# uncbiag/OAI_analysis_2

Measured on AMD Instinct MI355X. Metric: knee MRI volumes/sec (segment+register), 384x384x160 fp32, higher is better.
Workload: dtype fp16x3 (every fp32 value held as 2 fp16 terms = 22 mantissa bits, 3 MFMA passes per product, fp32 accumulate; fp32 in and out of every entry point; full-size parity vs the reference in `parity`)

## Files before the change

### include/oai_hip.h

```cpp
#ifndef OAI_HIP_H
#define OAI_HIP_H

#include <stddef.h>
#include <stdint.h>

#ifdef __cplusplus
extern "C" {
#endif

#define OAI_OK 0
#define OAI_ERR_ARG 1
#define OAI_ERR_HIP 2
#define OAI_ERR_WORKSPACE 3

int oai_version(void);
const char* oai_last_error(void);
int oai_device_info(char* name, int cap);


int oai_grid_sample3d(const float* src_dev, int C, int d, int h, int w,
                      const float* coords_dev, int D, int H, int W, float* out_dev, void* stream);

int oai_warp_set_option(const char* name, int value);

int oai_compose(const float* disp_dev, int d, int h, int w, const float* coords_dev,
                int D, int H, int W, int shortcut, float* out_dev, void* stream);

int oai_avgpool2_3d(const float* in_dev, int C, int D, int H, int W, float* out_dev, void* stream);

int oai_resize_trilinear(const float* in_dev, int C, int d, int h, int w,
                         float* out_dev, int D, int H, int W, void* stream);

int oai_phi_to_itk_displacement(const float* phi_dev, int D, int H, int W, double* disp_dev, void* stream);

#define OAI_WARP_CHAIN_MAX_FIELDS 8
int oai_warp_chain(const float* start_dev, int D, int H, int W, int n_fields, const float* const* fields,
                   const int* field_dims_zyx, const float* image_dev, int id, int ih, int iw, float* out_dev, void* stream);

typedef struct oai_affine { double A[9]; double b[3]; } oai_affine;

int oai_resample_through_disp(const float* prob_dev, int nzA, int nyA, int nxA,
                              const double* disp_dev, int Dn, int Hn, int Wn,
                              const oai_affine* b_index_to_net, const oai_affine* net_to_a_index,
                              float* out_dev, int nzB, int nyB, int nxB, void* stream);

int oai_resample_maps_through_phi(const float* probs_dev, int n_maps, int nzA, int nyA, int nxA,
                                  const float* phi_dev, int Dn, int Hn, int Wn,
                                  const oai_affine* b_index_to_net, const oai_affine* net_to_a_index,
                                  float* out_dev, int nzB, int nyB, int nxB, void* stream);

size_t oai_image_normalize_workspace_bytes(void);
int oai_image_normalize(const float* in_dev, size_t n, float pct_lo, float pct_hi, float out_min, float out_max,
                        float* out_dev, float* window_out_dev, void* workspace_dev, size_t workspace_bytes, void* stream);


typedef struct oai_unet oai_unet;

typedef struct oai_layer_params {
    int kind, cin, cout;
    const float* weight_host;
    const float* bias_host;
    const float* bn_gamma_host;
    const float* bn_beta_host;
    const float* bn_mean_host;
    const float* bn_var_host;
} oai_layer_params;

#define OAI_UNET_NUM_LAYERS 18

int oai_unet_create(const oai_layer_params layers_host[OAI_UNET_NUM_LAYERS], float bn_eps, oai_unet** out);
void oai_unet_destroy(oai_unet* h);

#define OAI_PREC_F32 0
#define OAI_PREC_BF16X3 1
#define OAI_PREC_BF16X6 2
#define OAI_PREC_FP16X3 3
int oai_unet_set_precision(oai_unet* h, int mode);
int oai_unet_range_flag(oai_unet* h, int reset, int* out, void* stream);
int oai_unet_range_flag_snapshot(oai_unet* h, int* dst_dev, void* stream);
#define OAI_UNET_RANGE_STATE_WORDS (1 + OAI_UNET_NUM_LAYERS)
int oai_unet_range_state_snapshot(oai_unet* h, int* state_dev, void* stream);
int oai_unet_range_flag_from_state(const int* state_dev, int* flag_dev, void* stream);
int oai_unet_census(oai_unet* h, float max_out[OAI_UNET_NUM_LAYERS], int reset, void* stream);
int oai_unet_calibrate_step(oai_unet* h, void* stream, int* more);
int oai_unet_get_act_exponents(const oai_unet* h, int e_out[OAI_UNET_NUM_LAYERS], int* calibrated);
int oai_unet_set_act_exponents(oai_unet* h, const int e[OAI_UNET_NUM_LAYERS]);
int oai_unet_set_option(oai_unet* h, const char* name, int value);

size_t oai_unet_workspace_bytes(const oai_unet* h, int td, int th, int tw, int batch);
size_t oai_segment_workspace_bytes(const oai_unet* h, int D, int H, int W, const int tile_zyx[3], const int overlap_zyx[3], int batch);

int oai_unet_forward_tiles(oai_unet* h, const float* tiles_dev, float* logits_dev, int B,
                           int td, int th, int tw, void* workspace_dev, size_t workspace_bytes,
                           void* stream);

int oai_segment_tiles(oai_unet* h, const float* vol_dev, int D, int H, int W,
                      const int tile_zyx[3], const int overlap_zyx[3], const int crop_zyx[3],
                      int tile_begin, int tile_end,
                      int out_mode, float* blocks_dev, int batch,
                      void* workspace_dev, size_t workspace_bytes, void* stream);

int oai_stitch_blocks(const float* blocks_dev, int n_classes, int D, int H, int W,
                      const int tile_zyx[3], const int overlap_zyx[3], const int crop_zyx[3],
                      float* maps_dev, void* stream);

int oai_stitch_blocks_ranged(const float* blocks_dev, int n_classes, int D, int H, int W,
                             const int tile_zyx[3], const int overlap_zyx[3], const int crop_zyx[3],
                             const int* bounds_host, int n_ranges, int slot_stride,
                             float* maps_dev, void* stream);

int oai_partition_tiles(const float* vol_dev, int D, int H, int W, const int tile_zyx[3], const int overlap_zyx[3],
                        int tile_begin, int tile_end, float* tiles_dev, void* stream);

int oai_assemble_vote(const int* tile_labels_dev, int n_labels, int D, int H, int W, const int tile_zyx[3], const int overlap_zyx[3],
                      unsigned char* out_dev, void* stream);

int oai_unet_profile(oai_unet* h, int enable);
int oai_unet_profile_read(oai_unet* h, double* conv3_ms, long long* conv3_launches);

double oai_unet_tile_flops(const oai_unet* h, int td, int th, int tw, const int overlap_zyx[3], int trimmed);
double oai_unet_volume_flops(const oai_unet* h, int D, int H, int W, const int tile_zyx[3], const int overlap_zyx[3],
                             const int crop_zyx[3], int trimmed, int conv3_only);
int oai_unet_tile_costs(const oai_unet* h, int D, int H, int W, const int tile_zyx[3], const int overlap_zyx[3],
                        const int crop_zyx[3], double* costs_host, int n_tiles);
double oai_unet_tile_flops_conv3(const oai_unet* h, int td, int th, int tw, const int overlap_zyx[3], int trimmed);


typedef struct oai_icon oai_icon;

typedef struct oai_icon_unet_params {
    const float* down_w[5]; const float* down_b[5];
    const float* up_w[5];   const float* up_b[5];
    const float* bn_gamma[5]; const float* bn_beta[5]; const float* bn_mean[5]; const float* bn_var[5];
    const float* last_w; const float* last_b;
} oai_icon_unet_params;

enum { OAI_ICON_FFVF = 0, OAI_ICON_DOWN = 1, OAI_ICON_TWO = 2 };
typedef struct oai_icon_node { int kind; int a; int b; } oai_icon_node;

int oai_icon_create(const oai_icon_unet_params* nets_host, int n_nets, const oai_icon_node* nodes_host, int n_nodes, int root,
                    int D, int H, int W, oai_icon** out);
int oai_icon_describe(const oai_icon* h, int* n_nets, int* levels_host, int* chain_len);
void oai_icon_destroy(oai_icon* h);
size_t oai_icon_workspace_bytes(const oai_icon* h);

int oai_icon_forward(oai_icon* h, const float* A_dev, const float* B_dev, float* phi_dev,
                     void* workspace_dev, size_t workspace_bytes, void* stream);

int oai_icon_set_graph(oai_icon* h, int enable);
int oai_icon_set_option(oai_icon* h, const char* name, int value);
int oai_icon_graph_info(const oai_icon* h, int* captured, long long* replays, long long* direct_runs);

int oai_icon_unet_forward(oai_icon* h, int which, const float* a_dev, const float* b_dev, int D, int H, int W,
                          float* out_dev, void* workspace_dev, size_t workspace_bytes, void* stream);

int oai_mc_table(signed char* out_256x16_host);
size_t oai_mc_workspace_bytes(int D, int H, int W);
int oai_mc_count(const float* vol_dev, int D, int H, int W, float iso, void* workspace_dev, size_t workspace_bytes,
                 long long* n_verts_host, long long* n_tris_host, void* stream);
int oai_mc_emit(const float* vol_dev, int D, int H, int W, float iso, const float spacing_xyz_host[3], const void* workspace_dev,
                float* verts_dev, int* faces_dev, void* stream);
int oai_mesh_smooth(const float* verts_in_dev, long long n_verts, const int* offsets_dev, const int* neighbours_dev,
                    int iterations, float relaxation, float* tmp_dev, float* verts_out_dev, void* stream);
int oai_mesh_point_distance(const float* points_dev, long long n_points, const float* verts_dev, const int* faces_dev,
                            long long n_tris, float* dist_dev, void* stream);
size_t oai_mesh_grid_workspace_bytes(const int grid_dims_xyz[3], long long n_tris);
int oai_mesh_point_distance_grid(const float* points_dev, long long n_points, const float* verts_dev, const int* faces_dev,
                                 long long n_tris, const float grid_lo_xyz_host[3], float cell_size, const int grid_dims_xyz_host[3],
                                 void* workspace_dev, size_t workspace_bytes, float* dist_dev, void* stream);

int oai_map_attributes(const float* src_pts_dev, long long n_src, const float* src_vals_dev, int n_comp, const float* tgt_pts_dev,
                       long long n_tgt, double radius, float* out_vals_dev, void* stream);
size_t oai_point_grid_workspace_bytes(const int grid_dims_xyz[3], long long n_src);
int oai_map_attributes_grid(const float* src_pts_dev, long long n_src, const float* src_vals_dev, int n_comp, const float* tgt_pts_dev,
                            long long n_tgt, double radius, const double grid_lo_xyz_host[3], double cell_size, const int grid_dims_xyz_host[3],
                            void* workspace_dev, size_t workspace_bytes, float* out_vals_dev, void* stream);
int oai_point_footprint(const float* src_pts_dev, long long n_src, const float* tgt_pts_dev, long long n_tgt, double radius, int* count_dev,
                        double* nearest_d2_dev, int* nearest_j_dev, void* stream);
int oai_point_footprint_grid(const float* src_pts_dev, long long n_src, const float* tgt_pts_dev, long long n_tgt, double radius,
                             const double grid_lo_xyz_host[3], double cell_size, const int grid_dims_xyz_host[3], void* workspace_dev,
                             size_t workspace_bytes, int* count_dev, double* nearest_d2_dev, int* nearest_j_dev, void* stream);
size_t oai_thickness_map_workspace_bytes(long long n_points);
int oai_fit_circle(const float* pts_dev, long long n, int col_x, int col_y, void* workspace_dev, size_t workspace_bytes, double centre_host[2],
                   double* radius_host, int* iterations_host, void* stream);
int oai_project_circle(const float* pts_dev, long long n, int col_x, int col_y, const double centre_host[2], double* angle_dev, double* z_dev,
                       void* stream);
int oai_project_plateaus(const float* pts_dev, const float* thickness_dev, long long n, void* workspace_dev, size_t workspace_bytes,
                         double* x_dev, double* y_dev, double* thickness_out_dev, long long* n_right_host, long long* n_left_host, void* stream);

size_t oai_thickness_image_workspace_bytes(long long n_faces, int height, int width);
int oai_thickness_image_build(const double* uv_dev, long long n_pts, const int* faces_dev, long long n_faces, const unsigned char* face_skip_dev,
                              const double lo_host[2], const double step_host[2], int height, int width, void* workspace_dev,
                              size_t workspace_bytes, int* owner_dev, int* corners_dev, double* weights_dev, long long* n_covered_host,
                              void* stream);
int oai_thickness_image_apply(const int* owner_dev, const int* corners_dev, const double* weights_dev, int height, int width,
                              const float* values_dev, long long n_pts, int n_knees, float* image_dev, void* stream);

#define OAI_MESH_FC 0
#define OAI_MESH_TC 1
size_t oai_mesh_split_workspace_bytes(long long n_verts, long long n_faces, int mesh_type, int n_init);
int oai_mesh_split_features(const float* verts_dev, long long n_verts, const int* faces_dev, long long n_faces, int mesh_type,
                            void* workspace_dev, size_t workspace_bytes, double* centroids_dev, double* normals_dev,
                            long long slab_counts_host[3], void* stream);
int oai_mesh_split_kmeans(long long n_faces, int mesh_type, void* workspace_dev, size_t workspace_bytes, const double* normals_dev, int n_init,
                          int max_iter, const long long slab_counts_host[3], const long long* first_centre_host, const double* uniforms_host,
                          signed char* side_dev, int* n_iter_host, void* stream);
size_t oai_mesh_submesh_workspace_bytes(long long n_verts, long long n_faces);
int oai_mesh_submesh(const float* verts_dev, long long n_verts, const int* faces_dev, long long n_faces, const signed char* side_dev, int which,
                     void* workspace_dev, size_t workspace_bytes, float* verts_out_dev, int* faces_out_dev, int* face_idx_out_dev,
                     long long* n_verts_out_host, long long* n_faces_out_host, void* stream);

size_t oai_mesh_components_workspace_bytes(long long n_verts, long long n_faces);
int oai_mesh_components(const int* faces_dev, long long n_faces, long long n_verts, void* workspace_dev, size_t workspace_bytes, int* label_dev,
                        int* rounds_host, void* stream);
size_t oai_mesh_keep_large_regions_workspace_bytes(long long n_verts, long long n_faces);
int oai_mesh_keep_large_regions(const float* verts_dev, long long n_verts, const int* faces_dev, long long n_faces, long long min_cells,
                                void* workspace_dev, size_t workspace_bytes, float* verts_out_dev, int* faces_out_dev, long long* n_verts_out_host,
                                long long* n_faces_out_host, void* stream);
size_t oai_mesh_adjacency_workspace_bytes(long long n_verts, long long n_faces);
int oai_mesh_adjacency(const int* faces_dev, long long n_faces, long long n_verts, void* workspace_dev, size_t workspace_bytes, int* offsets_dev,
                       int* nbrs_dev, long long* n_nbrs_host, void* stream);
size_t oai_mesh_grid_params_workspace_bytes(void);
int oai_mesh_grid_params(const float* verts_dev, long long n_verts, const int* faces_dev, long long n_faces, void* workspace_dev,
                         size_t workspace_bytes, double* out7_dev, void* stream);

size_t oai_cuberille_workspace_bytes(int D, int H, int W);
int oai_cuberille_count(const float* vol_dev, int D, int H, int W, float iso, void* workspace_dev, size_t workspace_bytes,
                        long long* n_verts_host, long long* n_faces_host, void* stream);
int oai_cuberille_emit(const float* vol_dev, int D, int H, int W, float iso, const double geometry_host[24], int flip_winding, int triangles,
                       int project, double threshold, double step_length, double relaxation, int max_steps, int move_after_converged,
                       void* workspace_dev, size_t workspace_bytes, long long n_verts, long long n_faces, float* verts_dev, int* faces_dev,
                       int* steps_dev, void* stream);

int oai_transform_points_through_phi(const float* pts_dev, long long n, const float* phi_dev, int Dn, int Hn, int Wn,
                                     const oai_affine* point_to_net, const oai_affine* net_to_out, float* out_dev, unsigned char* inside_dev,
                                     void* stream);

size_t oai_phi_jacobian_workspace_bytes(int D, int H, int W);
int oai_phi_jacobian(const float* phi_dev, int D, int H, int W, float* det_out_dev, void* workspace_dev, size_t workspace_bytes,
                     double* stats_dev, void* stream);
size_t oai_mask_overlap_workspace_bytes(long long n);
int oai_mask_overlap(const float* a_dev, const float* b_dev, long long n, float threshold, void* workspace_dev, size_t workspace_bytes,
                     long long* counts_dev, void* stream);

int oai_inverse_points_through_phi(const float* pts_dev, long long n, const float* phi_dev, int Dn, int Hn, int Wn,
                                   const oai_affine* point_to_net, const oai_affine* net_to_out, int max_iter, double tol, float* out_dev,
                                   unsigned char* status_dev, void* stream);
size_t oai_invert_phi_workspace_bytes(int D, int H, int W);
int oai_invert_phi(const float* phi_dev, int D, int H, int W, int max_iter, double tol, float* psi_out_dev, unsigned char* status_out_dev,
                   void* workspace_dev, size_t workspace_bytes, double* stats_dev, void* stream);

int oai_mask_surface(const float* map_dev, int D, int H, int W, float threshold, int mode, unsigned char* out_dev, void* stream);
size_t oai_edt_workspace_bytes(int D, int H, int W);
int oai_edt(const unsigned char* feature_dev, int D, int H, int W, const double spacing_xyz[3], float scale, int accumulate, float* dist_dev,
            double* sq_out_dev, void* workspace_dev, size_t workspace_bytes, long long* n_features_dev, void* stream);
size_t oai_surface_distance_workspace_bytes(long long n);
int oai_surface_distance(const unsigned char* surf_a_dev, const float* dist_to_b_dev, const unsigned char* surf_b_dev, const float* dist_to_a_dev,
                         long long n, const float* percentiles, int n_percentiles, void* workspace_dev, size_t workspace_bytes, double* out_dev,
                         void* stream);

size_t oai_image_moments_workspace_bytes(long long n);
int oai_image_moments(const float* a_dev, const float* b_dev, long long n, const unsigned char* mask_dev, void* workspace_dev,
                      size_t workspace_bytes, double* stats_dev, void* stream);
int oai_joint_histogram(const float* a_dev, const float* b_dev, long long n, const float range_a[2], const float range_b[2], int bins,
                        const unsigned char* mask_dev, long long* hist_dev, void* stream);
int oai_histogram_entropies(const long long* hist_dev, int bins, double* out_dev, void* stream);
size_t oai_lncc_workspace_bytes(int D, int H, int W);
int oai_lncc(const float* a_dev, const float* b_dev, int D, int H, int W, const double* taps_host, int radius, double eps,
             const unsigned char* mask_dev, double* cc_out_dev, void* workspace_dev, size_t workspace_bytes, double* stats_dev, void* stream);

size_t oai_label_components_workspace_bytes(int D, int H, int W);
int oai_label_components(const float* map_dev, const unsigned char* mask_dev, int D, int H, int W, float threshold, int complement,
                         int connectivity, long long min_voxels, int* labels_dev, int* size_dev, void* workspace_dev, size_t workspace_bytes,
                         long long* summary_dev, void* stream);
int oai_component_sizes(const int* labels_dev, long long n, long long n_components, long long* sizes_dev, void* stream);

size_t oai_local_thickness_workspace_bytes(int D, int H, int W);
// ... 19 lines not shown
```

### oai_analysis_2_amd/_lib.py

```python
from __future__ import annotations

import ctypes as C
import os
from typing import Optional

HERE = os.path.dirname(os.path.abspath(__file__))
LIB_PATH = os.environ.get("OAI_LIB_PATH") or os.path.join(HERE, "liboai_hip.so")


class OaiError(RuntimeError):
    pass


class Affine(C.Structure):
    _fields_ = [("A", C.c_double * 9), ("b", C.c_double * 3)]


class LayerParams(C.Structure):
    _fields_ = [("kind", C.c_int), ("cin", C.c_int), ("cout", C.c_int),
                ("weight", C.c_void_p), ("bias", C.c_void_p),
                ("bn_gamma", C.c_void_p), ("bn_beta", C.c_void_p), ("bn_mean", C.c_void_p), ("bn_var", C.c_void_p)]


class IconUnetParams(C.Structure):
    _fields_ = [("down_w", C.c_void_p * 5), ("down_b", C.c_void_p * 5),
                ("up_w", C.c_void_p * 5), ("up_b", C.c_void_p * 5),
                ("bn_gamma", C.c_void_p * 5), ("bn_beta", C.c_void_p * 5),
                ("bn_mean", C.c_void_p * 5), ("bn_var", C.c_void_p * 5),
                ("last_w", C.c_void_p), ("last_b", C.c_void_p)]


class IconNode(C.Structure):
    _fields_ = [("kind", C.c_int), ("a", C.c_int), ("b", C.c_int)]


_I, _P, _F, _Z, _D = C.c_int, C.c_void_p, C.c_float, C.c_size_t, C.c_double
_I3 = C.POINTER(C.c_int)
SIGNATURES = {
    "oai_version": (_I, []),
    "oai_last_error": (C.c_char_p, []),
    "oai_device_info": (_I, [C.c_char_p, _I]),
    "oai_grid_sample3d": (_I, [_P, _I, _I, _I, _I, _P, _I, _I, _I, _P, _P]),
    "oai_compose": (_I, [_P, _I, _I, _I, _P, _I, _I, _I, _I, _P, _P]),
    "oai_avgpool2_3d": (_I, [_P, _I, _I, _I, _I, _P, _P]),
    "oai_resize_trilinear": (_I, [_P, _I, _I, _I, _I, _P, _I, _I, _I, _P]),
    "oai_phi_to_itk_displacement": (_I, [_P, _I, _I, _I, _P, _P]),
    "oai_resample_through_disp": (_I, [_P, _I, _I, _I, _P, _I, _I, _I, C.POINTER(Affine), C.POINTER(Affine),
                                       _P, _I, _I, _I, _P]),
    "oai_warp_chain": (_I, [_P, _I, _I, _I, _I, C.POINTER(_P), C.POINTER(_I), _P, _I, _I, _I, _P, _P]),
    "oai_resample_maps_through_phi": (_I, [_P, _I, _I, _I, _I, _P, _I, _I, _I, C.POINTER(Affine), C.POINTER(Affine),
                                           _P, _I, _I, _I, _P]),
    "oai_unet_tile_costs": (_I, [_P, _I, _I, _I, C.POINTER(C.c_int), C.POINTER(C.c_int), C.POINTER(C.c_int), C.POINTER(C.c_double), _I]),
    "oai_mc_table": (_I, [_P]),
    "oai_mc_workspace_bytes": (_Z, [_I, _I, _I]),
    "oai_mc_count": (_I, [_P, _I, _I, _I, _F, _P, _Z, C.POINTER(C.c_longlong), C.POINTER(C.c_longlong), _P]),
    "oai_mc_emit": (_I, [_P, _I, _I, _I, _F, C.POINTER(C.c_float), _P, _P, _P, _P]),
    "oai_mesh_smooth": (_I, [_P, C.c_longlong, _P, _P, _I, _F, _P, _P, _P]),
    "oai_mesh_point_distance": (_I, [_P, C.c_longlong, _P, _P, C.c_longlong, _P, _P]),
    "oai_mesh_grid_workspace_bytes": (_Z, [C.POINTER(C.c_int), C.c_longlong]),
    "oai_mesh_point_distance_grid": (_I, [_P, C.c_longlong, _P, _P, C.c_longlong, C.POINTER(C.c_float), _F, C.POINTER(C.c_int), _P, _Z, _P, _P]),
    "oai_map_attributes": (_I, [_P, C.c_longlong, _P, _I, _P, C.c_longlong, _D, _P, _P]),
    "oai_point_grid_workspace_bytes": (_Z, [C.POINTER(C.c_int), C.c_longlong]),
    "oai_map_attributes_grid": (_I, [_P, C.c_longlong, _P, _I, _P, C.c_longlong, _D, C.POINTER(_D), _D, C.POINTER(C.c_int), _P, _Z, _P, _P]),
    "oai_point_footprint": (_I, [_P, C.c_longlong, _P, C.c_longlong, _D, _P, _P, _P, _P]),
    "oai_point_footprint_grid": (_I, [_P, C.c_longlong, _P, C.c_longlong, _D, C.POINTER(_D), _D, C.POINTER(C.c_int), _P, _Z, _P, _P, _P, _P]),
    "oai_thickness_map_workspace_bytes": (_Z, [C.c_longlong]),
    "oai_fit_circle": (_I, [_P, C.c_longlong, _I, _I, _P, _Z, C.POINTER(_D), C.POINTER(_D), C.POINTER(_I), _P]),
    "oai_project_circle": (_I, [_P, C.c_longlong, _I, _I, C.POINTER(_D), _P, _P, _P]),
    "oai_project_plateaus": (_I, [_P, _P, C.c_longlong, _P, _Z, _P, _P, _P, C.POINTER(C.c_longlong), C.POINTER(C.c_longlong), _P]),
    "oai_thickness_image_workspace_bytes": (_Z, [C.c_longlong, _I, _I]),
    "oai_thickness_image_build": (_I, [_P, C.c_longlong, _P, C.c_longlong, _P, C.POINTER(_D), C.POINTER(_D), _I, _I, _P, _Z, _P, _P, _P,
                                       C.POINTER(C.c_longlong), _P]),
    "oai_thickness_image_apply": (_I, [_P, _P, _P, _I, _I, _P, C.c_longlong, _I, _P, _P]),
    "oai_mesh_split_workspace_bytes": (_Z, [C.c_longlong, C.c_longlong, _I, _I]),
    "oai_mesh_split_features": (_I, [_P, C.c_longlong, _P, C.c_longlong, _I, _P, _Z, _P, _P, C.POINTER(C.c_longlong), _P]),
    "oai_mesh_split_kmeans": (_I, [C.c_longlong, _I, _P, _Z, _P, _I, _I, C.POINTER(C.c_longlong), C.POINTER(C.c_longlong), C.POINTER(_D), _P,
                                   C.POINTER(_I), _P]),
    "oai_mesh_submesh_workspace_bytes": (_Z, [C.c_longlong, C.c_longlong]),
    "oai_mesh_submesh": (_I, [_P, C.c_longlong, _P, C.c_longlong, _P, _I, _P, _Z, _P, _P, _P, C.POINTER(C.c_longlong), C.POINTER(C.c_longlong), _P]),
    "oai_mesh_components_workspace_bytes": (_Z, [C.c_longlong, C.c_longlong]),
    "oai_mesh_components": (_I, [_P, C.c_longlong, C.c_longlong, _P, _Z, _P, C.POINTER(_I), _P]),
    "oai_mesh_keep_large_regions_workspace_bytes": (_Z, [C.c_longlong, C.c_longlong]),
    "oai_mesh_keep_large_regions": (_I, [_P, C.c_longlong, _P, C.c_longlong, C.c_longlong, _P, _Z, _P, _P, C.POINTER(C.c_longlong),
                                         C.POINTER(C.c_longlong), _P]),
    "oai_mesh_adjacency_workspace_bytes": (_Z, [C.c_longlong, C.c_longlong]),
    "oai_mesh_adjacency": (_I, [_P, C.c_longlong, C.c_longlong, _P, _Z, _P, _P, C.POINTER(C.c_longlong), _P]),
    "oai_mesh_grid_params_workspace_bytes": (_Z, []),
    "oai_mesh_grid_params": (_I, [_P, C.c_longlong, _P, C.c_longlong, _P, _Z, _P, _P]),
    "oai_cuberille_workspace_bytes": (_Z, [_I, _I, _I]),
    "oai_cuberille_count": (_I, [_P, _I, _I, _I, _F, _P, _Z, C.POINTER(C.c_longlong), C.POINTER(C.c_longlong), _P]),
    "oai_cuberille_emit": (_I, [_P, _I, _I, _I, _F, C.POINTER(_D), _I, _I, _I, _D, _D, _D, _I, _I, _P, _Z, C.c_longlong, C.c_longlong,
                                _P, _P, _P, _P]),
    "oai_transform_points_through_phi": (_I, [_P, C.c_longlong, _P, _I, _I, _I, C.POINTER(Affine), C.POINTER(Affine), _P, _P, _P]),
    "oai_phi_jacobian_workspace_bytes": (_Z, [_I, _I, _I]),
    "oai_phi_jacobian": (_I, [_P, _I, _I, _I, _P, _P, _Z, _P, _P]),
    "oai_inverse_points_through_phi": (_I, [_P, C.c_longlong, _P, _I, _I, _I, C.POINTER(Affine), C.POINTER(Affine), _I, _D, _P, _P, _P]),
    "oai_invert_phi_workspace_bytes": (_Z, [_I, _I, _I]),
    "oai_invert_phi": (_I, [_P, _I, _I, _I, _I, _D, _P, _P, _P, _Z, _P, _P]),
    "oai_mask_overlap_workspace_bytes": (_Z, [C.c_longlong]),
    "oai_mask_overlap": (_I, [_P, _P, C.c_longlong, _F, _P, _Z, _P, _P]),
    "oai_mask_surface": (_I, [_P, _I, _I, _I, _F, _I, _P, _P]),
    "oai_edt_workspace_bytes": (_Z, [_I, _I, _I]),
    "oai_edt": (_I, [_P, _I, _I, _I, C.POINTER(_D), _F, _I, _P, _P, _P, _Z, _P, _P]),
    "oai_surface_distance_workspace_bytes": (_Z, [C.c_longlong]),
    "oai_surface_distance": (_I, [_P, _P, _P, _P, C.c_longlong, C.POINTER(_F), _I, _P, _Z, _P, _P]),
    "oai_image_moments_workspace_bytes": (_Z, [C.c_longlong]),
    "oai_image_moments": (_I, [_P, _P, C.c_longlong, _P, _P, _Z, _P, _P]),
    "oai_joint_histogram": (_I, [_P, _P, C.c_longlong, C.POINTER(_F), C.POINTER(_F), _I, _P, _P, _P]),
    "oai_histogram_entropies": (_I, [_P, _I, _P, _P]),
    "oai_lncc_workspace_bytes": (_Z, [_I, _I, _I]),
    "oai_lncc": (_I, [_P, _P, _I, _I, _I, C.POINTER(_D), _I, _D, _P, _P, _P, _Z, _P, _P]),
    "oai_label_components_workspace_bytes": (_Z, [_I, _I, _I]),
    "oai_label_components": (_I, [_P, _P, _I, _I, _I, _F, _I, _I, C.c_longlong, _P, _P, _P, _Z, _P, _P]),
    "oai_component_sizes": (_I, [_P, C.c_longlong, C.c_longlong, _P, _P]),
    "oai_local_thickness_workspace_bytes": (_Z, [_I, _I, _I]),
    "oai_local_thickness": (_I, [_P, _I, _I, _I, C.POINTER(_D), C.c_longlong, _P, _P, _P, _Z, _P, _P]),
    "oai_masked_stats_workspace_bytes": (_Z, [C.c_longlong]),
    "oai_masked_stats": (_I, [_P, _P, C.c_longlong, C.POINTER(_F), _I, _P, _Z, _P, _P]),
    "oai_mesh_areas_workspace_bytes": (_Z, [C.c_longlong, C.c_longlong]),
    "oai_mesh_areas": (_I, [_P, C.c_longlong, _P, C.c_longlong, _P, _Z, _P, _P, _P]),
    "oai_region_stats_workspace_bytes": (_Z, [C.c_longlong, _I]),
    "oai_region_stats": (_I, [_P, _P, _P, _P, C.c_longlong, _I, _P, _Z, _P, _P]),
    "oai_image_normalize_workspace_bytes": (_Z, []),
    "oai_image_normalize": (_I, [_P, _Z, _F, _F, _F, _F, _P, _P, _P, _Z, _P]),
    "oai_partition_tiles": (_I, [_P, _I, _I, _I, _I3, _I3, _I, _I, _P, _P]),
    "oai_assemble_vote": (_I, [_P, _I, _I, _I, _I, _I3, _I3, _P, _P]),
    "oai_unet_create": (_I, [C.POINTER(LayerParams), _F, C.POINTER(_P)]),
    "oai_unet_destroy": (None, [_P]),
    "oai_unet_set_precision": (_I, [_P, _I]),
    "oai_unet_range_flag": (_I, [_P, _I, C.POINTER(_I), _P]),
    "oai_unet_range_flag_snapshot": (_I, [_P, _P, _P]),
    "oai_unet_range_state_snapshot": (_I, [_P, _P, _P]),
    "oai_unet_range_flag_from_state": (_I, [_P, _P, _P]),
    "oai_unet_census": (_I, [_P, C.POINTER(_F), _I, _P]),
    "oai_unet_calibrate_step": (_I, [_P, _P, C.POINTER(_I)]),
    "oai_unet_get_act_exponents": (_I, [_P, C.POINTER(_I), C.POINTER(_I)]),
    "oai_unet_set_act_exponents": (_I, [_P, C.POINTER(_I)]),
    "oai_unet_set_option": (_I, [_P, C.c_char_p, _I]),
    "oai_unet_workspace_bytes": (_Z, [_P, _I, _I, _I, _I]),
    "oai_segment_workspace_bytes": (_Z, [_P, _I, _I, _I, _I3, _I3, _I]),
    "oai_unet_forward_tiles": (_I, [_P, _P, _P, _I, _I, _I, _I, _P, _Z, _P]),
    "oai_segment_tiles": (_I, [_P, _P, _I, _I, _I, _I3, _I3, _I3, _I, _I, _I, _P, _I, _P, _Z, _P]),
    "oai_unet_volume_flops": (_D, [_P, _I, _I, _I, _I3, _I3, _I3, _I, _I]),
    "oai_warp_set_option": (_I, [C.c_char_p, _I]),
    "oai_stitch_blocks": (_I, [_P, _I, _I, _I, _I, _I3, _I3, _I3, _P, _P]),
    "oai_stitch_blocks_ranged": (_I, [_P, _I, _I, _I, _I, _I3, _I3, _I3, _P, _I, _I, _P, _P]),
    "oai_unet_tile_flops": (_D, [_P, _I, _I, _I, _I3, _I]),
    "oai_unet_tile_flops_conv3": (_D, [_P, _I, _I, _I, _I3, _I]),
    "oai_unet_profile": (_I, [_P, _I]),
    "oai_unet_profile_read": (_I, [_P, C.POINTER(_D), C.POINTER(C.c_longlong)]),
    "oai_icon_create": (_I, [C.POINTER(IconUnetParams), _I, C.POINTER(IconNode), _I, _I, _I, _I, _I, C.POINTER(_P)]),
    "oai_icon_describe": (_I, [_P, C.POINTER(_I), C.POINTER(_I), C.POINTER(_I)]),
    "oai_icon_destroy": (None, [_P]),
    "oai_icon_workspace_bytes": (_Z, [_P]),
    "oai_icon_forward": (_I, [_P, _P, _P, _P, _P, _Z, _P]),
    "oai_icon_set_graph": (_I, [_P, _I]),
    "oai_icon_set_option": (_I, [_P, C.c_char_p, _I]),
    "oai_icon_graph_info": (_I, [_P, C.POINTER(_I), C.POINTER(C.c_longlong), C.POINTER(C.c_longlong)]),
    "oai_icon_unet_forward": (_I, [_P, _I, _P, _P, _I, _I, _I, _P, _P, _Z, _P]),
}

_lib: Optional[C.CDLL] = None


def load() -> C.CDLL:
    global _lib
    if _lib is not None:
        return _lib
    import torch
    if not os.path.exists(LIB_PATH):
        raise OaiError(f"{LIB_PATH} is missing: build it with `python -m oai_analysis_2_amd.build` "
                       "(there is no CPU fallback in this package)")
    lib = C.CDLL(LIB_PATH)
    for name, (res, args) in SIGNATURES.items():
        fn = getattr(lib, name, None)
        if fn is None:
            raise OaiError(f"liboai_hip.so does not export {name}")
        fn.restype = res
        fn.argtypes = args
    _lib = lib
    return lib


def check(status: int, what: str = "") -> None:
    if status != 0:
        msg = load().oai_last_error()
        raise OaiError(f"{what or 'liboai_hip'} failed ({status}): {msg.decode() if msg else '?'}")


STREAM = object()


def call(name: str, *args, device=None) -> None:
    if name not in SIGNATURES:
        raise OaiError(f"{name} is not an entry point of liboai_hip.so (include/oai_hip.h declares none of that name)")
    if device is None:
        if any(a is STREAM for a in args):
            raise ValueError(f"{name}: STREAM stands for the current stream of a device, and no device was given")
        check(getattr(load(), name)(*args), name)
        return
    import torch
    with torch.cuda.device(device):
        stream = torch.cuda.current_stream().cuda_stream
        check(getattr(load(), name)(*[stream if a is STREAM else a for a in args]), name)

# ... 10 lines not shown
```

### oai_analysis_2_amd/csrc/unet.hip

```cpp
#include <cmath>
#include <cstdint>
#include <cstdlib>
#include <cstring>
#include <vector>

#include "common.h"
#include "unet_kernels.h"
#include "unet_sres.h"
#include "unet_sres2.h"
#include "unet_wino.h"
#include "unet_wino_f32.h"

namespace oai {

enum LayerId { EC0, EC1, EC2, EC3, EC4, EC5, EC6, EC7, DC9, DC8, DC7, DC6, DC5, DC4, DC3, DC2, DC1, DC0 };
__host__ __device__ static inline int layer_level(int k) { const int v[18] = {0, 0, 1, 1, 2, 2, 3, 3, 2, 2, 2, 1, 1, 1, 0, 0, 0, 0}; return v[k]; }
__host__ __device__ static inline int layer_kind(int k) { const int v[18] = {0, 0, 0, 0, 0, 0, 0, 0, 2, 1, 1, 2, 1, 1, 2, 1, 1, 3}; return v[k]; }
static const int kKind[18] = {0, 0, 0, 0, 0, 0, 0, 0, 2, 1, 1, 2, 1, 1, 2, 1, 1, 3};

struct Layer {
    int kind = 0, cin = 0, cout = 0;
    int c0 = 0, c1 = 0;
    float4* panel = nullptr;
    float4* panel_bf[3] = {nullptr, nullptr, nullptr};
    float* scale_f16 = nullptr;
    float* shift_f16 = nullptr;
    float* plain_f16 = nullptr;
    std::vector<float> ws;
    int rel1 = 0;
    size_t panel_f16_floats = 0;
    float4* panel_wino_f32 = nullptr;
    float4* panel_wino = nullptr;
    size_t panel_wino_floats = 0;
    float4* panel_wino16 = nullptr;
    size_t panel_wino16_floats = 0;
    float4* panel_m16 = nullptr;
    size_t panel_m16_floats = 0;
    std::vector<float> wk_host;
    std::vector<float> scale_host, shift_host, plain_host;
    float* plain = nullptr;
    float* scale = nullptr;
    float* shift = nullptr;
};

}

struct oai_unet {
    oai::Layer L[18];
    int variant = 0;
    int precision = OAI_PREC_F32;
    int* range_flag = nullptr;
    unsigned* census = nullptr;
    int* eval_out = nullptr;
    int act_exp[18] = {0};
    bool calibrated = false;
    int opt_wino_f32 = 1;
    int opt_first_blocks = 24;
    int opt_up_nbw = 0;
    int opt_shared = 1;
    int opt_wide = 1;
    int opt_wino = 19;
    int opt_wino_layers = 0x3FFFF;
    int opt_m16 = 1;
    int opt_m16_layers = 0x3FFFF;
    int opt_dead_stores = 1;
    int opt_census = 1;
    int xcd_group = 32;
    int fuse_first = 1;
    int sres_mrep = 4;
    bool opt_sres = true;
    bool sres = false;
    unsigned char* zero_rec = nullptr;
    int n_classes = 0;
    std::vector<void*> allocs;
    bool profile = false;
    std::vector<hipEvent_t> ev_pool;
    size_t ev_used = 0;
};

#ifdef OAI_DIAG
static unsigned long long* g_diag_stamps = nullptr;
static unsigned long long* diag_stamps() {
    if (!g_diag_stamps && oai::diag_env("OAI_STAMPS", 0)) {
        if (hipMalloc((void**)&g_diag_stamps, 32 * sizeof(unsigned long long)) != hipSuccess) return nullptr;
        (void)hipMemset(g_diag_stamps, 0, 32 * sizeof(unsigned long long));
    }
    return g_diag_stamps;
}
extern "C" int oai_diag_stamps(unsigned long long out[32], int reset) {
    if (!g_diag_stamps) return 1;
    if (hipMemcpy(out, g_diag_stamps, 32 * sizeof(unsigned long long), hipMemcpyDeviceToHost) != hipSuccess) return 2;
    if (reset) (void)hipMemset(g_diag_stamps, 0, 32 * sizeof(unsigned long long));
    return 0;
}
#endif

namespace oai {

static int conv_kc(int variant) { return variant == 1 ? 16 : 8; }

static std::vector<float> canonical_k3(const oai_layer_params& p) {
    std::vector<float> w((size_t)27 * p.cin * p.cout);
    for (int t = 0; t < 27; ++t)
        for (int ci = 0; ci < p.cin; ++ci)
            for (int co = 0; co < p.cout; ++co) {
                float v;
                if (p.kind == 0) v = p.weight_host[((size_t)co * p.cin + ci) * 27 + t];
                else v = p.weight_host[((size_t)ci * p.cout + co) * 27 + (26 - t)];
                w[((size_t)t * p.cin + ci) * p.cout + co] = v;
            }
    return w;
}

struct ChunkSrc {
    bool first;
    int Csrc, cofs, cl0;
    ChunkSrc(int ch, int C0, int C1, int KC) {
        const int nch0 = (C0 + KC - 1) / KC;
        first = ch < nch0; Csrc = first ? C0 : C1; cofs = first ? 0 : C0; cl0 = (first ? ch : ch - nch0) * KC;
    }
};

static std::vector<float> pack_conv3_panel(const std::vector<float>& wk, int C0, int C1, int Cout, int KC) {
    const int Cin = C0 + C1, KG = KC / 8;
    const int ncb = (Cout + 63) / 64, nch0 = (C0 + KC - 1) / KC, nch1 = (C1 + KC - 1) / KC;
    std::vector<float> out(((size_t)ncb * (nch0 + nch1) * 27 * KG * 2 + 2) * 64 * 4, 0.0f);
    size_t o = 0;
    for (int cb = 0; cb < ncb; ++cb)
        for (int ch = 0; ch < nch0 + nch1; ++ch) {
            const ChunkSrc cs(ch, C0, C1, KC);
            for (int t = 0; t < 27; ++t)
                for (int kg = 0; kg < KG; ++kg)
                    for (int nr = 0; nr < 2; ++nr)
                        for (int lane = 0; lane < 64; ++lane)
                            for (int s = 0; s < 4; ++s, ++o) {
                                const int cl = cs.cl0 + kg * 8 + 4 * (lane >> 5) + s;
                                const int co = cb * 64 + nr * 32 + (lane & 31);
                                if (cl < cs.Csrc && co < Cout) out[o] = wk[((size_t)t * Cin + cs.cofs + cl) * Cout + co];
                            }
        }
    return out;
}

static inline double wino_u(int f, double g0, double g1, double g2) { return f == 0 ? g0 : f == 1 ? 0.5 * (g0 + g1 + g2) : f == 2 ? 0.5 * (g0 - g1 + g2) : g2; }

static inline float wino_weight(const std::vector<float>& wk, int f, int t, int Cin, int ci, int Cout, int co, double scale = 1.0) {
    const size_t i = ((size_t)(t * 3) * Cin + ci) * Cout + co, dx = (size_t)Cin * Cout;
    return (float)wino_u(f, wk[i] * scale, wk[i + dx] * scale, wk[i + 2 * dx] * scale);
}

static std::vector<float> pack_wino_f32_panel(const std::vector<float>& wk, int C0, int C1, int Cout) {
    constexpr int KC = 8;
    const int Cin = C0 + C1;
    const int ncb = (Cout + 63) / 64, nch0 = (C0 + KC - 1) / KC, nch1 = (C1 + KC - 1) / KC;
    std::vector<float> out(((size_t)ncb * 4 * (nch0 + nch1) * 9 * 2 + 6) * 64 * 4, 0.0f);
    size_t o = 0;
    for (int cb = 0; cb < ncb; ++cb)
        for (int f = 0; f < 4; ++f)
            for (int ch = 0; ch < nch0 + nch1; ++ch) {
                const ChunkSrc cs(ch, C0, C1, KC);
                for (int q = 0; q < 9; ++q)
                    for (int nr = 0; nr < 2; ++nr)
                        for (int lane = 0; lane < 64; ++lane)
                            for (int s = 0; s < 4; ++s, ++o) {
                                const int cl = cs.cl0 + 4 * (lane >> 5) + s;
                                const int co = cb * 64 + nr * 32 + (lane & 31);
                                if (cl < cs.Csrc && co < Cout) out[o] = wino_weight(wk, f, q, Cin, cs.cofs + cl, Cout, co);
                            }
            }
    return out;
}

static inline uint16_t f32_to_bf16_rne(float f) {
    uint32_t u;
    memcpy(&u, &f, 4);
    if ((u & 0x7fffffffu) > 0x7f800000u) return (uint16_t)((u >> 16) | 0x40);
    u += 0x7fffu + ((u >> 16) & 1u);
    return (uint16_t)(u >> 16);
}
static inline float bf16_to_f32(uint16_t b) {
    uint32_t u = (uint32_t)b << 16;
    float f;
    memcpy(&f, &u, 4);
    return f;
}

static inline uint16_t f32_to_f16_rne(float f) {
    uint32_t u;
    memcpy(&u, &f, 4);
    const uint32_t sign = (u >> 16) & 0x8000u;
    u &= 0x7fffffffu;
    if (u >= 0x7f800000u) return (uint16_t)(sign | (u > 0x7f800000u ? 0x7e00u : 0x7c00u));
    if (u >= 0x477ff000u) return (uint16_t)(sign | 0x7c00u);
    if (u < 0x33000001u) return (uint16_t)sign;
    int e = (int)(u >> 23) - 127;
    uint32_t m = (u & 0x7fffffu) | 0x800000u;
    int shift = e < -14 ? (-14 - e) + 13 : 13;
    uint32_t half = m >> shift, rem = m & ((1u << shift) - 1), mid = 1u << (shift - 1);
    if (rem > mid || (rem == mid && (half & 1))) ++half;
    uint32_t out = e < -14 ? half : (((uint32_t)(e + 15) << 10) + (half - 0x400u));
    return (uint16_t)(sign | out);
}
static inline float f16_to_f32(uint16_t h) {
    const uint32_t sign = (uint32_t)(h & 0x8000u) << 16;
    uint32_t e = (h >> 10) & 31u, m = h & 0x3ffu, u;
    if (e == 0) {
        if (m == 0) u = sign;
        else { int s = 0; while (!(m & 0x400u)) { m <<= 1; ++s; } u = sign | ((uint32_t)(113 - s) << 23) | ((m & 0x3ffu) << 13); }
    } else if (e == 31) u = sign | 0x7f800000u | (m << 13);
    else u = sign | ((e + 112) << 23) | (m << 13);
    float f;
// ... 129 lines not shown
    std::vector<float> out((size_t)nnb * nkg * 2 * 64 * 4, 0.0f);
    size_t o = 0;
    for (int nb = 0; nb < nnb; ++nb)
        for (int kg = 0; kg < nkg; ++kg)
            for (int nr = 0; nr < 2; ++nr)
                for (int lane = 0; lane < 64; ++lane)
                    for (int s = 0; s < 4; ++s, ++o) {
                        const int ci = kg * 8 + 4 * (lane >> 5) + s;
                        const int col = nb * 64 + nr * 32 + (lane & 31);
                        if (ci < p.cin && col < N) {
                            const int par = col / p.cout, co = col % p.cout;
                            out[o] = p.weight_host[((size_t)ci * p.cout + co) * 8 + par];
                        }
                    }
    return out;
}

static std::vector<float> pack_up_panel_f16(const float* w , int cin, int cout, const std::vector<float>& wscale) {
    const int N = 8 * cout, nnb = (N + 63) / 64, nks = (cin + 15) / 16;
    std::vector<float> out((size_t)nnb * nks * 4 * 64 * 4, 0.0f);
    uint16_t* o16 = reinterpret_cast<uint16_t*>(out.data());
    size_t u = 0;
    for (int nb = 0; nb < nnb; ++nb)
        for (int ks = 0; ks < nks; ++ks)
            for (int k = 0; k < 2; ++k)
                for (int nr = 0; nr < 2; ++nr)
                    for (int lane = 0; lane < 64; ++lane, ++u)
                        for (int j = 0; j < 8; ++j) {
                            const int ci = ks * 16 + 8 * (lane >> 5) + j;
                            const int col = nb * 64 + nr * 32 + (lane & 31);
                            if (ci < cin && col < N) {
                                const int par = col / cout, co = col % cout;
                                o16[u * 8 + j] = f16_term(w[((size_t)ci * cout + co) * 8 + par] * wscale[co], k);
                            }
                        }
    return out;
}

template <typename T>
static int upload(oai_unet* h, const std::vector<float>& v, T** dst) {
    void* d = nullptr;
    OAI_CHECK_HIP(hipMalloc(&d, v.size() * sizeof(float)));
    h->allocs.push_back(d);
    OAI_CHECK_HIP(hipMemcpy(d, v.data(), v.size() * sizeof(float), hipMemcpyHostToDevice));
    *dst = reinterpret_cast<T*>(d);
    return OAI_OK;
}

template <typename T>
static int upload_into(oai_unet* h, const std::vector<float>& v, T** dst) {
    if (!*dst) return upload(h, v, dst);
    OAI_CHECK_HIP(hipMemcpy(*dst, v.data(), v.size() * sizeof(float), hipMemcpyHostToDevice));
    return OAI_OK;
}

static inline int layer_src0(int k) { return k - 1; }
static inline int layer_src1(int k) { return k == DC8 ? EC5 : k == DC5 ? EC3 : k == DC2 ? EC1 : -1; }

static int pack_wino_layer(oai_unet* h, int k) {
    Layer& L = h->L[k];
    if (L.kind == 2 || L.wk_host.empty() || L.cout % 64 != 0 || L.ws.empty()) return OAI_OK;
    const std::vector<float> panel = pack_wino_panel(L.wk_host, L.c0, L.c1, L.cout, L.ws, ldexpf(1.0f, L.rel1));
    if (L.panel_wino && panel.size() != L.panel_wino_floats) return set_error(OAI_ERR_ARG, "Winograd panel of layer %d changed size", k);
    L.panel_wino_floats = panel.size();
    if (int rc = upload_into(h, panel, &L.panel_wino)) return rc;
    const std::vector<float> p16 = pack_wino16_panel(L.wk_host, L.c0, L.c1, L.cout, L.ws, ldexpf(1.0f, L.rel1));
    if (L.panel_wino16 && p16.size() != L.panel_wino16_floats) return set_error(OAI_ERR_ARG, "16x16x32 Winograd panel of layer %d changed size", k);
    L.panel_wino16_floats = p16.size();
    return upload_into(h, p16, &L.panel_wino16);
}

static int pack_fp16_layer(oai_unet* h, int k) {
    Layer& L = h->L[k];
    const int s1 = layer_src1(k);
    const int rel1 = s1 >= 0 ? h->act_exp[layer_src0(k)] - h->act_exp[s1] : 0;
    const float f1 = ldexpf(1.0f, rel1);
    L.ws.assign(L.cout, 1.0f);
    std::vector<float> panel;
    if (L.kind == 2) {
        for (int co = 0; co < L.cout; ++co) {
            float amax = 0.0f;
            for (int ci = 0; ci < L.cin; ++ci)
                for (int q = 0; q < 8; ++q) amax = fmaxf(amax, fabsf(L.wk_host[((size_t)ci * L.cout + co) * 8 + q]));
            if (amax > 0.0f && std::isfinite(amax)) { int e; frexpf(amax, &e); L.ws[co] = ldexpf(1.0f, 8 - e); }
        }
        panel = pack_up_panel_f16(L.wk_host.data(), L.cin, L.cout, L.ws);
    } else {
        const int Cin = L.c0 + L.c1;
        const size_t per = L.wk_host.size() / L.cout;
        for (int co = 0; co < L.cout; ++co) {
            float amax = 0.0f;
            for (size_t i = 0; i < per; ++i)
                amax = fmaxf(amax, fabsf(L.wk_host[i * L.cout + co]) * ((int)(i % Cin) >= L.c0 ? f1 : 1.0f));
            if (amax > 0.0f && std::isfinite(amax)) { int e; frexpf(amax, &e); L.ws[co] = ldexpf(1.0f, 8 - e); }
        }
        panel = pack_conv3_panel_bf(L.wk_host, L.c0, L.c1, L.cout, 2, true, &L.ws, f1);
    }
    if (L.panel_bf[2] && panel.size() != L.panel_f16_floats) return set_error(OAI_ERR_ARG, "fp16 panel of layer %d changed size", k);
    L.panel_f16_floats = panel.size();
    L.rel1 = rel1;
    if (int rc = upload_into(h, panel, &L.panel_bf[2])) return rc;
    if (L.kind != 2) {
        const std::vector<float> p16 = pack_conv3_m16_panel(L.wk_host, L.c0, L.c1, L.cout, L.ws, f1);
        if (L.panel_m16 && p16.size() != L.panel_m16_floats) return set_error(OAI_ERR_ARG, "16x16x32 panel of layer %d changed size", k);
        L.panel_m16_floats = p16.size();
        if (int rc = upload_into(h, p16, &L.panel_m16)) return rc;
    }
    return (h->opt_wino || L.panel_wino) ? pack_wino_layer(h, k) : OAI_OK;
}

static int refresh_fp16_affine(oai_unet* h) {
    for (int k = 0; k < 17; ++k) {
        Layer& L = h->L[k];
        const int e_out = h->act_exp[k], e_in = k == EC0 ? 0 : h->act_exp[layer_src0(k)];
        std::vector<float> sc(L.cout), sh(L.cout);
        for (int co = 0; co < L.cout; ++co) {
            const float ws = L.ws.empty() ? 1.0f : L.ws[co];
            sc[co] = ldexpf(L.scale_host[co] / ws, e_out - e_in);
            sh[co] = ldexpf(L.shift_host[co], e_out);
        }
        if (int rc = upload_into(h, sc, &L.scale_f16)) return rc;
        if (int rc = upload_into(h, sh, &L.shift_f16)) return rc;
    }
    Layer& H = h->L[DC0];
    std::vector<float> w(H.plain_host.size());
    for (size_t i = 0; i < w.size(); ++i) w[i] = ldexpf(H.plain_host[i], -h->act_exp[DC1]);
    return upload_into(h, w, &H.plain_f16);
}

struct Box { int lo[3], hi[3]; };

__host__ __device__ static void full_box(Box& b, const int dims[3]) { for (int i = 0; i < 3; ++i) { b.lo[i] = 0; b.hi[i] = dims[i]; } }

__host__ __device__ static void plan_regions(const int tile[3], const int keep_lo[3], const int keep_hi[3], bool trimmed, Box need[18]) {
    int dims[4][3];
    for (int l = 0; l < 4; ++l) for (int i = 0; i < 3; ++i) dims[l][i] = tile[i] >> l;
    for (int k = 0; k < 18; ++k) full_box(need[k], dims[layer_level(k)]);
    for (int i = 0; i < 3; ++i) { need[DC0].lo[i] = keep_lo[i]; need[DC0].hi[i] = keep_hi[i]; }
    if (!trimmed) return;
    auto grow = [&](const Box& b, int lvl) { Box r; for (int i = 0; i < 3; ++i) { r.lo[i] = b.lo[i] > 0 ? b.lo[i] - 1 : 0; r.hi[i] = b.hi[i] + 1 < dims[lvl][i] ? b.hi[i] + 1 : dims[lvl][i]; } return r; };
    auto halve = [&](const Box& b) { Box r; for (int i = 0; i < 3; ++i) { r.lo[i] = b.lo[i] / 2; r.hi[i] = (b.hi[i] + 1) / 2; } return r; };
    Box keep; for (int i = 0; i < 3; ++i) { keep.lo[i] = keep_lo[i]; keep.hi[i] = keep_hi[i]; }
    need[DC0] = keep; need[DC1] = keep;
    need[DC2] = grow(need[DC1], 0);
    need[DC3] = grow(need[DC2], 0);
    need[DC4] = halve(need[DC3]);
    need[DC5] = grow(need[DC4], 1);
    need[DC6] = grow(need[DC5], 1);
    need[DC7] = halve(need[DC6]);
    need[DC8] = grow(need[DC7], 2);
}

constexpr int kMaxTilesPerTable = 4096;
enum Buf { B_E0, B_SYN0, B_P0, B_E2, B_SYN1, B_P1, B_E4, B_SYN2, B_P2, B_E6, B_E7, B_U9, B_D8, B_D7, B_U6, B_D5, B_D4, B_U3, B_D2, B_D1, B_COUNT };

static size_t carve_workspace(const oai_unet* h, int td, int th, int tw, int batch, const void* base, float* buf[B_COUNT], int*& table) {
    const size_t v0 = (size_t)td * th * tw, v1 = v0 / 8, v2 = v1 / 8, v3 = v2 / 8;
    const oai::Layer* L = h->L;
    auto pc = [&](int k) { return (size_t)((L[k].cout + 15) / 16 * 16); };
    const size_t sizes[B_COUNT] = {
        v0 * pc(EC0), v0 * pc(EC1), v1 * pc(EC1), v1 * pc(EC2), v1 * pc(EC3), v2 * pc(EC3),
        v2 * pc(EC4), v2 * pc(EC5), v3 * pc(EC5), v3 * pc(EC6), v3 * pc(EC7), v2 * pc(DC9),
        v2 * pc(DC8), v2 * pc(DC7), v1 * pc(DC6), v1 * pc(DC5), v1 * pc(DC4), v0 * pc(DC3),
        v0 * pc(DC2), v0 * pc(DC1)};
    Ws ws(base);
    table = ws.take<int>((size_t)18 * kMaxTilesPerTable * 6);
    for (int i = 0; i < B_COUNT; ++i) buf[i] = ws.take<float>(sizes[i] * batch);
    return ws.off;
}
static size_t workspace_bytes(const oai_unet* h, int td, int th, int tw, int batch) {
    float* buf[B_COUNT];
    int* table;
    return carve_workspace(h, td, th, tw, batch, nullptr, buf, table);
}

static int launch_begin(const oai_unet* h, hipStream_t st) {
    if (!h->profile) return OAI_OK;
    oai_unet* hm = const_cast<oai_unet*>(h);
    while (hm->ev_used + 2 > hm->ev_pool.size()) {
        hipEvent_t e;
        OAI_CHECK_HIP(hipEventCreate(&e));
        hm->ev_pool.push_back(e);
    }
    OAI_CHECK_HIP(hipEventRecord(hm->ev_pool[hm->ev_used], st));
    return OAI_OK;
}
static int launch_end(const oai_unet* h, hipStream_t st) {
    OAI_CHECK_LAUNCH();
    if (!h->profile) return OAI_OK;
    oai_unet* hm = const_cast<oai_unet*>(h);
    OAI_CHECK_HIP(hipEventRecord(hm->ev_pool[hm->ev_used + 1], st));
    hm->ev_used += 2;
    return OAI_OK;
}

static unsigned xcd_deal(const oai_unet* h, unsigned grid, int& nblocks, int& xcd_group) {
    if (h->xcd_group <= 0) return grid;
    nblocks = (int)grid; xcd_group = h->xcd_group;
    const unsigned q = 8u * (unsigned)h->xcd_group;
    return (grid + q - 1) / q * q;
}

static inline int layer_id(const oai_unet* h, const Layer& L) { return (int)(&L - h->L); }
static inline bool layer_bit(const oai_unet* h, int mask, const Layer& L) { return (mask >> layer_id(h, L)) & 1; }
static inline unsigned* census_of(const oai_unet* h, int k) { return h->opt_census ? h->census + 16 * k : nullptr; }
#ifdef OAI_DIAG
static unsigned long long* layer_stamps(const oai_unet* h, const Layer& L) {
    static const int only = diag_env("OAI_STAMP_LAYER", -1);
    return only >= 0 && layer_id(h, L) != only ? nullptr : diag_stamps();
}
#endif

static inline unsigned capped_blocks(size_t total, size_t cap) { return (unsigned)std::min<size_t>((total + 255) / 256, cap); }

template <int RX, int RY, int WY, int WX, int V = 0>
static void launch_sres2(int var, unsigned grid, hipStream_t st, const ConvArgs& a, const unsigned char* zero_rec) {
#ifdef OAI_DIAG
    if constexpr (V < 10)
        if (var != V) return launch_sres2<RX, RY, WY, WX, V + 1>(var, grid, st, a, zero_rec);
#endif
    conv3_igemm_sres2<RX, RY, WY, WX, V><<<grid, 512, 0, st>>>(a, zero_rec);
}

template <int MREP, int KC, int RX, int RY, int WY, int WX>
static int launch_conv3_shape(const oai_unet* h, ConvArgs a, const Box& box, int ntiles, hipStream_t st, int mrep_override = 0) {
    for (int i = 0; i < 3; ++i) { a.lo[i] = box.lo[i]; a.hi[i] = box.hi[i]; }
    if (box.hi[0] <= box.lo[0] || box.hi[1] <= box.lo[1] || box.hi[2] <= box.lo[2]) return OAI_OK;
    const int sres_mrep = mrep_override ? mrep_override : h->sres_mrep;
    constexpr bool kMainShape = RX == 16 && RY == 2 && WY == 4 && WX == 1;
    constexpr bool kWideShape = kMainShape || (RX == 16 && RY == 2 && WY == 2 && WX == 2);
    bool wide = KC == 8 && kWideShape && h->sres && h->opt_wide && sres_mrep == 4 && !a.first_w && !a.head_w && a.Cout % 128 == 0;
    if (wide && h->opt_wide == 1) {
        const size_t nwg = (size_t)ntiles * cdiv(box.hi[0] - box.lo[0], 4) * cdiv(box.hi[1] - box.lo[1], WY * RY) * cdiv(box.hi[2] - box.lo[2], WX * RX) * (a.Cout / 128);
        wide = nwg >= (kMainShape ? 1024 : 512);
    }
    if (wide) a.ncb = a.Cout / 128;
    const bool bf = KC == 8 && h->precision != OAI_PREC_F32;
    constexpr int kF32Mrep = MREP > 2 ? 2 : MREP;
    a.nbz = cdiv(box.hi[0] - box.lo[0], bf ? (h->sres ? sres_mrep : 2) : kF32Mrep);
    a.nby = cdiv(box.hi[1] - box.lo[1], WY * RY);
    a.nbx = cdiv(box.hi[2] - box.lo[2], WX * RX);
    unsigned grid = (unsigned)((size_t)ntiles * a.nbz * a.nby * a.nbx * a.ncb);
    if (KC == 8 && h->sres) grid = xcd_deal(h, grid, a.nblocks, a.xcd_group);
    if (int rc = launch_begin(h, st)) return rc;
    if (KC == 8 && h->sres) {
        static const int one_wg = diag_env("OAI_ONE_WG", 0);
        bool done = false;
        const bool m16 = h->opt_m16 && a.wpanel16 && a.Cout % 128 != 0 && !one_wg;
        if (m16) a.wpanel = a.wpanel16;
        if constexpr (RX == 16 && RY == 2 && WY == 4 && WX == 1) {
            if (a.first_w) {
                if (m16) conv3_igemm_sres<4, RX, RY, WY, WX, true, true><<<grid, 256, 0, st>>>(a, h->zero_rec);
                else conv3_igemm_sres<4, RX, RY, WY, WX, true><<<grid, 256, 0, st>>>(a, h->zero_rec);
                done = true;
            }
        }
        if constexpr (kWideShape) {
            if (wide) {
                static const int var = diag_env("OAI_WIDE_VAR", 0);
                launch_sres2<RX, RY, WY, WX>(var >= 1 && var <= 10 ? var : 0, grid, st, a, h->zero_rec);
                done = true;
            }
        }
        if (done) { }
        else if (a.first_w) return set_error(OAI_ERR_ARG, "fused ec0 asked of a tile shape that has no such kernel");
        else if (m16 && sres_mrep == 4) conv3_igemm_sres<4, RX, RY, WY, WX, false, true><<<grid, 256, 0, st>>>(a, h->zero_rec);
        else if (m16) conv3_igemm_sres<2, RX, RY, WY, WX, false, true><<<grid, 256, 0, st>>>(a, h->zero_rec);
        else if (sres_mrep == 4) conv3_igemm_sres<4, RX, RY, WY, WX><<<grid, 256, one_wg ? 24 * 1024 : 0, st>>>(a, h->zero_rec);
        else conv3_igemm_sres<2, RX, RY, WY, WX><<<grid, 256, 0, st>>>(a, h->zero_rec);
    }
    else if (KC == 8 && h->precision == OAI_PREC_BF16X3) conv3_igemm_bf16s<2, false, 2, RX, RY, WY, WX><<<grid, 256, 0, st>>>(a);
    else if (KC == 8 && h->precision == OAI_PREC_BF16X6) conv3_igemm_bf16s<3, false, 2, RX, RY, WY, WX><<<grid, 256, 0, st>>>(a);
    else if (KC == 8 && h->precision == OAI_PREC_FP16X3) conv3_igemm_bf16s<2, true, 2, RX, RY, WY, WX><<<grid, 256, 0, st>>>(a);
    else conv3_igemm_f32<kF32Mrep, KC, RX, RY, WY, WX><<<grid, 256, 0, st>>>(a);
    return launch_end(h, st);
}

struct Cover { Box main, xs, ys; int hr, wr; };
static Cover cover_box(const Box& box, int xunit, int tall_y, int tall_x, bool no_strips) {
    const int ry = box.hi[1] - box.lo[1], rx = box.hi[2] - box.lo[2], ny = ry / 8, nx = rx / xunit;
    Cover c{box, box, box, ry - 8 * ny, rx - xunit * nx};
    if (no_strips || ny == 0 || nx == 0) c.hr = c.wr = 0;
    if (c.hr > tall_y) c.hr = 0;
    if (c.wr > tall_x) c.wr = 0;
    if (c.hr) c.main.hi[1] = box.lo[1] + 8 * ny;
    if (c.wr) c.main.hi[2] = box.lo[2] + xunit * nx;
    c.xs.lo[2] = c.main.hi[2];
    c.ys.lo[1] = c.main.hi[1]; c.ys.hi[2] = c.main.hi[2];
    return c;
}
static Cover direct_cover(const oai_unet* h, const Box& box) { return cover_box(box, 16, 4, 8, h->variant == 2); }

static bool first_fusion_ok(const oai_unet* h) {
    return h->sres && h->fuse_first && h->variant == 0 && h->sres_mrep == 4 && h->L[EC0].cout == 32 && h->L[EC1].c0 == 32;
}
static bool first_fusable(const oai_unet* h, const Box& ec1_box) {
    if (!first_fusion_ok(h)) return false;
    const Cover c = direct_cover(h, ec1_box);
    return c.hr == 0 && c.wr == 0;
}

struct Scatter { const int* boxes; int ntiles, tile0; int g[3], e[3], t[3]; };

static int fill_conv_args(const oai_unet* h, const Layer& L, const float* s0, const float* s1, float* out, const int dims[3],
                          const int* boxes, float* pool_out, const ConvArgs* head, const TileSource* first, const int* store_boxes,
                          const Scatter* sc, ConvArgs& a) {
    if (head) a = *head;
    if (store_boxes && h->sres && h->opt_dead_stores) { a.store_boxes = store_boxes; a.store_grow = 1; }
    if (first) {
        a.first_w = h->L[EC0].plain; a.first_scale = h->L[EC0].scale_f16; a.first_shift = h->L[EC0].shift_f16; a.first_src = *first;
        a.first_census = census_of(h, EC0);
    }
    if (sc) {
        a.sc_boxes = sc->boxes; a.sc_ntiles = sc->ntiles; a.sc_tile0 = sc->tile0;
        for (int i = 0; i < 3; ++i) { a.sc_g[i] = sc->g[i]; a.sc_e[i] = sc->e[i]; a.sc_t[i] = sc->t[i]; }
    }
    a.boxes = boxes;
    a.pool_out = pool_out;
    a.range_flag = h->range_flag;
#ifdef OAI_DIAG
    a.stamps = layer_stamps(h, L);
#endif
    a.src0 = s0; a.src1 = s1; a.C0 = L.c0; a.C1 = s1 ? L.c1 : 0;
    const bool f16 = h->precision == OAI_PREC_FP16X3;
    a.out = out; a.Cout = L.cout; a.scale = f16 ? L.scale_f16 : L.scale; a.shift = f16 ? L.shift_f16 : L.shift;
    a.census = h->sres ? census_of(h, layer_id(h, L)) : nullptr;
    a.wpanel = h->precision == OAI_PREC_F32 ? L.panel : L.panel_bf[h->precision == OAI_PREC_BF16X3 ? 0 : h->precision == OAI_PREC_BF16X6 ? 1 : 2];
    a.wpanel16 = h->precision == OAI_PREC_FP16X3 && layer_bit(h, h->opt_m16_layers, L) ? L.panel_m16 : nullptr;
    a.D = dims[0]; a.H = dims[1]; a.W = dims[2];
    a.ncb = (L.cout + 63) / 64;
    a.relu = 1;
    if (h->sres && (size_t)dims[0] * dims[1] * dims[2] * 128 >= (1ull << 32))
        return set_error(OAI_ERR_ARG, "tile level %dx%dx%d too large for the split-resident kernel (>= 2^25 voxels)", dims[0], dims[1], dims[2]);
    return OAI_OK;
}

template <int RX, int RY, int WY, int WX>
static int launch_conv3_one(const oai_unet* h, const Layer& L, const float* s0, float* out, const int dims[3], const Box& box, int ntiles,
                            hipStream_t st, const int* boxes, float* pool_only = nullptr) {
    ConvArgs a;
    if (int rc = fill_conv_args(h, L, s0, nullptr, out, dims, boxes, pool_only, nullptr, nullptr, nullptr, nullptr, a)) return rc;
    if (pool_only) { a.store_boxes = boxes; a.store_grow = -(1 << 20); }
    return launch_conv3_shape<4, 8, RX, RY, WY, WX>(h, a, box, ntiles, st, pool_only ? 2 : 0);
}

static bool wino_ws_fits() {
    static const bool fits = [] {
        auto one = [](auto kern) { int n = 0; return hipOccupancyMaxActiveBlocksPerMultiprocessor(&n, kern, 512, 0) == hipSuccess && n >= 1; };
        return one(conv3_wino_sres<1, 8, 4, 1, true>) && one(conv3_wino_sres<1, 16, 2, 1, true>) &&
               one(conv3_wino_sres<1, 8, 4, 1, true, true>) && one(conv3_wino_sres<1, 16, 2, 1, true, true>);
    }();
    return fits;
}
static bool wino_m16_64(const oai_unet* h, const Layer& L, int cout) {
    return cout % 128 != 0 && (h->opt_wino & 32) && !(h->opt_wino & (4 | 8)) && L.panel_wino16 && wino_ws_fits();
}

template <int TY, int NP>
static int launch_wino_shape(const oai_unet* h, const Layer& L, ConvArgs a, const Box& box, int ntiles, hipStream_t st) {
    for (int i = 0; i < 3; ++i) { a.lo[i] = box.lo[i]; a.hi[i] = box.hi[i]; }
    if (box.hi[0] <= box.lo[0] || box.hi[1] <= box.lo[1] || box.hi[2] <= box.lo[2]) return OAI_OK;
    const int ng = (a.Cout % 128 == 0 && !((h->opt_wino & 8) && TY != 4)) ? 2 : 1;
    a.wpanel = L.panel_wino;
    a.ncb = a.Cout / (64 * ng);
    a.nbz = cdiv(box.hi[0] - box.lo[0], 4); a.nby = cdiv(box.hi[1] - box.lo[1], TY); a.nbx = cdiv(box.hi[2] - box.lo[2], 2 * NP);
    unsigned grid = (unsigned)((size_t)ntiles * a.nbz * a.nby * a.nbx * a.ncb);
    grid = xcd_deal(h, grid, a.nblocks, a.xcd_group);
    if (int rc = launch_begin(h, st)) return rc;
    if (ng == 2 && (h->opt_wino & 16) && L.panel_wino16) {
        a.wpanel = L.panel_wino16;
        conv3_wino_sres<2, TY, NP, 1, false, true><<<grid, 512, 0, st>>>(a, h->zero_rec);
    } else if (ng == 2) conv3_wino_sres<2, TY, NP><<<grid, 512, 0, st>>>(a, h->zero_rec);
    else if constexpr (TY != 4) {
        if ((h->opt_wino & 4) || !wino_ws_fits()) conv3_wino_sres<1, TY, NP, 2><<<grid, 512, 0, st>>>(a, h->zero_rec);
        else if (wino_m16_64(h, L, a.Cout)) {
            a.wpanel = L.panel_wino16;
            conv3_wino_sres<1, TY, NP, 1, true, true><<<grid, 512, 0, st>>>(a, h->zero_rec);
        } else conv3_wino_sres<1, TY, NP, 1, true><<<grid, 512, 0, st>>>(a, h->zero_rec);
    } else if (wino_m16_64(h, L, a.Cout)) {
        a.wpanel = L.panel_wino16;
        conv3_wino_sres<1, TY, NP, 2, false, true><<<grid, 512, 0, st>>>(a, h->zero_rec);
    } else conv3_wino_sres<1, TY, NP, 2><<<grid, 512, 0, st>>>(a, h->zero_rec);
    return launch_end(h, st);
}

static int launch_conv3_wino(const oai_unet* h, const Layer& L, const ConvArgs& a, Box box, int ntiles, hipStream_t st) {
    box.lo[2] &= ~1;
    const Cover c = cover_box(box, 8, 4, 4, false);
    if (int rc = launch_wino_shape<8, 4>(h, L, a, c.main, ntiles, st)) return rc;
    if (c.wr)
        if (int rc = launch_wino_shape<16, 2>(h, L, a, c.xs, ntiles, st)) return rc;
    if (c.hr)
        if (int rc = launch_wino_shape<4, 8>(h, L, a, c.ys, ntiles, st)) return rc;
    return OAI_OK;
}

static bool wino_pool_box(const Box& box, const int dims[3]) {
    for (int i = 0; i < 3; ++i)
        if (box.lo[i] != 0 || box.hi[i] != dims[i] || (dims[i] & 1)) return false;
    return dims[0] % 4 == 0 && dims[1] % 8 == 0 && dims[2] % 8 == 0;
}

template <int TY, int NP>
static int launch_wino_f32_shape(const oai_unet* h, const Layer& L, ConvArgs a, const Box& box, int ntiles, hipStream_t st) {
    for (int i = 0; i < 3; ++i) { a.lo[i] = box.lo[i]; a.hi[i] = box.hi[i]; }
    if (box.hi[0] <= box.lo[0] || box.hi[1] <= box.lo[1] || box.hi[2] <= box.lo[2]) return OAI_OK;
    a.wpanel = L.panel_wino_f32;
    a.ncb = (a.Cout + 63) / 64;
    a.nbz = cdiv(box.hi[0] - box.lo[0], 2); a.nby = cdiv(box.hi[1] - box.lo[1], TY); a.nbx = cdiv(box.hi[2] - box.lo[2], 2 * NP);
    unsigned grid = (unsigned)((size_t)ntiles * a.nbz * a.nby * a.nbx * a.ncb);
    grid = xcd_deal(h, grid, a.nblocks, a.xcd_group);
    if (int rc = launch_begin(h, st)) return rc;
    conv3_wino_f32<TY, NP><<<grid, 256, 0, st>>>(a, reinterpret_cast<const float*>(h->zero_rec));
    return launch_end(h, st);
}

static int launch_conv3_wino_f32(const oai_unet* h, const Layer& L, const ConvArgs& a, Box box, int ntiles, hipStream_t st) {
    box.lo[2] &= ~1;
    const Cover c = cover_box(box, 8, 4, 4, a.pool_out != nullptr);
    if (int rc = launch_wino_f32_shape<8, 4>(h, L, a, c.main, ntiles, st)) return rc;
    if (c.wr)
        if (int rc = launch_wino_f32_shape<16, 2>(h, L, a, c.xs, ntiles, st)) return rc;
    if (c.hr)
        if (int rc = launch_wino_f32_shape<4, 8>(h, L, a, c.ys, ntiles, st)) return rc;
    return OAI_OK;
}

static int launch_conv3(const oai_unet* h, const Layer& L, const float* s0, const float* s1, float* out,
                        const int dims[3], const Box& box, int ntiles, hipStream_t st, const int* boxes = nullptr,
                        float* pool_out = nullptr, const ConvArgs* head = nullptr, const TileSource* first = nullptr,
                        const int* store_boxes = nullptr, const Scatter* sc = nullptr) {
    ConvArgs a;
    if (int rc = fill_conv_args(h, L, s0, s1, out, dims, boxes, pool_out, head, first, store_boxes, sc, a)) return rc;
    if (h->variant == 1) return launch_conv3_shape<2, 16, 16, 2, 4, 1>(h, a, box, ntiles, st);
    if (h->precision == OAI_PREC_F32 && h->variant == 0 && h->opt_wino_f32 && L.panel_wino_f32 && a.Cout % 4 == 0 && !a.head_w && !a.first_w && !a.sc_boxes &&
        (!a.pool_out || (wino_pool_box(box, dims) && dims[0] % 2 == 0)) && layer_bit(h, h->opt_wino_layers, L))
        return launch_conv3_wino_f32(h, L, a, box, ntiles, st);
    if (h->sres && h->opt_wino && L.panel_wino && h->sres_mrep == 4 && !a.first_w && !a.head_w && !a.sc_boxes &&
        (!a.pool_out || (a.Cout % 128 == 0 && a.relu && wino_pool_box(box, dims))) && a.Cout % 64 == 0 && (h->opt_wino & (a.Cout % 128 == 0 ? 1 : 2)) && (a.Cout % 128 == 0 || (a.C0 + 15) / 16 + (a.C1 + 15) / 16 >= 8) && layer_bit(h, h->opt_wino_layers, L) && (size_t)dims[0] * dims[1] * dims[2] < (1u << 24))
        return launch_conv3_wino(h, L, a, box, ntiles, st);
    const Cover c = direct_cover(h, box);
    if (int rc = launch_conv3_shape<4, 8, 16, 2, 4, 1>(h, a, c.main, ntiles, st)) return rc;
    if (c.wr) {
        const int rc = c.wr <= 2 ? launch_conv3_shape<4, 8, 2, 16, 4, 1>(h, a, c.xs, ntiles, st)
                     : c.wr <= 4 ? launch_conv3_shape<4, 8, 4, 8, 4, 1>(h, a, c.xs, ntiles, st)
                                 : launch_conv3_shape<4, 8, 8, 4, 4, 1>(h, a, c.xs, ntiles, st);
        if (rc) return rc;
    }
    if (!c.hr) return OAI_OK;
    return c.hr <= 2 ? launch_conv3_shape<4, 8, 16, 2, 1, 4>(h, a, c.ys, ntiles, st) : launch_conv3_shape<4, 8, 16, 2, 2, 2>(h, a, c.ys, ntiles, st);
}

static int launch_up(const oai_unet* h, const Layer& L, const float* src, float* out, const int in_dims[3], const Box& out_need,
                     int ntiles, hipStream_t st, const int* in_boxes = nullptr) {
    UpArgs a;
    a.boxes = in_boxes;
    a.range_flag = h->range_flag;
    a.zero = h->zero_rec;
#ifdef OAI_DIAG
    a.stamps = layer_stamps(h, L);
#endif
    const bool split = h->precision == OAI_PREC_FP16X3 && L.panel_bf[2];
    a.src = src; a.Cin = L.cin; a.out = out; a.Cout = L.cout;
    a.wpanel = split ? L.panel_bf[2] : L.panel;
    a.scale = split ? L.scale_f16 : L.scale;
    a.shift = split ? L.shift_f16 : L.shift;
    a.census = h->sres ? census_of(h, layer_id(h, L)) : nullptr;
    a.D = in_dims[0]; a.H = in_dims[1]; a.W = in_dims[2];
    for (int i = 0; i < 3; ++i) { a.lo[i] = out_need.lo[i] / 2; a.hi[i] = (out_need.hi[i] + 1) / 2; }
    const int nvox = (a.hi[0] - a.lo[0]) * (a.hi[1] - a.lo[1]) * (a.hi[2] - a.lo[2]);
    a.nmb = cdiv(nvox, split && h->sres ? 128 : 64);
    a.nnb = cdiv(8 * L.cout, 256);
    a.relu = 1;
    if (split && h->sres) {
        a.nbw = 1;
        if (L.cout % 16 == 0 && h->opt_up_nbw > 1) a.nbw = std::min(h->opt_up_nbw, a.nnb);
        else if (L.cout % 16 == 0 && h->opt_up_nbw == 0) {
            a.nbw = a.nnb;
            while (a.nbw > 1 && (size_t)ntiles * a.nmb * cdiv(a.nnb, a.nbw) < 8192) a.nbw = (a.nbw + 1) / 2;
        }
        const unsigned grid = xcd_deal(h, (unsigned)((size_t)ntiles * a.nmb * cdiv(a.nnb, a.nbw)), a.nblocks, a.xcd_group);
        upconv2_igemm_sres<<<grid, 256, 0, st>>>(a);
    }
    else if (split) upconv2_igemm<true><<<(unsigned)((size_t)ntiles * a.nmb * a.nnb), 256, 0, st>>>(a);
    else upconv2_igemm<false><<<(unsigned)((size_t)ntiles * a.nmb * a.nnb), 256, 0, st>>>(a);
    OAI_CHECK_LAUNCH();
    return OAI_OK;
}

static bool pool_fusable(const oai_unet* h, const int dims[3], const Box& box) {
    if (h->variant != 0) return false;
    for (int i = 0; i < 3; ++i) if (box.lo[i] != 0 || box.hi[i] != dims[i]) return false;
    return dims[0] % 4 == 0 && dims[1] % 8 == 0 && dims[2] % 16 == 0;
}

static int launch_pool(const oai_unet* h, const float* in, float* out, const int dims[3], int C, int ntiles, hipStream_t st, int shell_only = 0) {
    if (h->sres) {
        const int nch = (C + 15) / 16;
        const size_t Do = dims[0] / 2, Ho = dims[1] / 2, Wo = dims[2] / 2;
        const size_t faces = Do * Ho * Wo - (Do - 2) * (Ho - 2) * (Wo - 2) - (shell_only == 2 ? 2 * Ho * Wo : 0);
        const size_t total = (size_t)ntiles * (shell_only ? faces : Do * Ho * Wo) * nch * 4;
        maxpool2_sres_kernel<<<capped_blocks(total, 256 * 32), 256, 0, st>>>(reinterpret_cast<const unsigned char*>(in), reinterpret_cast<unsigned char*>(out),
                                                                dims[0], dims[1], dims[2], nch, total, shell_only);
        OAI_CHECK_LAUNCH();
        return OAI_OK;
    }
    const size_t total4 = (size_t)ntiles * (dims[0] / 2) * (dims[1] / 2) * (dims[2] / 2) * (C / 4);
    maxpool2_kernel<<<capped_blocks(total4, 256 * 32), 256, 0, st>>>(in, out, dims[0], dims[1], dims[2], C, total4);
    OAI_CHECK_LAUNCH();
    return OAI_OK;
}

struct SharedEnc {
    float* SP0;
    int PD, PH, PW;
    const float* vol; int D, H, W;
    int grid[3], eff[3], overlap[3];
};

static int run_batch(oai_unet* h, const TileSource& src, int n, const Box need[18], int out_mode,
                     float* blocks_out, float* const buf[B_COUNT], hipStream_t st,
                     const int* table = nullptr, int table_tiles = 0, int t0 = 0, const SharedEnc* se = nullptr) {
    auto tb = [&](int layer) -> const int* { return table ? table + ((size_t)layer * table_tiles + t0) * 6 : nullptr; };
    const Layer* L = h->L;
    int d[4][3];
    for (int l = 0; l < 4; ++l) { d[l][0] = src.td >> l; d[l][1] = src.th >> l; d[l][2] = src.tw >> l; }
    const size_t v0 = (size_t)src.td * src.th * src.tw;

    int rc;
#define RUN(x) do { rc = (x); if (rc) return rc; } while (0)
    if (se) {
        {
            TileSource vs{};
            vs.vol = se->vol; vs.D = se->D; vs.H = se->H; vs.W = se->W; vs.td = se->PD; vs.th = se->PH; vs.tw = se->PW;
            vs.ez = se->PD; vs.ey = se->PH; vs.ex = se->PW; vs.oz = se->overlap[0]; vs.oy = se->overlap[1]; vs.ox = se->overlap[2]; vs.gy = 1; vs.gx = 1;
            const int per_row = se->grid[1] * se->grid[2], P[3] = {se->PD, se->PH, se->PW};
            Scatter sc;
            sc.boxes = tb(DC2); sc.ntiles = n; sc.tile0 = src.tile_begin;
            for (int i = 0; i < 3; ++i) { sc.g[i] = se->grid[i]; sc.e[i] = se->eff[i]; }
            sc.t[0] = src.td; sc.t[1] = src.th; sc.t[2] = src.tw;
            const int t_first = src.tile_begin, t_last = src.tile_begin + n - 1;
            const int zspan = (src.td + se->eff[0] - 1) / se->eff[0];
            const int s_first = t_first / per_row, s_last = t_last / per_row + zspan - 1;
            Box prev{}; bool have_prev = false;
            for (int s = s_first; s <= s_last; ++s) {
                int jlo = 1 << 30, jhi = -1, klo = 1 << 30, khi = -1;
                for (int i = s - zspan + 1; i <= s; ++i) {
                    if (i < 0 || i >= se->grid[0]) continue;
                    const int a0 = std::max(t_first, i * per_row), a1 = std::min(t_last, (i + 1) * per_row - 1);
                    if (a0 > a1) continue;
                    const int j0 = (a0 - i * per_row) / se->grid[2], j1 = (a1 - i * per_row) / se->grid[2];
                    jlo = std::min(jlo, j0); jhi = std::max(jhi, j1);
                    if (j0 == j1) { klo = std::min(klo, (a0 - i * per_row) % se->grid[2]); khi = std::max(khi, (a1 - i * per_row) % se->grid[2]); }
                    else { klo = 0; khi = se->grid[2] - 1; }
                }
                if (jhi < 0) continue;
                Box bx;
                bx.lo[0] = se->eff[0] * s; bx.hi[0] = std::min(P[0], se->eff[0] * (s + 1));
                if (s == s_last) bx.hi[0] = std::min(P[0], se->eff[0] * (t_last / per_row) + src.td);
                bx.lo[1] = se->eff[1] * jlo; bx.hi[1] = std::min(P[1], se->eff[1] * jhi + src.th);
                bx.lo[2] = se->eff[2] * klo; bx.hi[2] = std::min(P[2], se->eff[2] * khi + src.tw);
                if (have_prev && prev.lo[1] == bx.lo[1] && prev.hi[1] == bx.hi[1] && prev.lo[2] == bx.lo[2] && prev.hi[2] == bx.hi[2] && prev.hi[0] == bx.lo[0]) {
                    prev.hi[0] = bx.hi[0];
                    continue;
                }
                if (have_prev) RUN(launch_conv3(h, L[EC1], nullptr, nullptr, buf[B_SYN0], P, prev, 1, st, nullptr, se->SP0, nullptr, &vs, nullptr, &sc));
                prev = bx; have_prev = true;
            }
            if (have_prev) RUN(launch_conv3(h, L[EC1], nullptr, nullptr, buf[B_SYN0], P, prev, 1, st, nullptr, se->SP0, nullptr, &vs, nullptr, &sc));
        }
        const int nch1 = (L[EC1].cout + 15) / 16;
        {
            const size_t total = (size_t)n * (d[1][0] * d[1][1] * d[1][2]) * nch1 * 4;
            pooled_gather_kernel<<<capped_blocks(total, 256 * 64), 256, 0, st>>>(reinterpret_cast<const unsigned char*>(se->SP0), reinterpret_cast<unsigned char*>(buf[B_P0]), src,
                                                                   d[1][0], d[1][1], d[1][2], se->PD / 2, se->PH / 2, se->PW / 2, nch1, total);
            OAI_CHECK_LAUNCH();
        }
        {
            const size_t pairs = (size_t)6 * d[0][1] * (d[0][2] / 2) + (size_t)(d[0][0] - 6) * 6 * (d[0][2] / 2) + (size_t)(d[0][0] - 6) * (d[0][1] - 6) * 4;
            dim3 grid(std::min<unsigned>(cdiv(pairs, 256), (unsigned)h->opt_first_blocks), n);
            conv3_first_sres_kernel<32><<<grid, 256, 0, st>>>(src, L[EC0].plain, L[EC0].scale_f16, L[EC0].shift_f16, reinterpret_cast<unsigned char*>(buf[B_E0]), 1,
                                                              h->range_flag, census_of(h, EC0), 3);
            OAI_CHECK_LAUNCH();
        }
        const int td = d[0][0], th = d[0][1], tw = d[0][2];
        const Box zlo = {{0, 0, 0}, {2, th, tw}}, zhi = {{td - 2, 0, 0}, {td, th, tw}};
        const Box ylo = {{2, 0, 0}, {td - 2, 2, tw}}, yhi = {{2, th - 2, 0}, {td - 2, th, tw}};
        const Box xlo = {{2, 2, 0}, {td - 2, th - 2, 2}}, xhi = {{2, 2, tw - 2}, {td - 2, th - 2, tw}};
        const bool zpool = tb(EC1) != nullptr && h->opt_dead_stores;
        RUN((launch_conv3_one<16, 2, 4, 1>(h, L[EC1], buf[B_E0], buf[B_SYN0], d[0], zlo, n, st, tb(EC1), zpool ? buf[B_P0] : nullptr)));
        RUN((launch_conv3_one<16, 2, 4, 1>(h, L[EC1], buf[B_E0], buf[B_SYN0], d[0], zhi, n, st, tb(EC1), zpool ? buf[B_P0] : nullptr)));
        RUN((launch_conv3_one<16, 2, 1, 4>(h, L[EC1], buf[B_E0], buf[B_SYN0], d[0], ylo, n, st, tb(EC1))));
        RUN((launch_conv3_one<16, 2, 1, 4>(h, L[EC1], buf[B_E0], buf[B_SYN0], d[0], yhi, n, st, tb(EC1))));
        RUN((launch_conv3_one<2, 16, 4, 1>(h, L[EC1], buf[B_E0], buf[B_SYN0], d[0], xlo, n, st, tb(EC1))));
        RUN((launch_conv3_one<2, 16, 4, 1>(h, L[EC1], buf[B_E0], buf[B_SYN0], d[0], xhi, n, st, tb(EC1))));
        RUN(launch_pool(h, buf[B_SYN0], buf[B_P0], d[0], L[EC1].cout, n, st, zpool ? 2 : 1));
    } else {
    const bool fuse_first = first_fusable(h, need[EC1]);
    const TileSource* fsrc = fuse_first ? &src : nullptr;
    if (!fuse_first) {
        const dim3 grid_all(cdiv(v0 / 2, 256), n);
        const dim3 grid(std::min<unsigned>(cdiv(v0 / 2, 256), (unsigned)h->opt_first_blocks), n);
        const int c = L[EC0].cout;
        unsigned char* e0s = reinterpret_cast<unsigned char*>(buf[B_E0]);
        const bool f16 = h->precision == OAI_PREC_FP16X3;
        const float* sc0 = f16 ? L[EC0].scale_f16 : L[EC0].scale;
        const float* sh0 = f16 ? L[EC0].shift_f16 : L[EC0].shift;
        unsigned* cen0 = census_of(h, EC0);
        if (h->sres && c == 32) conv3_first_sres_kernel<32><<<grid, 256, 0, st>>>(src, L[EC0].plain, sc0, sh0, e0s, 1, h->range_flag, cen0, 0);
        else if (h->sres && c == 16) conv3_first_sres_kernel<16><<<grid, 256, 0, st>>>(src, L[EC0].plain, sc0, sh0, e0s, 1, h->range_flag, cen0, 0);
        else if (h->sres && c == 8) conv3_first_sres_kernel<8><<<grid, 256, 0, st>>>(src, L[EC0].plain, sc0, sh0, e0s, 1, h->range_flag, cen0, 0);
        else if (c == 32) conv3_first_kernel<32><<<grid_all, 256, 0, st>>>(src, L[EC0].plain, sc0, sh0, buf[B_E0], 1);
        else if (c == 16) conv3_first_kernel<16><<<grid_all, 256, 0, st>>>(src, L[EC0].plain, sc0, sh0, buf[B_E0], 1);
        else if (c == 8) conv3_first_kernel<8><<<grid_all, 256, 0, st>>>(src, L[EC0].plain, sc0, sh0, buf[B_E0], 1);
        else return set_error(OAI_ERR_ARG, "ec0 cout %d unsupported (8, 16 or 32)", c);
        OAI_CHECK_LAUNCH();
    }
    if (pool_fusable(h, d[0], need[EC1])) {
        RUN(launch_conv3(h, L[EC1], buf[B_E0], nullptr, buf[B_SYN0], d[0], need[EC1], n, st, tb(EC1), buf[B_P0], nullptr, fsrc, tb(DC2)));
    } else {
        RUN(launch_conv3(h, L[EC1], buf[B_E0], nullptr, buf[B_SYN0], d[0], need[EC1], n, st, tb(EC1), nullptr, nullptr, fsrc));
        RUN(launch_pool(h, buf[B_SYN0], buf[B_P0], d[0], L[EC1].cout, n, st));
    }
    }
    RUN(launch_conv3(h, L[EC2], buf[B_P0], nullptr, buf[B_E2], d[1], need[EC2], n, st, tb(EC2)));
    if (pool_fusable(h, d[1], need[EC3])) {
        RUN(launch_conv3(h, L[EC3], buf[B_E2], nullptr, buf[B_SYN1], d[1], need[EC3], n, st, tb(EC3), buf[B_P1], nullptr, nullptr, tb(DC5)));
    } else {
        RUN(launch_conv3(h, L[EC3], buf[B_E2], nullptr, buf[B_SYN1], d[1], need[EC3], n, st, tb(EC3)));
        RUN(launch_pool(h, buf[B_SYN1], buf[B_P1], d[1], L[EC3].cout, n, st));
    }
    RUN(launch_conv3(h, L[EC4], buf[B_P1], nullptr, buf[B_E4], d[2], need[EC4], n, st, tb(EC4)));
    if (pool_fusable(h, d[2], need[EC5])) {
        RUN(launch_conv3(h, L[EC5], buf[B_E4], nullptr, buf[B_SYN2], d[2], need[EC5], n, st, tb(EC5), buf[B_P2], nullptr, nullptr, tb(DC8)));
    } else {
        RUN(launch_conv3(h, L[EC5], buf[B_E4], nullptr, buf[B_SYN2], d[2], need[EC5], n, st, tb(EC5)));
        RUN(launch_pool(h, buf[B_SYN2], buf[B_P2], d[2], L[EC5].cout, n, st));
    }
    RUN(launch_conv3(h, L[EC6], buf[B_P2], nullptr, buf[B_E6], d[3], need[EC6], n, st, tb(EC6)));
    RUN(launch_conv3(h, L[EC7], buf[B_E6], nullptr, buf[B_E7], d[3], need[EC7], n, st, tb(EC7)));
    RUN(launch_up(h, L[DC9], buf[B_E7], buf[B_U9], d[3], need[DC9], n, st, tb(DC9)));
    RUN(launch_conv3(h, L[DC8], buf[B_U9], buf[B_SYN2], buf[B_D8], d[2], need[DC8], n, st, tb(DC8)));
    RUN(launch_conv3(h, L[DC7], buf[B_D8], nullptr, buf[B_D7], d[2], need[DC7], n, st, tb(DC7)));
    RUN(launch_up(h, L[DC6], buf[B_D7], buf[B_U6], d[2], need[DC6], n, st, tb(DC6)));
    RUN(launch_conv3(h, L[DC5], buf[B_U6], buf[B_SYN1], buf[B_D5], d[1], need[DC5], n, st, tb(DC5)));
    RUN(launch_conv3(h, L[DC4], buf[B_D5], nullptr, buf[B_D4], d[1], need[DC4], n, st, tb(DC4)));
    RUN(launch_up(h, L[DC3], buf[B_D4], buf[B_U3], d[1], need[DC3], n, st, tb(DC3)));
    RUN(launch_conv3(h, L[DC2], buf[B_U3], buf[B_SYN0], buf[B_D2], d[0], need[DC2], n, st, tb(DC2)));
    const int kz = src.vol ? src.oz : 0, ky = src.vol ? src.oy : 0, kx = src.vol ? src.ox : 0;
    const int ez = src.vol ? src.ez : src.td, ey = src.vol ? src.ey : src.th, ex = src.vol ? src.ex : src.tw;
    static const bool no_fuse = diag_env("OAI_NO_HEAD_FUSE", 0) != 0;
    const bool fuse_head = h->sres && !no_fuse && L[DC1].cout <= 64 && L[DC0].cin == L[DC1].cout && h->n_classes <= 4 &&
                           need[DC1].lo[0] <= need[DC0].lo[0] && need[DC1].hi[0] >= need[DC0].hi[0];
    if (fuse_head) {
        ConvArgs ha;
        ha.head_w = L[DC0].plain_f16; ha.head_b = L[DC0].shift;
        ha.head_boxes = tb(DC0); ha.head_out = blocks_out;
        ha.head_ncls = h->n_classes; ha.head_mode = out_mode;
        ha.head_k[0] = kz; ha.head_k[1] = ky; ha.head_k[2] = kx; ha.head_e[0] = ez; ha.head_e[1] = ey; ha.head_e[2] = ex;
        RUN(launch_conv3(h, L[DC1], buf[B_D2], nullptr, buf[B_D1], d[0], need[DC0], n, st, tb(DC0), nullptr, &ha));
        return OAI_OK;
    }
    RUN(launch_conv3(h, L[DC1], buf[B_D2], nullptr, buf[B_D1], d[0], need[DC1], n, st, tb(DC1)));
#undef RUN
    {
        const Box& k = need[DC0];
        const float* hw = h->precision == OAI_PREC_FP16X3 ? L[DC0].plain_f16 : L[DC0].plain;
        const int bz = k.hi[0] - k.lo[0], by = k.hi[1] - k.lo[1], bx = k.hi[2] - k.lo[2];
        dim3 grid(cdiv((size_t)bz * by * bx, 256), n);
        if (h->sres)
            head_sres_kernel<<<grid, 256, 0, st>>>(reinterpret_cast<const unsigned char*>(buf[B_D1]), L[DC0].cin, d[0][0], d[0][1], d[0][2],
                                                   k.lo[0], k.lo[1], k.lo[2], bz, by, bx, kz, ky, kx, ez, ey, ex, hw,
                                                   L[DC0].shift, h->n_classes, out_mode, blocks_out, tb(DC0));
        else
        head_kernel<<<grid, 256, 0, st>>>(buf[B_D1], L[DC0].cin, d[0][0], d[0][1], d[0][2], k.lo[0], k.lo[1], k.lo[2],
                                          bz, by, bx, kz, ky, kx, ez, ey, ex, hw, L[DC0].shift, h->n_classes,
                                          out_mode, blocks_out, tb(DC0));
        OAI_CHECK_LAUNCH();
    }
    return OAI_OK;
}

static double layer_flops(const oai_unet* h, int k, const Box& b) {
    const double vox = (double)(b.hi[0] - b.lo[0]) * (b.hi[1] - b.lo[1]) * (b.hi[2] - b.lo[2]);
    const int taps = (kKind[k] == 0 || kKind[k] == 1) ? 27 : 1;
    return 2.0 * vox * taps * h->L[k].cin * h->L[k].cout;
}

constexpr float kLowRange = 8.0f;
constexpr int kTargetExp = 10;

__global__ void range_eval_kernel(int* __restrict__ flag, unsigned* __restrict__ census, int* __restrict__ dst, int reset, float low) {
    const int t = threadIdx.x;
    unsigned m = 0;
    if (t < 18)
        for (int i = 0; i < 16; ++i) m = max(m, census[t * 16 + i]);
    const bool lowhit = t < 17 && m != 0 && __uint_as_float(m) < low;
    const unsigned long long any = __ballot(lowhit);
    if (t == 0) {
        dst[0] = flag[0] | (any ? 2 : 0);
        if (reset) flag[0] = 0;
    }
    if (reset && t < 18)
        for (int i = 0; i < 16; ++i) census[t * 16 + i] = 0;
}

__global__ void range_state_kernel(int* __restrict__ flag, unsigned* __restrict__ census, int* __restrict__ dst) {
    const int t = threadIdx.x;
    if (t < 18) {
        unsigned m = 0;
        for (int i = 0; i < 16; ++i) { m = max(m, census[t * 16 + i]); census[t * 16 + i] = 0; }
        dst[1 + t] = (int)m;
    }
    if (t == 0) { dst[0] = flag[0] & 1; flag[0] = 0; }
}

__global__ void range_flag_from_state_kernel(const int* __restrict__ state, int* __restrict__ dst, float low) {
    const int t = threadIdx.x;
    const unsigned m = t < 17 ? (unsigned)state[1 + t] : 0u;
    const bool lowhit = t < 17 && m != 0 && __uint_as_float(m) < low;
    const unsigned long long any = __ballot(lowhit);
    if (t == 0) dst[0] = (state[0] & 1) | (any ? 2 : 0);
}

}

using namespace oai;

static int stitch_impl(const float* blocks, int ncls, int D, int H, int W, const int tile[3], const int overlap[3],
                       const int crop[3], float* maps, void* stream, const StitchRanges& rg);

template <typename T>
static int alloc_zeroed(oai_unet* h, size_t bytes, T** ptr) {
    void* d = nullptr;
    if (hipMalloc(&d, bytes) != hipSuccess) return set_error(OAI_ERR_HIP, "oai_unet_create: hipMalloc failed");
    h->allocs.push_back(d);
    (void)hipMemset(d, 0, bytes);
    *ptr = reinterpret_cast<T*>(d);
    return OAI_OK;
}

static inline bool is_conv3_igemm(int k) { return k >= 1 && k < 17 && (kKind[k] == 0 || kKind[k] == 1); }

static double tile_flops(const oai_unet* h, int td, int th, int tw, const int overlap[3], int trimmed, bool conv3_only) {
    if (!h) return 0.0;
    const int tile[3] = {td, th, tw};
    int lo[3], hi[3];
    for (int i = 0; i < 3; ++i) { lo[i] = overlap ? overlap[i] : 0; hi[i] = tile[i] - lo[i]; }
    Box need[18];
    plan_regions(tile, lo, hi, trimmed != 0, need);
    double f = 0;
    for (int k = 0; k < 18; ++k)
        if (!conv3_only || is_conv3_igemm(k)) f += layer_flops(h, k, need[k]);
    return f;
}

extern "C" {

int oai_unet_create(const oai_layer_params layers[OAI_UNET_NUM_LAYERS], float bn_eps, oai_unet** out) {
    OAI_CHECK_ARG(layers && out, "oai_unet_create: null pointer");
    for (int k = 0; k < 18; ++k) {
        OAI_CHECK_ARG(layers[k].weight_host, "oai_unet_create: layer %d has no weight (strict load)", k);
        OAI_CHECK_ARG(layers[k].kind == kKind[k], "oai_unet_create: layer %d kind %d, expected %d", k, layers[k].kind, kKind[k]);
        OAI_CHECK_ARG(layers[k].cin > 0 && layers[k].cout > 0, "oai_unet_create: layer %d bad channels", k);
    }
    const int chain[][2] = {{EC0, EC1}, {EC1, EC2}, {EC2, EC3}, {EC3, EC4}, {EC4, EC5}, {EC5, EC6}, {EC6, EC7}, {EC7, DC9},
                            {DC8, DC7}, {DC7, DC6}, {DC5, DC4}, {DC4, DC3}, {DC2, DC1}, {DC1, DC0}};
    for (auto& c : chain)
        OAI_CHECK_ARG(layers[c[0]].cout == layers[c[1]].cin, "oai_unet_create: layer %d cout != layer %d cin", c[0], c[1]);
    OAI_CHECK_ARG(layers[DC8].cin == layers[DC9].cout + layers[EC5].cout, "oai_unet_create: dc8 cin != dc9 + ec5");
    OAI_CHECK_ARG(layers[DC5].cin == layers[DC6].cout + layers[EC3].cout, "oai_unet_create: dc5 cin != dc6 + ec3");
    OAI_CHECK_ARG(layers[DC2].cin == layers[DC3].cout + layers[EC1].cout, "oai_unet_create: dc2 cin != dc3 + ec1");
    OAI_CHECK_ARG(layers[EC0].cin == 1, "oai_unet_create: only in_channels == 1 is supported (the reference's config)");
    OAI_CHECK_ARG(layers[DC0].cout <= 4, "oai_unet_create: n_classes must be <= 4");
    for (int k = 0; k < 18; ++k) {
        OAI_CHECK_ARG(k == EC0 || layers[k].cin % 8 == 0, "oai_unet_create: layer %d cin must be a multiple of 8", k);
        OAI_CHECK_ARG(k == DC0 || layers[k].cout % 8 == 0, "oai_unet_create: layer %d cout must be a multiple of 8", k);
    }

    oai_unet* h = new oai_unet();
    int rc = alloc_zeroed(h, 256, &h->range_flag);
    if (!rc) rc = alloc_zeroed(h, 256, &h->zero_rec);
    if (!rc) rc = alloc_zeroed(h, 18 * 16 * sizeof(unsigned) + 256, &h->census);
    if (rc) { oai_unet_destroy(h); return rc; }
    h->eval_out = reinterpret_cast<int*>(h->census + 18 * 16);
    h->variant = diag_env("OAI_CONV_VARIANT", 0);
    if (h->variant < 0 || h->variant > 2) h->variant = 0;
    h->n_classes = layers[DC0].cout;
    const int KC = conv_kc(h->variant);
    for (int k = 0; k < 18 && rc == OAI_OK; ++k) {
        const oai_layer_params& p = layers[k];
        Layer& L = h->L[k];
        L.kind = p.kind; L.cin = p.cin; L.cout = p.cout; L.c0 = p.cin; L.c1 = 0;
        if (k == DC8) { L.c0 = layers[DC9].cout; L.c1 = layers[EC5].cout; }
        if (k == DC5) { L.c0 = layers[DC6].cout; L.c1 = layers[EC3].cout; }
        if (k == DC2) { L.c0 = layers[DC3].cout; L.c1 = layers[EC1].cout; }
        std::vector<float> sc(p.cout, 1.0f), sh(p.cout, 0.0f);
        for (int c = 0; c < p.cout; ++c) {
            const float b = p.bias_host ? p.bias_host[c] : 0.0f;
            if (p.bn_gamma_host) {
                const float s = p.bn_gamma_host[c] / sqrtf(p.bn_var_host[c] + bn_eps);
                sc[c] = s;
                sh[c] = (b - p.bn_mean_host[c]) * s + p.bn_beta_host[c];
            } else sh[c] = b;
        }
        L.scale_host = sc; L.shift_host = sh;
        if ((rc = upload(h, sc, &L.scale))) break;
        if ((rc = upload(h, sh, &L.shift))) break;
        if (k == EC0) {
            std::vector<float> wk = canonical_k3(p);
            rc = upload(h, wk, &L.plain);
        } else if (p.kind == 0 || p.kind == 1) {
            L.wk_host = canonical_k3(p);
            rc = upload(h, pack_conv3_panel(L.wk_host, L.c0, L.c1, p.cout, KC), &L.panel);
            if (!rc && KC == 8) rc = upload(h, pack_wino_f32_panel(L.wk_host, L.c0, L.c1, p.cout), &L.panel_wino_f32);
        } else if (p.kind == 2) {
            L.wk_host.assign(p.weight_host, p.weight_host + (size_t)p.cin * p.cout * 8);
            rc = upload(h, pack_up_panel(p), &L.panel);
        } else {
            std::vector<float> w(p.weight_host, p.weight_host + (size_t)p.cout * p.cin);
            L.plain_host = w;
            rc = upload(h, w, &L.plain);
        }
    }
    if (rc != OAI_OK) { oai_unet_destroy(h); return rc; }
    *out = h;
    return OAI_OK;
}

int oai_unet_set_precision(oai_unet* h, int mode) {
    OAI_CHECK_ARG(h, "oai_unet_set_precision: null handle");
    OAI_CHECK_ARG(mode >= OAI_PREC_F32 && mode <= OAI_PREC_FP16X3, "oai_unet_set_precision: unknown mode %d", mode);
    OAI_CHECK_ARG(mode == OAI_PREC_F32 || h->variant == 0, "oai_unet_set_precision: split modes need OAI_CONV_VARIANT=0");
    if (mode != OAI_PREC_F32) {
        const int slot = mode == OAI_PREC_BF16X3 ? 0 : mode == OAI_PREC_BF16X6 ? 1 : 2, NS = slot == 1 ? 3 : 2;
        for (int k = 1; k < 17; ++k) {
            Layer& L = h->L[k];
            if (slot == 2) {
                if (!L.panel_bf[2])
                    if (int rc = pack_fp16_layer(h, k)) return rc;
                continue;
            }
            if ((L.kind != 0 && L.kind != 1) || L.panel_bf[slot]) continue;
            if (int rc = upload(h, pack_conv3_panel_bf(L.wk_host, L.c0, L.c1, L.cout, NS), &L.panel_bf[slot])) return rc;
        }
        if (slot == 2 && !h->L[EC0].scale_f16)
            if (int rc = refresh_fp16_affine(h)) return rc;
    }
    h->precision = mode;
    h->sres = mode == OAI_PREC_FP16X3 && h->opt_sres;
    return OAI_OK;
}

struct IntOption { const char* name; int oai_unet::*field; int lo, hi; const char* message; };
static const IntOption kIntOptions[] = {
    {"shared_enc", &oai_unet::opt_shared, 0, 1, "oai_unet_set_option: shared_enc must be 0 or 1"},
    {"wide", &oai_unet::opt_wide, 0, 2, "oai_unet_set_option: wide must be 0, 1 or 2 (2 = also for launches of fewer than 1024 workgroups)"},
    {"winograd_layers", &oai_unet::opt_wino_layers, 0, 0x3FFFF, "oai_unet_set_option: winograd_layers is a mask over the 18 layers"},
    {"m16", &oai_unet::opt_m16, 0, 1, "oai_unet_set_option: m16 must be 0 or 1"},
    {"m16_layers", &oai_unet::opt_m16_layers, 0, 0x3FFFF, "oai_unet_set_option: m16_layers is a mask over the 18 layers"},
    {"dead_stores", &oai_unet::opt_dead_stores, 0, 1, "oai_unet_set_option: dead_stores must be 0 or 1"},
    {"winograd_f32", &oai_unet::opt_wino_f32, 0, 1, "oai_unet_set_option: winograd_f32 must be 0 or 1"},
    {"first_blocks", &oai_unet::opt_first_blocks, 1, 4096, "oai_unet_set_option: first_blocks must be in [1, 4096]"},
    {"up_nbw", &oai_unet::opt_up_nbw, 0, 64, "oai_unet_set_option: up_nbw must be in [0, 64]"},
    {"fuse_first", &oai_unet::fuse_first, 0, 1, "oai_unet_set_option: fuse_first must be 0 or 1"},
    {"xcd_group", &oai_unet::xcd_group, 0, 4096, "oai_unet_set_option: xcd_group must be in [0, 4096]"},
};

int oai_unet_set_option(oai_unet* h, const char* name, int value) {
    OAI_CHECK_ARG(h && name, "oai_unet_set_option: null pointer");
    for (const IntOption& o : kIntOptions)
        if (!strcmp(name, o.name)) {
            OAI_CHECK_ARG(value >= o.lo && value <= o.hi, "%s", o.message);
            h->*o.field = value;
            return OAI_OK;
        }
    if (!strcmp(name, "sres")) {
        OAI_CHECK_ARG(value == 0 || value == 1, "oai_unet_set_option: sres must be 0 or 1");
        h->opt_sres = value != 0;
        h->sres = h->precision == OAI_PREC_FP16X3 && h->opt_sres;
    } else if (!strcmp(name, "sres_mrep")) {
        OAI_CHECK_ARG(value == 2 || value == 4, "oai_unet_set_option: sres_mrep must be 2 or 4");
        h->sres_mrep = value;
    } else if (!strcmp(name, "winograd")) {
        OAI_CHECK_ARG(value >= 0 && value <= 63, "oai_unet_set_option: winograd must be in [0, 63]");
        if (value && !h->opt_wino && h->L[EC0].scale_f16) {
            OAI_CHECK_HIP(hipDeviceSynchronize());
            for (int k = 1; k < 17; ++k)
                if (h->L[k].panel_bf[2] && !h->L[k].panel_wino)
                    if (int rc = pack_wino_layer(h, k)) return rc;
        }
        h->opt_wino = value;
    } else if (!strcmp(name, "census")) {
        OAI_CHECK_ARG(value == 0 || value == 1, "oai_unet_set_option: census must be 0 or 1");
        OAI_CHECK_ARG(value == 1 || h->calibrated, "oai_unet_set_option: census 0 needs a calibrated handle (activation exponents set)");
        h->opt_census = value;
    } else if (!strcmp(name, "calibrated")) {
        OAI_CHECK_ARG(value == 0, "oai_unet_set_option: calibrated can only be cleared (0)");
        OAI_CHECK_ARG(h->opt_census == 1, "oai_unet_set_option: an uncalibrated handle needs the census (option census is 0)");
        h->calibrated = false;
    } else {
        return set_error(OAI_ERR_ARG, "oai_unet_set_option: unknown option '%s'", name);
    }
    return OAI_OK;
}

int oai_unet_range_flag(oai_unet* h, int reset, int* out, void* stream) {
    OAI_CHECK_ARG(h && out, "oai_unet_range_flag: null pointer");
    hipStream_t st = (hipStream_t)stream;
    range_eval_kernel<<<1, 64, 0, st>>>(h->range_flag, h->census, h->eval_out, reset, kLowRange);
    OAI_CHECK_LAUNCH();
    OAI_CHECK_HIP(hipMemcpyAsync(out, h->eval_out, sizeof(int), hipMemcpyDeviceToHost, st));
    OAI_CHECK_HIP(hipStreamSynchronize(st));
    return OAI_OK;
}

int oai_unet_range_flag_snapshot(oai_unet* h, int* dst_dev, void* stream) {
    OAI_CHECK_ARG(h && dst_dev, "oai_unet_range_flag_snapshot: null pointer");
    hipStream_t st = (hipStream_t)stream;
    range_eval_kernel<<<1, 64, 0, st>>>(h->range_flag, h->census, dst_dev, 1, kLowRange);
    OAI_CHECK_LAUNCH();
    return OAI_OK;
}

int oai_unet_range_state_snapshot(oai_unet* h, int* state_dev, void* stream) {
    OAI_CHECK_ARG(h && state_dev, "oai_unet_range_state_snapshot: null pointer");
    range_state_kernel<<<1, 64, 0, (hipStream_t)stream>>>(h->range_flag, h->census, state_dev);
    OAI_CHECK_LAUNCH();
    return OAI_OK;
}

int oai_unet_range_flag_from_state(const int* state_dev, int* flag_dev, void* stream) {
    OAI_CHECK_ARG(state_dev && flag_dev, "oai_unet_range_flag_from_state: null pointer");
    range_flag_from_state_kernel<<<1, 64, 0, (hipStream_t)stream>>>(state_dev, flag_dev, kLowRange);
    OAI_CHECK_LAUNCH();
    return OAI_OK;
}

int oai_unet_census(oai_unet* h, float max_out[OAI_UNET_NUM_LAYERS], int reset, void* stream) {
    OAI_CHECK_ARG(h && max_out, "oai_unet_census: null pointer");
    hipStream_t st = (hipStream_t)stream;
    unsigned host[18 * 16];
    OAI_CHECK_HIP(hipMemcpyAsync(host, h->census, sizeof(host), hipMemcpyDeviceToHost, st));
    OAI_CHECK_HIP(hipStreamSynchronize(st));
    for (int k = 0; k < 18; ++k) {
        unsigned m = 0;
        for (int i = 0; i < 16; ++i) m = host[k * 16 + i] > m ? host[k * 16 + i] : m;
        memcpy(&max_out[k], &m, 4);
    }
    if (reset) {
        OAI_CHECK_HIP(hipMemsetAsync(h->census, 0, sizeof(host), st));
        OAI_CHECK_HIP(hipMemsetAsync(h->range_flag, 0, sizeof(int), st));
    }
    return OAI_OK;
}

int oai_unet_get_act_exponents(const oai_unet* h, int e_out[OAI_UNET_NUM_LAYERS], int* calibrated) {
    OAI_CHECK_ARG(h && e_out, "oai_unet_get_act_exponents: null pointer");
    for (int k = 0; k < 18; ++k) e_out[k] = h->act_exp[k];
    if (calibrated) *calibrated = h->calibrated ? 1 : 0;
    return OAI_OK;
}

int oai_unet_set_act_exponents(oai_unet* h, const int e[OAI_UNET_NUM_LAYERS]) {
    OAI_CHECK_ARG(h && e, "oai_unet_set_act_exponents: null pointer");
    for (int k = 0; k < 17; ++k) OAI_CHECK_ARG(e[k] >= -100 && e[k] <= 100, "oai_unet_set_act_exponents: exponent %d of layer %d outside [-100, 100]", e[k], k);
    OAI_CHECK_ARG(e[DC0] == 0, "oai_unet_set_act_exponents: dc0 produces logits, its exponent must be 0");
    OAI_CHECK_HIP(hipDeviceSynchronize());
    for (int k = 0; k < 18; ++k) h->act_exp[k] = e[k];
    h->calibrated = true;
    if (!h->L[EC0].scale_f16) return OAI_OK;
    for (int k : {DC8, DC5, DC2}) {
        const int rel1 = h->act_exp[layer_src0(k)] - h->act_exp[layer_src1(k)];
        if (rel1 != h->L[k].rel1)
            if (int rc = pack_fp16_layer(h, k)) return rc;
    }
    return refresh_fp16_affine(h);
}

int oai_unet_calibrate_step(oai_unet* h, void* stream, int* more) {
    OAI_CHECK_ARG(h && more, "oai_unet_calibrate_step: null pointer");
    OAI_CHECK_ARG(h->precision == OAI_PREC_FP16X3, "oai_unet_calibrate_step: the activation exponents belong to OAI_PREC_FP16X3");
    float mx[18];
    if (int rc = oai_unet_census(h, mx, 1, stream)) return rc;
    int e[18], changed = 0, reported = 0;
    for (int k = 0; k < 18; ++k) e[k] = h->act_exp[k];
    for (int k = 0; k < 17; ++k) {
        if (!(mx[k] > 0.0f)) continue;
        ++reported;
        if (!std::isfinite(mx[k])) { e[k] = e[k] - 32 < -100 ? -100 : e[k] - 32; changed = 1; continue; }
        int b;
        frexpf(mx[k], &b);
        if (b - 1 >= kTargetExp - 1 && b - 1 <= kTargetExp + 1) continue;
        e[k] += kTargetExp - (b - 1);
        if (e[k] > 100) e[k] = 100;
        if (e[k] < -100) e[k] = -100;
        changed = 1;
    }
    *more = changed;
    if (!reported)
        return oai::set_error(OAI_ERR_ARG, "oai_unet_calibrate_step: the range census is empty (no fp16x3 pass since the last step, or option census / sres is 0)");
    if (!changed) { h->calibrated = true; return OAI_OK; }
    const bool was = h->calibrated;
    const int rc = oai_unet_set_act_exponents(h, e);
    h->calibrated = was;
    return rc;
}

int oai_unet_profile(oai_unet* h, int enable) {
    OAI_CHECK_ARG(h, "oai_unet_profile: null handle");
    h->profile = enable != 0;
    return OAI_OK;
}

int oai_unet_profile_read(oai_unet* h, double* conv3_ms, long long* conv3_launches) {
    OAI_CHECK_ARG(h && conv3_ms && conv3_launches, "oai_unet_profile_read: null pointer");
    double ms = 0.0;
    for (size_t i = 0; i + 1 < h->ev_used; i += 2) {
        OAI_CHECK_HIP(hipEventSynchronize(h->ev_pool[i + 1]));
        float t = 0.0f;
        OAI_CHECK_HIP(hipEventElapsedTime(&t, h->ev_pool[i], h->ev_pool[i + 1]));
        ms += t;
    }
    *conv3_ms = ms;
    *conv3_launches = (long long)(h->ev_used / 2);
    h->ev_used = 0;
    return OAI_OK;
}

double oai_unet_tile_flops_conv3(const oai_unet* h, int td, int th, int tw, const int overlap[3], int trimmed) {
    return tile_flops(h, td, th, tw, overlap, trimmed, true);
}

void oai_unet_destroy(oai_unet* h) {
    if (!h) return;
    for (hipEvent_t e : h->ev_pool) (void)hipEventDestroy(e);
    for (void* p : h->allocs) (void)hipFree(p);
    delete h;
}

size_t oai_unet_workspace_bytes(const oai_unet* h, int td, int th, int tw, int batch) {
    if (!h || td <= 0 || th <= 0 || tw <= 0 || batch <= 0) return 0;
    return workspace_bytes(h, td, th, tw, batch);
}

double oai_unet_tile_flops(const oai_unet* h, int td, int th, int tw, const int overlap[3], int trimmed) {
    return tile_flops(h, td, th, tw, overlap, trimmed, false);
}

static int check_tile(int td, int th, int tw) {
    OAI_CHECK_ARG(td >= 8 && th >= 8 && tw >= 8 && td % 8 == 0 && th % 8 == 0 && tw % 8 == 0,
                  "tile size %dx%dx%d must be a positive multiple of 8 per axis (three 2x poolings)", td, th, tw);
    return OAI_OK;
}

int oai_unet_forward_tiles(oai_unet* h, const float* tiles, float* logits, int B, int td, int th, int tw,
                           void* ws, size_t ws_bytes, void* stream) {
    OAI_CHECK_ARG(h && tiles && logits && ws, "oai_unet_forward_tiles: null pointer");
    OAI_CHECK_ARG(B > 0, "oai_unet_forward_tiles: B must be > 0");
    if (int rc = check_tile(td, th, tw)) return rc;
    int batch = B;
    while (batch > 1 && workspace_bytes(h, td, th, tw, batch) > ws_bytes) --batch;
    float* buf[B_COUNT];
    int* table;
    const size_t need_bytes = carve_workspace(h, td, th, tw, batch, ws, buf, table);
    if (need_bytes > ws_bytes)
        return set_error(OAI_ERR_WORKSPACE, "oai_unet_forward_tiles: workspace %zu B < %zu B needed for one tile", ws_bytes, need_bytes);
    const int tile[3] = {td, th, tw};
    const int lo[3] = {0, 0, 0};
    Box need[18];
    plan_regions(tile, lo, tile, false, need);
    TileSource src{};
    src.vol = nullptr; src.td = td; src.th = th; src.tw = tw;
    const size_t v0 = (size_t)td * th * tw;
    for (int s = 0; s < B; s += batch) {
        const int n = B - s < batch ? B - s : batch;
        src.tiles = tiles + (size_t)s * v0;
        src.tile_begin = 0;
        if (int rc = run_batch(h, src, n, need, 2, logits + (size_t)s * h->n_classes * v0, buf, (hipStream_t)stream)) return rc;
    }
    return OAI_OK;
}

__host__ __device__ static void keep_interval(int t, int eff, int ovl, int size, int crop, int& lo, int& hi) {
    const int v0 = t * eff;
    const int a = crop - v0 > 0 ? crop - v0 : 0;
    const int b = size - crop - v0 < eff ? size - crop - v0 : eff;
    lo = ovl + a;
    hi = ovl + b;
}

struct SegGeom {
    int eff[3], grid[3], ntiles;
};

static int seg_geometry(int D, int H, int W, const int tile[3], const int overlap[3], SegGeom& g) {
    const int size[3] = {D, H, W};
    for (int i = 0; i < 3; ++i) {
        OAI_CHECK_ARG(overlap[i] >= 0 && tile[i] - 2 * overlap[i] > 0, "overlap too large for the tile");
        g.eff[i] = tile[i] - 2 * overlap[i];
        g.grid[i] = (size[i] + g.eff[i] - 1) / g.eff[i];
    }
    g.ntiles = g.grid[0] * g.grid[1] * g.grid[2];
    return OAI_OK;
}

struct SegParams {
    int size[3], tile[3], overlap[3], crop[3], eff[3], grid[3];
    int trimmed;
};

__host__ __device__ static void tile_regions(int t, const SegParams& p, Box need[18]) {
    const int idx[3] = {t / (p.grid[1] * p.grid[2]), (t / p.grid[2]) % p.grid[1], t % p.grid[2]};
    int lo[3], hi[3];
    bool dead = false;
    for (int i = 0; i < 3; ++i) {
        keep_interval(idx[i], p.eff[i], p.overlap[i], p.size[i], p.crop[i], lo[i], hi[i]);
        if (hi[i] <= lo[i]) dead = true;
        if (!p.trimmed) { lo[i] = p.overlap[i]; hi[i] = p.tile[i] - p.overlap[i]; }
    }
    plan_regions(p.tile, lo, hi, p.trimmed != 0, need);
    if (dead && p.trimmed)
        for (int k = 0; k < 18; ++k) for (int i = 0; i < 3; ++i) need[k].lo[i] = need[k].hi[i] = 0;
}

__global__ void box_table_kernel(SegParams p, int t0, int n, int* __restrict__ table) {
    const int t = blockIdx.x * blockDim.x + threadIdx.x;
    if (t >= n) return;
    Box need[18];
    tile_regions(t0 + t, p, need);
    for (int k = 0; k < 18; ++k) {
        int* row = table + ((size_t)k * n + t) * 6;
        const bool up = layer_kind(k) == 2;
        for (int i = 0; i < 3; ++i) {
            row[i] = up ? need[k].lo[i] / 2 : need[k].lo[i];
            row[3 + i] = up ? (need[k].hi[i] + 1) / 2 : need[k].hi[i];
        }
    }
}

static SegParams seg_params(int D, int H, int W, const int tile[3], const int overlap[3], const int* crop, const SegGeom& g, bool trimmed) {
    SegParams p;
    const int size[3] = {D, H, W};
    for (int i = 0; i < 3; ++i) {
        p.size[i] = size[i]; p.tile[i] = tile[i]; p.overlap[i] = overlap[i]; p.crop[i] = crop ? crop[i] : 0;
        p.eff[i] = g.eff[i]; p.grid[i] = g.grid[i];
    }
    p.trimmed = trimmed ? 1 : 0;
    return p;
}

static size_t shared_enc_bytes(const oai_unet* h, const int tile[3], const int overlap[3], const SegGeom& g, int P[3]) {
    if (!first_fusion_ok(h) || !h->opt_shared || h->L[EC1].cout % 16 != 0) return 0;
    const int blk[3] = {4, 8, 16};
    for (int i = 0; i < 3; ++i) {
        P[i] = g.eff[i] * g.grid[i] + 2 * overlap[i];
        if (tile[i] % blk[i] || P[i] % blk[i] || g.eff[i] % blk[i] || overlap[i] < 4 || tile[i] < 8) return 0;
    }
    const size_t pv = (size_t)P[0] * P[1] * P[2];
    if (pv * 128 >= (1ull << 32)) return 0;
    const size_t nch = (size_t)h->L[EC1].cout / 16;
    return (nch * (pv / 8) * 64 + 255) / 256 * 256;
}

size_t oai_segment_workspace_bytes(const oai_unet* h, int D, int H, int W, const int tile[3], const int overlap[3], int batch) {
    if (!h || !tile || !overlap || batch <= 0) return 0;
    SegGeom g;
    if (seg_geometry(D, H, W, tile, overlap, g)) return 0;
    int P[3];
    return workspace_bytes(h, tile[0], tile[1], tile[2], batch) + shared_enc_bytes(h, tile, overlap, g, P);
}

int oai_segment_tiles(oai_unet* h, const float* vol, int D, int H, int W, const int tile[3], const int overlap[3],
                      const int crop[3], int tile_begin, int tile_end, int out_mode, float* blocks, int batch,
                      void* ws, size_t ws_bytes, void* stream) {
    OAI_CHECK_ARG(h && vol && tile && overlap && blocks && ws, "oai_segment_tiles: null pointer");
    OAI_CHECK_ARG(D > 1 && H > 1 && W > 1, "oai_segment_tiles: volume axes must be > 1 (reflect padding)");
    OAI_CHECK_ARG(out_mode >= 0 && out_mode <= 2, "oai_segment_tiles: out_mode must be 0, 1 or 2");
    if (int rc = check_tile(tile[0], tile[1], tile[2])) return rc;
    SegGeom g;
    if (int rc = seg_geometry(D, H, W, tile, overlap, g)) return rc;
    OAI_CHECK_ARG(0 <= tile_begin && tile_begin <= tile_end && tile_end <= g.ntiles,
                  "oai_segment_tiles: tile range [%d,%d) outside [0,%d)", tile_begin, tile_end, g.ntiles);
    OAI_CHECK_ARG(batch > 0, "oai_segment_tiles: batch must be > 0");
    if (crop) for (int i = 0; i < 3; ++i) OAI_CHECK_ARG(crop[i] >= 0, "oai_segment_tiles: negative crop");
    float* buf[B_COUNT];
    int* table_dev;
    const size_t need_bytes = carve_workspace(h, tile[0], tile[1], tile[2], batch, ws, buf, table_dev);
    if (need_bytes > ws_bytes)
        return set_error(OAI_ERR_WORKSPACE, "oai_segment_tiles: workspace %zu B < %zu B needed for batch %d", ws_bytes, need_bytes, batch);
    const bool trimmed = diag_env("OAI_NO_TRIM", 0) == 0;
    hipStream_t st = (hipStream_t)stream;
    TileSource src{};
    src.vol = vol; src.tiles = nullptr; src.D = D; src.H = H; src.W = W;
    src.td = tile[0]; src.th = tile[1]; src.tw = tile[2];
    src.ez = g.eff[0]; src.ey = g.eff[1]; src.ex = g.eff[2];
    src.oz = overlap[0]; src.oy = overlap[1]; src.ox = overlap[2];
    src.gy = g.grid[1]; src.gx = g.grid[2];
    const size_t bvox = (size_t)g.eff[0] * g.eff[1] * g.eff[2];
    const SegParams sp = seg_params(D, H, W, tile, overlap, crop, g, trimmed);
    Box need[18];
    SharedEnc se{};
    bool shared = false;
    if (trimmed && tile_end > tile_begin) {
        int P[3];
        const size_t sb = shared_enc_bytes(h, tile, overlap, g, P);
        if (sb && need_bytes + sb <= ws_bytes) {
            shared = true;
            se.SP0 = reinterpret_cast<float*>((char*)ws + need_bytes);
            se.PD = P[0]; se.PH = P[1]; se.PW = P[2];
            se.vol = vol; se.D = D; se.H = H; se.W = W;
            for (int i = 0; i < 3; ++i) { se.grid[i] = g.grid[i]; se.eff[i] = g.eff[i]; se.overlap[i] = overlap[i]; }
        }
    }
    for (int c0 = tile_begin; c0 < tile_end; c0 += kMaxTilesPerTable) {
        const int nc = tile_end - c0 < kMaxTilesPerTable ? tile_end - c0 : kMaxTilesPerTable;
        box_table_kernel<<<cdiv(nc, 64), 64, 0, st>>>(sp, c0, nc, table_dev);
        OAI_CHECK_LAUNCH();
        for (int t = c0; t < c0 + nc; t += batch) {
            const int n = c0 + nc - t < batch ? c0 + nc - t : batch;
            Box uni[18];
            for (int k = 0; k < 18; ++k) for (int i = 0; i < 3; ++i) { uni[k].lo[i] = 1 << 30; uni[k].hi[i] = 0; }
            for (int j = 0; j < n; ++j) {
                tile_regions(t + j, sp, need);
                for (int k = 0; k < 18; ++k) {
                    if (need[k].hi[0] <= need[k].lo[0]) continue;
                    for (int i = 0; i < 3; ++i) {
                        if (need[k].lo[i] < uni[k].lo[i]) uni[k].lo[i] = need[k].lo[i];
                        if (need[k].hi[i] > uni[k].hi[i]) uni[k].hi[i] = need[k].hi[i];
                    }
                }
            }
            if (uni[0].hi[0] == 0) continue;
            src.tile_begin = t;
            if (int rc = run_batch(h, src, n, uni, out_mode, blocks + (size_t)(t - tile_begin) * h->n_classes * bvox,
                                   buf, st, table_dev, nc, t - c0, shared ? &se : nullptr)) return rc;
        }
    }
    return OAI_OK;
}

double oai_unet_volume_flops(const oai_unet* h, int D, int H, int W, const int tile[3], const int overlap[3],
                             const int crop[3], int trimmed, int conv3_only) {
    if (!h || !tile || !overlap) return 0.0;
    SegGeom g;
    if (seg_geometry(D, H, W, tile, overlap, g)) return 0.0;
    double f = 0.0;
    Box need[18];
    const SegParams sp = seg_params(D, H, W, tile, overlap, crop, g, trimmed != 0);
    for (int t = 0; t < g.ntiles; ++t) {
        tile_regions(t, sp, need);
        for (int k = 0; k < 18; ++k) {
            if (conv3_only && !is_conv3_igemm(k)) continue;
            f += layer_flops(h, k, need[k]);
        }
    }
    return f;
}

int oai_unet_tile_costs(const oai_unet* h, int D, int H, int W, const int tile[3], const int overlap[3], const int crop[3],
                        double* costs_host, int n_tiles) {
    OAI_CHECK_ARG(h && tile && overlap && costs_host, "oai_unet_tile_costs: null pointer");
    SegGeom g;
    if (int rc = seg_geometry(D, H, W, tile, overlap, g)) return rc;
    OAI_CHECK_ARG(n_tiles == g.ntiles, "oai_unet_tile_costs: the volume has %d tiles, not %d", g.ntiles, n_tiles);
    Box need[18];
    const SegParams sp = seg_params(D, H, W, tile, overlap, crop, g, true);
    for (int t = 0; t < g.ntiles; ++t) {
        tile_regions(t, sp, need);
        double f = 0.0;
        for (int k = 0; k < 18; ++k) f += layer_flops(h, k, need[k]);
        costs_host[t] = f;
    }
    return OAI_OK;
}

int oai_stitch_blocks(const float* blocks, int ncls, int D, int H, int W, const int tile[3], const int overlap[3],
                      const int crop[3], float* maps, void* stream) {
    StitchRanges rg{};
    return stitch_impl(blocks, ncls, D, H, W, tile, overlap, crop, maps, stream, rg);
}

int oai_stitch_blocks_ranged(const float* blocks, int ncls, int D, int H, int W, const int tile[3], const int overlap[3],
                             const int crop[3], const int* bounds_host, int n_ranges, int slot_stride, float* maps, void* stream) {
    OAI_CHECK_ARG(bounds_host, "oai_stitch_blocks_ranged: null pointer");
    OAI_CHECK_ARG(n_ranges >= 1 && n_ranges <= 64, "oai_stitch_blocks_ranged: 1..64 ranges, got %d", n_ranges);
    StitchRanges rg{};
    rg.n = n_ranges; rg.stride = slot_stride;
    OAI_CHECK_ARG(bounds_host[0] == 0, "oai_stitch_blocks_ranged: the ranges must start at tile 0");
    for (int r = 0; r <= n_ranges; ++r) {
        rg.bound[r] = bounds_host[r];
        if (r) OAI_CHECK_ARG(bounds_host[r] >= bounds_host[r - 1] && bounds_host[r] - bounds_host[r - 1] <= slot_stride,
                             "oai_stitch_blocks_ranged: range %d is not ascending or longer than the slot stride %d", r - 1, slot_stride);
    }
    if (tile && overlap) {
        long long nt = 1;
        const int size[3] = {D, H, W};
        for (int i = 0; i < 3; ++i) { const int e = tile[i] - 2 * overlap[i]; if (e > 0) nt *= (size[i] + e - 1) / e; }
        OAI_CHECK_ARG(bounds_host[n_ranges] == nt, "oai_stitch_blocks_ranged: the ranges cover %d tiles, the volume has %lld", bounds_host[n_ranges], nt);
    }
    return stitch_impl(blocks, ncls, D, H, W, tile, overlap, crop, maps, stream, rg);
}

}

static int stitch_impl(const float* blocks, int ncls, int D, int H, int W, const int tile[3], const int overlap[3],
                       const int crop[3], float* maps, void* stream, const StitchRanges& rg) {
    OAI_CHECK_ARG(blocks && maps && tile && overlap, "oai_stitch_blocks: null pointer");
    int eff[3], grid[3];
    const int size[3] = {D, H, W};
    for (int i = 0; i < 3; ++i) {
        eff[i] = tile[i] - 2 * overlap[i];
        OAI_CHECK_ARG(eff[i] > 0, "oai_stitch_blocks: overlap too large for the tile");
        grid[i] = (size[i] + eff[i] - 1) / eff[i];
    }
    const size_t total = (size_t)ncls * D * H * W;
    if (crop && (crop[0] == 0 || crop[1] == 0 || crop[2] == 0)) {
        OAI_CHECK_HIP(hipMemsetAsync(maps, 0, total * sizeof(float), (hipStream_t)stream));
        return OAI_OK;
    }
    stitch_kernel<<<capped_blocks(total, 256 * 32), 256, 0, (hipStream_t)stream>>>(blocks, ncls, D, H, W, eff[0], eff[1], eff[2], grid[1], grid[2],
                                                                crop ? crop[0] : 0, crop ? crop[1] : 0, crop ? crop[2] : 0, maps, rg);
    OAI_CHECK_LAUNCH();
    return OAI_OK;
}
```

### oai_analysis_2_amd/csrc/unet_kernels.h

```cpp
#pragma once
#include <hip/hip_runtime.h>

namespace oai {

typedef float f32x16 __attribute__((ext_vector_type(16)));


struct TileSource {
    const float* vol;
    const float* tiles;
    int D, H, W;
    int td, th, tw;
    int ez, ey, ex;
    int oz, oy, ox;
    int gy, gx;
    int tile_begin;
};

__device__ __forceinline__ int reflect_index(int v, int n) {
    const int p = 2 * (n - 1);
    int m = v % p;
    if (m < 0) m += p;
    return m < n ? m : p - m;
}

struct ConvArgs {
    const float* src0; const float* src1;
    int C0, C1;
    float* out; int Cout;
    const float4* wpanel;
    const float4* wpanel16 = nullptr;
    const float* scale; const float* shift;
    int D, H, W;
    int lo[3], hi[3];
    int nbz, nby, nbx, ncb;
    int relu;
    const int* boxes;
    float* pool_out;
    int* range_flag;
    const int* store_boxes = nullptr;
    int store_grow = 0;
    const int* sc_boxes = nullptr;
    int sc_ntiles = 0, sc_tile0 = 0;
    int sc_g[3] = {0, 0, 0}, sc_e[3] = {0, 0, 0}, sc_t[3] = {0, 0, 0};
    unsigned* census = nullptr;
    unsigned* first_census = nullptr;
    int reserved0 = 0;
    unsigned long long* stamps = nullptr;
    int nblocks = 0, xcd_group = 0;
    int* reserved1 = nullptr;
    const float* head_w = nullptr;
    const float* head_b = nullptr;
    const int* head_boxes = nullptr;
    float* head_out = nullptr;
    int head_ncls = 0, head_mode = 0;
    int head_k[3] = {0, 0, 0}, head_e[3] = {0, 0, 0};
    const float* first_w = nullptr;
    const float* first_scale = nullptr; const float* first_shift = nullptr;
    TileSource first_src = {};
};

__device__ __forceinline__ int xcd_block_id(int nblocks, int G) {
    const int xcd = (int)blockIdx.x & 7, j = (int)blockIdx.x >> 3;
    const int id = ((j / G) * 8 + xcd) * G + j % G;
    return id < nblocks ? id : -1;
}

__device__ __forceinline__ bool tile_box(const int* boxes, int tile, const int (&llo)[3], const int (&lhi)[3],
                                         int (&lo)[3], int (&hi)[3]) {
#pragma unroll
    for (int i = 0; i < 3; ++i) { lo[i] = llo[i]; hi[i] = lhi[i]; }
    if (boxes) {
        const int* b = boxes + 6 * tile;
#pragma unroll
        for (int i = 0; i < 3; ++i) { lo[i] = max(lo[i], b[i]); hi[i] = min(hi[i], b[3 + i]); }
    }
    return lo[0] < hi[0] && lo[1] < hi[1] && lo[2] < hi[2];
}


template <int MREP, typename F>
__device__ __forceinline__ void pooled_store(const ConvArgs& a, int tile, int co, int oz0, int oy, int ox0, int half, F&& value) {
    const int Dp = a.D / 2, Hp = a.H / 2, Wp = a.W / 2;
#pragma unroll
    for (int m = 0; m < MREP; m += 2)
#pragma unroll
        for (int g = 0; g < 2; ++g)
#pragma unroll
            for (int p = 0; p < 2; ++p) {
                const int r0 = 4 * g + 2 * p;
                float v = fmaxf(fmaxf(value(m, r0), value(m, r0 + 1)), fmaxf(value(m, r0 + 8), value(m, r0 + 9)));
                v = fmaxf(v, fmaxf(fmaxf(value(m + 1, r0), value(m + 1, r0 + 1)), fmaxf(value(m + 1, r0 + 8), value(m + 1, r0 + 9))));
                const int x = ox0 + 8 * g + 4 * half + 2 * p;
                a.pool_out[((((size_t)tile * Dp + (oz0 + m) / 2) * Hp + oy / 2) * Wp + x / 2) * a.Cout + co] = v;
            }
}

template <int MREP, int KC, int RX, int RY, int WY, int WX>
__global__ void __launch_bounds__(256, 2) conv3_igemm_f32(const ConvArgs a) {
    static_assert(RX * RY == 32 && WY * WX == 4, "bad tile shape");
    constexpr int kConvTY = WY * RY, kConvTX = WX * RX, kConvHY = kConvTY + 2, kConvHX = kConvTX + 2;
    constexpr int NREP = 2;
    constexpr int TZ = MREP, HZ = TZ + 2;
    constexpr int STRIDE = KC + 4;
    constexpr int HVOX = HZ * kConvHY * kConvHX;
    constexpr int Q = KC / 4;
    constexpr int KG = KC / 8;
    constexpr int NSLOT = (HVOX * Q + 255) / 256;
    constexpr int NSTEP = 27 * KG;
    __shared__ __attribute__((aligned(16))) float lds[HVOX * STRIDE];

    const int tid = threadIdx.x, lane = tid & 63, wave = tid >> 6;
    int id = blockIdx.x;
    const int cb = id % a.ncb; id /= a.ncb;
    const int bx = id % a.nbx; id /= a.nbx;
    const int by = id % a.nby; id /= a.nby;
    const int bz = id % a.nbz; id /= a.nbz;
    const int tile = id;
    const int oz0 = a.lo[0] + bz * TZ, oy0 = a.lo[1] + by * kConvTY, ox0 = a.lo[2] + bx * kConvTX;
    int blo[3], bhi[3];
    if (!tile_box(a.boxes, tile, a.lo, a.hi, blo, bhi)) return;
    if (oz0 >= bhi[0] || oz0 + TZ <= blo[0] || oy0 >= bhi[1] || oy0 + kConvTY <= blo[1] || ox0 >= bhi[2] || ox0 + kConvTX <= blo[2]) return;
    const int m_lo = max(0, blo[0] - oz0), m_hi = min(MREP, bhi[0] - oz0);

    f32x16 acc[MREP][NREP], part[MREP][NREP];
#pragma unroll
    for (int m = 0; m < MREP; ++m)
#pragma unroll
        for (int n = 0; n < NREP; ++n)
#pragma unroll
            for (int r = 0; r < 16; ++r) { acc[m][n][r] = 0.0f; part[m][n][r] = 0.0f; }

    const int row = lane & 31, half = lane >> 5;
    const int wy = wave / WX, wx = wave % WX;
    const int lx = wx * RX + row % RX, ly = wy * RY + row / RX;
    const float* a_ptr = &lds[(ly * kConvHX + lx) * STRIDE + 4 * half];

    const int nch0 = (a.C0 + KC - 1) / KC, nch1 = (a.C1 + KC - 1) / KC;
    const int nchunks = nch0 + nch1;
    const float4* wp = a.wpanel + (size_t)cb * nchunks * NSTEP * NREP * 64 + lane;
    const size_t plane = (size_t)a.D * a.H * a.W;

    float4 hreg[NSLOT];
    auto halo_load = [&](int ch) {
        const bool first = ch < nch0;
        const float* src = first ? a.src0 : a.src1;
        const int C = first ? a.C0 : a.C1;
        const int c0 = (first ? ch : ch - nch0) * KC;
        const float* sbase = src + (size_t)tile * plane * C + c0;
#pragma unroll
        for (int i = 0; i < NSLOT; ++i) {
            const int slot = tid + i * 256;
            const int hv = slot / Q, q = slot - hv * Q;
            const int hx = hv % kConvHX;
            const int t2 = hv / kConvHX;
            const int hy = t2 % kConvHY, hz = t2 / kConvHY;
            const int gz = oz0 - 1 + hz, gy = oy0 - 1 + hy, gx = ox0 - 1 + hx;
            float4 v = make_float4(0.f, 0.f, 0.f, 0.f);
            if (slot < HVOX * Q && (unsigned)gz < (unsigned)a.D && (unsigned)gy < (unsigned)a.H &&
                (unsigned)gx < (unsigned)a.W && c0 + 4 * q < C)
                v = *reinterpret_cast<const float4*>(sbase + (((size_t)gz * a.H + gy) * a.W + gx) * C + 4 * q);
            hreg[i] = v;
        }
    };
    auto halo_store = [&]() {
#pragma unroll
        for (int i = 0; i < NSLOT; ++i) {
            const int slot = tid + i * 256;
            const int hv = slot / Q, q = slot - hv * Q;
            if (slot < HVOX * Q) *reinterpret_cast<float4*>(&lds[hv * STRIDE + 4 * q]) = hreg[i];
        }
    };

    float4 bcur[NREP], bnext[NREP];
#pragma unroll
    for (int n = 0; n < NREP; ++n) bcur[n] = wp[n * 64];
    wp += NREP * 64;
    halo_load(0);

    for (int ch = 0; ch < nchunks; ++ch) {
        __syncthreads();
        halo_store();
        __syncthreads();
        if (ch + 1 < nchunks) halo_load(ch + 1);
#pragma unroll
        for (int st = 0; st < NSTEP; ++st) {
            const int t = st / KG, kg = st % KG;
            const int dz = t / 9, dy = (t / 3) % 3, dx = t % 3;
            float4 acur[MREP];
#pragma unroll
            for (int m = 0; m < MREP; ++m)
                acur[m] = *reinterpret_cast<const float4*>(
                    a_ptr + (((m + dz) * kConvHY + dy) * kConvHX + dx) * STRIDE + 8 * kg);
#pragma unroll
            for (int n = 0; n < NREP; ++n) bnext[n] = wp[n * 64];
            wp += NREP * 64;
            __builtin_amdgcn_sched_barrier(0);
#pragma unroll
            for (int s = 0; s < 4; ++s) {
#pragma unroll
// ... 114 lines not shown
    for (int m = 0; m < MREP; ++m)
#pragma unroll
        for (int n = 0; n < NREP; ++n)
#pragma unroll
            for (int r = 0; r < 16; ++r) acc[m][n][r] = 0.0f;

    const int row = lane & 31, half = lane >> 5;
    const int wy = wave / WX, wx = wave % WX;
    const int lx = wx * RX + row % RX, ly = wy * RY + row / RX;
    const unsigned char* a_ptr = &lds[(ly * HX + lx) * REC + 16 * half];

    const int nch0 = (a.C0 + KC - 1) / KC, nch1 = (a.C1 + KC - 1) / KC;
    const int nchunks = nch0 + nch1;
    constexpr int STEP = NS * NREP * 64;
    const float4* wp = a.wpanel + (size_t)cb * nchunks * 27 * STEP + lane;
    const size_t plane = (size_t)a.D * a.H * a.W;

    float4 hreg[NSLOT];
    auto halo_load = [&](int ch) {
        const bool first = ch < nch0;
        const float* src = first ? a.src0 : a.src1;
        const int C = first ? a.C0 : a.C1;
        const int c0 = (first ? ch : ch - nch0) * KC;
        const float* sbase = src + (size_t)tile * plane * C + c0;
#pragma unroll
        for (int i = 0; i < NSLOT; ++i) {
            const int slot = tid + i * 256;
            const int hv = slot / Q, q = slot - hv * Q;
            const int hx = hv % HX;
            const int t2 = hv / HX;
            const int hy = t2 % HY, hz = t2 / HY;
            const int gz = oz0 - 1 + hz, gy = oy0 - 1 + hy, gx = ox0 - 1 + hx;
            float4 v = make_float4(0.f, 0.f, 0.f, 0.f);
            if (slot < HVOX * Q && (unsigned)gz < (unsigned)a.D && (unsigned)gy < (unsigned)a.H &&
                (unsigned)gx < (unsigned)a.W && c0 + 4 * q < C)
                v = *reinterpret_cast<const float4*>(sbase + (((size_t)gz * a.H + gy) * a.W + gx) * C + 4 * q);
            hreg[i] = v;
        }
    };
    auto halo_store = [&]() {
#pragma unroll
        for (int i = 0; i < NSLOT; ++i) {
            const int slot = tid + i * 256;
            const int hv = slot / Q, q = slot - hv * Q;
            if (slot < HVOX * Q) {
                u16x4 t[NS];
                if constexpr (FP16) {
                    const float4 v = hreg[i];
                    if (!(fmaxf(fmaxf(fabsf(v.x), fabsf(v.y)), fmaxf(fabsf(v.z), fabsf(v.w))) <= 65504.0f)) atomicOr(a.range_flag, 1);
                }
                split_terms<NS, FP16>(hreg[i], t);
#pragma unroll
                for (int k = 0; k < NS; ++k) *reinterpret_cast<u16x4*>(&lds[hv * REC + k * 32 + q * 8]) = t[k];
            }
        }
    };

    float4 bcur[NS][NREP], bnext[NS][NREP];
#pragma unroll
    for (int k = 0; k < NS; ++k)
#pragma unroll
        for (int n = 0; n < NREP; ++n) bcur[k][n] = wp[(k * NREP + n) * 64];
    wp += STEP;
    halo_load(0);

    for (int ch = 0; ch < nchunks; ++ch) {
        __syncthreads();
        halo_store();
        __syncthreads();
        if (ch + 1 < nchunks) halo_load(ch + 1);
#pragma unroll
        for (int t = 0; t < 27; ++t) {
            const int dz = t / 9, dy = (t / 3) % 3, dx = t % 3;
            float4 acur[NS][MREP];
#pragma unroll
            for (int k = 0; k < NS; ++k)
#pragma unroll
                for (int m = 0; m < MREP; ++m)
                    acur[k][m] = *reinterpret_cast<const float4*>(a_ptr + (((m + dz) * HY + dy) * HX + dx) * REC + k * 32);
#pragma unroll
            for (int k = 0; k < NS; ++k)
#pragma unroll
                for (int n = 0; n < NREP; ++n) bnext[k][n] = wp[(k * NREP + n) * 64];
            wp += STEP;
            __builtin_amdgcn_sched_barrier(0);
#pragma unroll
            for (int p = 0; p < NPASS; ++p) {
#pragma unroll
                for (int m = 0; m < MREP; ++m) {
                    if (m >= m_lo && m < m_hi) {
#pragma unroll
                        for (int n = 0; n < NREP; ++n)
                            acc[m][n] = mfma_16bit<FP16>(acur[PA[p]][m], bcur[PB[p]][n], acc[m][n]);
                    }
                }
            }
            __builtin_amdgcn_sched_barrier(0);
#pragma unroll
            for (int k = 0; k < NS; ++k)
#pragma unroll
                for (int n = 0; n < NREP; ++n) bcur[k][n] = bnext[k][n];
        }
    }

#pragma unroll
    for (int n = 0; n < NREP; ++n) {
        const int co = cb * 64 + n * 32 + row;
        if (co >= a.Cout) continue;
        float sc = a.scale[co], sh = a.shift[co];
        asm volatile("" : "+v"(sc), "+v"(sh));
#pragma unroll
        for (int m = 0; m < MREP; ++m) {
            const int oz = oz0 + m;
            if (oz < blo[0] || oz >= bhi[0]) continue;
#pragma unroll
            for (int r = 0; r < 16; ++r) {
                const int rr = (r & 3) + 8 * (r >> 2) + 4 * half;
                const int ox = ox0 + wx * RX + rr % RX, oy = oy0 + wy * RY + rr / RX;
                if (ox >= blo[2] && ox < bhi[2] && oy >= blo[1] && oy < bhi[1]) {
                    float v = acc[m][n][r] * sc + sh;
                    if (a.relu) v = fmaxf(v, 0.0f);
                    a.out[((size_t)tile * plane + ((size_t)oz * a.H + oy) * a.W + ox) * a.Cout + co] = v;
                }
            }
        }
        if constexpr (RX == 16 && RY == 2 && WY == 4 && WX == 1 && MREP % 2 == 0) {
            if (a.pool_out) {
                const bool relu = a.relu != 0;
                pooled_store<MREP>(a, tile, co, oz0, oy0 + 2 * wy, ox0, half, [&](int m, int r) {
                    const float v = acc[m][n][r] * sc + sh;
                    return relu ? fmaxf(v, 0.0f) : v;
                });
            }
        }
    }
}


struct UpArgs {
    const float* src; int Cin;
    float* out; int Cout;
    const float4* wpanel;
    const float* scale; const float* shift;
    int D, H, W;
    int lo[3], hi[3];
    int nmb;
    int nnb;
    int relu;
    const int* boxes;
    int* range_flag;
    unsigned* census = nullptr;
    const unsigned char* zero = nullptr;
    unsigned long long* stamps = nullptr;
    int reserved0 = 0;
    int nblocks = 0, xcd_group = 0;
    int nbw = 1;
};

template <bool SPLIT>
__global__ void __launch_bounds__(256, 2) upconv2_igemm(const UpArgs a) {
    const int tid = threadIdx.x, lane = tid & 63, wave = tid >> 6;
    int id = blockIdx.x;
    const int nb = id % a.nnb; id /= a.nnb;
    const int mb = id % a.nmb; id /= a.nmb;
    const int tile = id;
    const int N = 8 * a.Cout;
    const int ncol0 = nb * 256 + wave * 64;
    if (ncol0 >= N) return;
    const int row = lane & 31, half = lane >> 5;
    const int rz = a.hi[0] - a.lo[0], ry = a.hi[1] - a.lo[1], rx = a.hi[2] - a.lo[2];
    const int nvox = rz * ry * rx;
    int blo[3], bhi[3];
    if (!tile_box(a.boxes, tile, a.lo, a.hi, blo, bhi)) return;
    {
        const int zf = a.lo[0] + (mb * 64) / (rx * ry), zl = a.lo[0] + min(mb * 64 + 63, nvox - 1) / (rx * ry);
        if (zl < blo[0] || zf >= bhi[0]) return;
    }
    const size_t plane = (size_t)a.D * a.H * a.W;

    const float* ap[2];
    bool av[2];
#pragma unroll
    for (int m = 0; m < 2; ++m) {
        const int v = mb * 64 + m * 32 + row;
        av[m] = v < nvox;
        const int vv = av[m] ? v : 0;
        const int x = vv % rx, y = (vv / rx) % ry, z = vv / (rx * ry);
        ap[m] = a.src + ((size_t)tile * plane + ((size_t)(a.lo[0] + z) * a.H + (a.lo[1] + y)) * a.W + (a.lo[2] + x)) * a.Cin + 4 * half;
    }
    f32x16 acc[2][2];
#pragma unroll
    for (int m = 0; m < 2; ++m)
#pragma unroll
        for (int n = 0; n < 2; ++n)
#pragma unroll
            for (int r = 0; r < 16; ++r) acc[m][n][r] = 0.0f;

  if constexpr (!SPLIT) {
    const int nkg = (a.Cin + 7) / 8;
    const float4* wp = a.wpanel + (size_t)(ncol0 / 64) * nkg * 2 * 64 + lane;
    auto load_a = [&](int kg, float4 (&af)[2]) {
#pragma unroll
        for (int m = 0; m < 2; ++m)
            af[m] = (av[m] && kg * 8 + 4 * half < a.Cin) ? *reinterpret_cast<const float4*>(ap[m] + kg * 8)
                                                         : make_float4(0.f, 0.f, 0.f, 0.f);
    };
    float4 af[2], bf[2], afn[2], bfn[2];
    load_a(0, af);
#pragma unroll
    for (int n = 0; n < 2; ++n) bf[n] = wp[n * 64];
    for (int kg = 0; kg < nkg; ++kg) {
        load_a(kg + 1 < nkg ? kg + 1 : kg, afn);
#pragma unroll
        for (int n = 0; n < 2; ++n) bfn[n] = wp[((kg + 1 < nkg ? kg + 1 : kg) * 2 + n) * 64];
        __builtin_amdgcn_sched_barrier(0);
#pragma unroll
        for (int s = 0; s < 4; ++s)
#pragma unroll
            for (int m = 0; m < 2; ++m) {
                const float x = s == 0 ? af[m].x : s == 1 ? af[m].y : s == 2 ? af[m].z : af[m].w;
#pragma unroll
                for (int n = 0; n < 2; ++n) {
                    const float y = s == 0 ? bf[n].x : s == 1 ? bf[n].y : s == 2 ? bf[n].z : bf[n].w;
                    acc[m][n] = __builtin_amdgcn_mfma_f32_32x32x2f32(x, y, acc[m][n], 0, 0, 0);
                }
            }
        __builtin_amdgcn_sched_barrier(0);
#pragma unroll
        for (int m = 0; m < 2; ++m) af[m] = afn[m];
#pragma unroll
        for (int n = 0; n < 2; ++n) bf[n] = bfn[n];
    }
  } else {
    const int nks = (a.Cin + 15) / 16;
    const float4* wp = a.wpanel + (size_t)(ncol0 / 64) * nks * 4 * 64 + lane;
    auto load_a = [&](int ks, float4 (&raw)[2][2]) {
#pragma unroll
        for (int m = 0; m < 2; ++m)
#pragma unroll
            for (int q = 0; q < 2; ++q) {
                const int c = ks * 16 + 8 * half + 4 * q;
                raw[m][q] = (av[m] && c < a.Cin) ? *reinterpret_cast<const float4*>(ap[m] - 4 * half + c)
                                                 : make_float4(0.f, 0.f, 0.f, 0.f);
            }
    };
    float4 raw[2][2], rawn[2][2], bf[2][2], bfn[2][2];
    load_a(0, raw);
#pragma unroll
    for (int k = 0; k < 2; ++k)
#pragma unroll
        for (int n = 0; n < 2; ++n) bf[k][n] = wp[(k * 2 + n) * 64];
    constexpr int PA[3] = {0, 0, 1}, PB[3] = {0, 1, 0};
    for (int ks = 0; ks < nks; ++ks) {
        const int nx = ks + 1 < nks ? ks + 1 : ks;
        load_a(nx, rawn);
#pragma unroll
        for (int k = 0; k < 2; ++k)
#pragma unroll
            for (int n = 0; n < 2; ++n) bfn[k][n] = wp[((size_t)nx * 4 + k * 2 + n) * 64];
        float4 at[2][2];
#pragma unroll
        for (int m = 0; m < 2; ++m) {
            u16x4 lo4[2], hi4[2];
            split_terms<2, true>(raw[m][0], lo4);
            split_terms<2, true>(raw[m][1], hi4);
            if (!(fmaxf(fmaxf(fabsf(raw[m][0].x), fabsf(raw[m][0].y)), fmaxf(fabsf(raw[m][0].z), fabsf(raw[m][0].w))) <= 65504.0f) ||
                !(fmaxf(fmaxf(fabsf(raw[m][1].x), fabsf(raw[m][1].y)), fmaxf(fabsf(raw[m][1].z), fabsf(raw[m][1].w))) <= 65504.0f))
                atomicOr(a.range_flag, 1);
#pragma unroll
            for (int k = 0; k < 2; ++k) {
                typedef unsigned short u16x8 __attribute__((ext_vector_type(8)));
                u16x8 v;
#pragma unroll
                for (int j = 0; j < 4; ++j) { v[j] = lo4[k][j]; v[4 + j] = hi4[k][j]; }
                at[k][m] = __builtin_bit_cast(float4, v);
            }
        }
        __builtin_amdgcn_sched_barrier(0);
#pragma unroll
        for (int p = 0; p < 3; ++p)
#pragma unroll
            for (int m = 0; m < 2; ++m)
#pragma unroll
                for (int n = 0; n < 2; ++n) acc[m][n] = mfma_16bit<true>(at[PA[p]][m], bf[PB[p]][n], acc[m][n]);
        __builtin_amdgcn_sched_barrier(0);
#pragma unroll
        for (int m = 0; m < 2; ++m)
#pragma unroll
            for (int q = 0; q < 2; ++q) raw[m][q] = rawn[m][q];
#pragma unroll
        for (int k = 0; k < 2; ++k)
#pragma unroll
            for (int n = 0; n < 2; ++n) bf[k][n] = bfn[k][n];
    }
  }
    const int Ho = 2 * a.H, Wo = 2 * a.W;
    int vx[2][4], vy[2][4], vz[2][4];
#pragma unroll
    for (int m = 0; m < 2; ++m)
#pragma unroll
        for (int g = 0; g < 4; ++g) {
            const int v = mb * 64 + m * 32 + 8 * g + 4 * half;
            vx[m][g] = v % rx;
            const int t = v / rx;
            vy[m][g] = t % ry;
            vz[m][g] = t / ry;
        }
// ... 204 lines not shown
```

### oai_analysis_2_amd/csrc/unet_sres.h

```cpp
#pragma once
#include <hip/hip_runtime.h>

#include <type_traits>

#include "unet_kernels.h"

namespace oai {

typedef unsigned short u16x8 __attribute__((ext_vector_type(8)));

__device__ __forceinline__ unsigned split2_f16(float x, unsigned& lo_bits) {
    const _Float16 h = (_Float16)x;
    const _Float16 l = (_Float16)(x - (float)h);
    lo_bits = __builtin_bit_cast(unsigned short, l);
    return __builtin_bit_cast(unsigned short, h);
}

__device__ __forceinline__ float join2_f16(unsigned short hi, unsigned short lo) {
    return (float)__builtin_bit_cast(_Float16, hi) + (float)__builtin_bit_cast(_Float16, lo);
}

__device__ __forceinline__ unsigned census_peek(const unsigned* census) {
    typedef const __attribute__((address_space(4))) unsigned* cuptr;
    return census ? *((cuptr)census + (blockIdx.x & 15)) : 0u;
// ... 633 lines not shown
                        }
                    }
            }
        } else if (FIRST && a.sc_boxes) {
            static_assert(!FIRST || kTX == 16, "lane split of the scatter copy-out");
            const int t5 = tid >> 3, q = tid & 7;
            const int x_lane = t5 % kTX, y_lane = t5 / kTX;
            const bool cok = cb * 4 + n * 2 + (q >> 2) < nco;
            const size_t tplane = (size_t)a.sc_t[0] * a.sc_t[1] * a.sc_t[2];
            for (int iz = oz0 / a.sc_e[0]; iz >= 0 && oz0 - iz * a.sc_e[0] < a.sc_t[0]; --iz) {
                if (iz >= a.sc_g[0]) continue;
                for (int iy = oy0 / a.sc_e[1]; iy >= 0 && oy0 - iy * a.sc_e[1] < a.sc_t[1]; --iy) {
                    if (iy >= a.sc_g[1]) continue;
                    for (int ix = ox0 / a.sc_e[2]; ix >= 0 && ox0 - ix * a.sc_e[2] < a.sc_t[2]; --ix) {
                        if (ix >= a.sc_g[2]) continue;
                        const int t = (iz * a.sc_g[1] + iy) * a.sc_g[2] + ix - a.sc_tile0;
                        if (t < 0 || t >= a.sc_ntiles) continue;
                        const int lz0 = oz0 - iz * a.sc_e[0], ly0 = oy0 - iy * a.sc_e[1], lx0 = ox0 - ix * a.sc_e[2];
                        typedef const __attribute__((address_space(4))) int* ciptr;
                        const ciptr sb = (ciptr)(a.sc_boxes + 6 * t);
                        const int s0z = sb[0] - 1, s0y = sb[1] - 1, s0x = sb[2] - 1, s1z = sb[3] + 1, s1y = sb[4] + 1, s1x = sb[5] + 1;
                        if (sb[3] <= sb[0] || lz0 >= s1z || lz0 + TZ <= s0z || ly0 >= s1y || ly0 + kTY <= s0y || lx0 >= s1x || lx0 + kTX <= s0x) continue;
                        unsigned char* ob = outb + ((size_t)t * nco + cb * 4 + n * 2) * tplane * 64;
                        const long long lane_off = (long long)(((size_t)(q >> 2) * tplane + (size_t)y_lane * a.sc_t[2] + x_lane) * 64 + (q & 3) * 16);
#pragma unroll
                        for (int it = 0; it < EIT; ++it) {
                            const int c = (it & 3) * 32, zc = it >> 2, yc = c / kTX;
                            const int lz = lz0 + zc, ly = ly0 + y_lane + yc, lx = lx0 + x_lane;
                            if (cok && lz >= s0z && lz < s1z && ly >= s0y && ly < s1y && lx >= s0x && lx < s1x &&
                                (unsigned)lz < (unsigned)a.sc_t[0] && (unsigned)ly < (unsigned)a.sc_t[1] && (unsigned)lx < (unsigned)a.sc_t[2]) {
                                const long long uni = ((long long)(lz * a.sc_t[1] + ly0 + yc) * a.sc_t[2] + lx0) * 64;
                                float4* dstp = reinterpret_cast<float4*>(ob + (lane_off + uni));
                                const float4 val = *reinterpret_cast<const float4*>(lds + (it * 256 + tid) * 16);
                                __builtin_nontemporal_store(val.x, &dstp->x); __builtin_nontemporal_store(val.y, &dstp->y);
                                __builtin_nontemporal_store(val.z, &dstp->z); __builtin_nontemporal_store(val.w, &dstp->w);
                            }
                        }
                    }
                }
            }
        } else {
            static_assert(kTX * kTY == 128, "the index split below");
            constexpr bool kWide = kTX >= 32;
            const int t5 = tid >> 3, q = tid & 7;
            const int x_lane = kWide ? t5 : t5 % kTX, y_lane = kWide ? 0 : t5 / kTX;
            const bool cok = cb * 4 + n * 2 + (q >> 2) < nco;
            unsigned char* ob = outb + ((size_t)tile * nco + cb * 4 + n * 2) * plane * 64;
            const unsigned lane_off = (unsigned)(((size_t)(q >> 2) * plane + (size_t)y_lane * a.W + x_lane) * 64 + (q & 3) * 16);
            const int oyl = oy0 + y_lane, oxl = ox0 + x_lane;
#pragma unroll
            for (int it = 0; it < EIT; ++it) {
                constexpr int kDummy = 0; (void)kDummy;
                const int c = (it & 3) * 32, zc = it >> 2;
                const int xc = kWide ? c % kTX : 0, yc = c / kTX;
                const int oz = oz0 + zc, oy = oyl + yc, ox = oxl + xc;
                if (cok && oz >= clo[0] && oz < chi[0] && oy >= clo[1] && oy < chi[1] && ox >= clo[2] && ox < chi[2]) {
                    const unsigned uni = (unsigned)(((oz * a.H + oy0 + yc) * a.W + ox0 + xc) * 64);
                    float4* dstp = reinterpret_cast<float4*>(ob + (size_t)(lane_off + uni));
                    const float4 val = *reinterpret_cast<const float4*>(lds + (it * 256 + tid) * 16);
                    __builtin_nontemporal_store(val.x, &dstp->x); __builtin_nontemporal_store(val.y, &dstp->y);
                    __builtin_nontemporal_store(val.z, &dstp->z); __builtin_nontemporal_store(val.w, &dstp->w);
                }
            }
        }
        OAI_STAMPB(head ? 4 : 3);
        if constexpr (RX == 16 && RY == 2 && WY == 4 && WX == 1) {
            if (a.pool_out) {
                unsigned char* pb = reinterpret_cast<unsigned char*>(a.pool_out);
                const int Dp = a.D / 2, Hp = a.H / 2, Wp = a.W / 2;
                const bool relu = a.relu != 0;
                auto val = [&](int m, int r) {
                    const float v = acc_el(m, n, r) * scv[n][M16 ? (r >> 2) & 1 : 0] + shv[n][M16 ? (r >> 2) & 1 : 0];
                    return relu ? fmaxf(v, 0.0f) : v;
                };
#pragma unroll
                for (int g = 0; g < 2; ++g)
#pragma unroll
                    for (int p = 0; p < 2; ++p) {
                        const int r0 = 4 * g + 2 * p;
#pragma unroll
                        for (int m = 0; m < MREP; m += 2) {
                            float v = fmaxf(fmaxf(val(m, r0), val(m, r0 + 1)), fmaxf(val(m, r0 + 8), val(m, r0 + 9)));
                            v = fmaxf(v, fmaxf(fmaxf(val(m + 1, r0), val(m + 1, r0 + 1)), fmaxf(val(m + 1, r0 + 8), val(m + 1, r0 + 9))));
                            const int x = M16 ? ox0 + 4 * rq16 + 2 * p : ox0 + 8 * g + 4 * half + 2 * p, y = oy0 + 2 * wy, z = oz0 + m;
                            const int pco = M16 ? cb * 64 + n * 32 + 16 * g + col16 : co;
                            store_split_pair(pb + srec(tile, nco, (size_t)Dp * Hp * Wp, 0, (((size_t)(z / 2)) * Hp + y / 2) * Wp + x / 2), (size_t)Dp * Hp * Wp * 64,
                                             pco, v, M16 ? (g ? cvalid1 : cvalid) : cvalid, a.range_flag);
                        }
                    }
            }
        }
    }
    OAI_STAMPB(5);
    if (head) {
        int hlo[3], hhi[3];
        tile_box(a.head_boxes, tile, blo, bhi, hlo, hhi);
        const size_t evox = (size_t)a.head_e[0] * a.head_e[1] * a.head_e[2];
#pragma unroll
        for (int j = 0; j < HV; ++j) {
            const int vox = j * 256 + tid;
            const int oz = oz0 + vox / (kTX * kTY), oy = oy0 + (vox / kTX) % kTY, ox = ox0 + vox % kTX;
            if (oz >= hlo[0] && oz < hhi[0] && oy >= hlo[1] && oy < hhi[1] && ox >= hlo[2] && ox < hhi[2]) {
                const size_t o = ((size_t)(oz - a.head_k[0]) * a.head_e[1] + (oy - a.head_k[1])) * a.head_e[2] + (ox - a.head_k[2]);
#pragma unroll
                for (int k = 0; k < 4; ++k)
                    if (k < a.head_ncls) {
                        const float l = hacc[j][k] + head_b[k];
                        float r = l;
                        if (a.head_mode != 2) {
                            const float pr = 1.0f / (1.0f + expf(-l));
                            r = a.head_mode == 1 ? (pr > 0.5f ? 1.0f : 0.0f) : pr;
                        }
                        a.head_out[((size_t)tile * a.head_ncls + k) * evox + o] = r;
                    }
            }
        }
    }
    if constexpr (FIRST) census_note(a.first_census, a.range_flag, first_max, seen_first);
    census_note(a.census, a.range_flag, vmax, seen);
#ifdef OAI_DIAG
    OAI_STAMP(6);
    OAI_STAMPB(6);
    if (a.stamps && lane == 0) {
        for (int i = 0; i < 8; ++i) atomicAdd(a.stamps + i, (unsigned long long)st_sum[i]);
        atomicAdd(a.stamps + 8, 1ull);
        atomicAdd(a.stamps + 9, (unsigned long long)st_chunks);
    }
#endif
#undef OAI_STAMP
#undef OAI_STAMPB
#undef OAI_STAMP_
}

__global__ void __launch_bounds__(256, 2) upconv2_igemm_sres(const UpArgs a) {
#ifdef OAI_DIAG
    unsigned ust[5] = {0, 0, 0, 0, 0};
    unsigned long long ulast = __builtin_amdgcn_s_memtime();
#define OAI_USTAMP(i) do { if (a.stamps) { const unsigned long long now_ = __builtin_amdgcn_s_memtime(); ust[i] += (unsigned)(now_ - ulast); ulast = now_; } } while (0)
#else
#define OAI_USTAMP(i) do { } while (0)
#endif
    constexpr int kStage = 24 * 1024, kRing = 3 * kStage;
    __shared__ __attribute__((aligned(16))) unsigned char ulds[kRing + 512];
    const int tid = threadIdx.x, lane = tid & 63, wave = tid >> 6;
    const int wm = wave >> 1, wn = wave & 1;
    int id = a.xcd_group ? xcd_block_id(a.nblocks, a.xcd_group) : (int)blockIdx.x;
    if (id < 0) return;
    const int nbw = a.nbw > 0 ? a.nbw : 1, nnbg = (a.nnb + nbw - 1) / nbw;
    const int nbg = id % nnbg; id /= nnbg;
    const int mb = id % a.nmb; id /= a.nmb;
    const int tile = id;
    const int N = 8 * a.Cout;
    const int row = lane & 31, half = lane >> 5;
    const int rz = a.hi[0] - a.lo[0], ry = a.hi[1] - a.lo[1], rx = a.hi[2] - a.lo[2];
    const int nvox = rz * ry * rx;
    int blo[3], bhi[3];
    if (!tile_box(a.boxes, tile, a.lo, a.hi, blo, bhi)) return;
    {
        const int zf = a.lo[0] + (mb * 128) / (rx * ry), zl = a.lo[0] + min(mb * 128 + 127, nvox - 1) / (rx * ry);
        if (zl < blo[0] || zf >= bhi[0]) return;
    }
    const size_t plane = (size_t)a.D * a.H * a.W;
    const int nks = (a.Cin + 15) / 16;
    const int Ho = 2 * a.H, Wo = 2 * a.W;
    const int nco = (a.Cout + 15) / 16;
    unsigned* vtab = reinterpret_cast<unsigned*>(ulds + kRing);
    if (tid < 128) {
        const int v = mb * 128 + tid;
        unsigned e = ~0u;
        if (v < nvox) {
            const int x = v % rx, t = v / rx, y = t % ry, z = t / ry;
            const int iz = a.lo[0] + z, iy = a.lo[1] + y, ix = a.lo[2] + x;
            if (iz >= blo[0] && iz < bhi[0] && iy >= blo[1] && iy < bhi[1] && ix >= blo[2] && ix < bhi[2])
                e = (unsigned)(((2 * iz) * Ho + 2 * iy) * Wo + 2 * ix);
        }
        vtab[tid] = e;
    }
    const unsigned char* asrc[2];
#pragma unroll
    for (int it = 0; it < 2; ++it) {
        const int p = it * 256 + tid, vl = p >> 2, v = mb * 128 + vl;
        if (v < nvox) {
            const int x = v % rx, y = (v / rx) % ry, z = v / (rx * ry);
            asrc[it] = reinterpret_cast<const unsigned char*>(a.src) +
                       srec(tile, nks, plane, 0, ((size_t)(a.lo[0] + z) * a.H + (a.lo[1] + y)) * a.W + (a.lo[2] + x)) + (((p & 3) ^ ((vl >> 2) & 3)) << 4);
        } else asrc[it] = nullptr;
    }
    unsigned char* outb = reinterpret_cast<unsigned char*>(a.out) + srec(tile, nco, 8 * plane, 0, 0);
    const unsigned seen = census_peek(a.census);
    unsigned umax = 0;
    f32x16 acc[2][4];
    bool looped = true;
    int nb = nbg * nbw, ncol0 = nb * 256 + wn * 128;
    for (int nbi = 0; nbi < nbw && nb < a.nnb; ++nbi, ++nb) {
    ncol0 = nb * 256 + wn * 128;
    if (nbi > 0) __syncthreads();
    const int ngroups = (N + 63) / 64;
    const unsigned char* bsrc[4];
#pragma unroll
    for (int g = 0; g < 4; ++g)
        bsrc[g] = nb * 4 + g < ngroups ? reinterpret_cast<const unsigned char*>(a.wpanel + (size_t)(nb * 4 + g) * nks * 4 * 64) + tid * 16 : nullptr;
    const unsigned ring_addr = lds_addr_of(ulds);
    auto issue = [&](int st, int ks) {
        const unsigned base = __builtin_amdgcn_readfirstlane(ring_addr + st * kStage + wave * 1024);
#pragma unroll
        for (int it = 0; it < 2; ++it)
            lds_dma16(asrc[it] ? asrc[it] + (size_t)ks * plane * 64 : a.zero, base + it * 4096);
#pragma unroll
        for (int g = 0; g < 4; ++g)
            lds_dma16(bsrc[g] ? bsrc[g] + (size_t)ks * 4096 : a.zero, base + 8192 + g * 4096);
    };
#pragma unroll
    for (int m = 0; m < 2; ++m)
#pragma unroll
        for (int n = 0; n < 4; ++n)
#pragma unroll
            for (int r = 0; r < 16; ++r) acc[m][n][r] = 0.0f;
    const bool active = ncol0 < N;
    int aoff[2][2];
#pragma unroll
    for (int m = 0; m < 2; ++m) {
        const int vl = wm * 64 + m * 32 + row;
#pragma unroll
        for (int k = 0; k < 2; ++k) aoff[k][m] = vl * 64 + (((k * 2 + half) ^ ((vl >> 2) & 3)) << 4);
    }
    const int boff = 8192 + wn * 8192 + lane * 16;
    OAI_USTAMP(0);
    issue(0, 0);
    if (nks > 1) issue(1, 1);
    constexpr int PA[3] = {0, 0, 1}, PB[3] = {0, 1, 0};
    for (int ks = 0; ks < nks; ++ks) {
        if (ks + 1 < nks) asm volatile("s_waitcnt vmcnt(6) lgkmcnt(0)" ::: "memory");
        else asm volatile("s_waitcnt vmcnt(0) lgkmcnt(0)" ::: "memory");
        __builtin_amdgcn_s_barrier();
        asm volatile("" ::: "memory");
        if (ks + 2 < nks) issue((ks + 2) % 3, ks + 2);
        if (active) {
            const unsigned char* sp = ulds + (ks % 3) * kStage;
            float4 at[2][2], bf[2][4];
#pragma unroll
            for (int k = 0; k < 2; ++k)
#pragma unroll
                for (int m = 0; m < 2; ++m) at[k][m] = *reinterpret_cast<const float4*>(sp + aoff[k][m]);
#pragma unroll
            for (int k = 0; k < 2; ++k)
#pragma unroll
                for (int n = 0; n < 4; ++n) bf[k][n] = *reinterpret_cast<const float4*>(sp + boff + (n >> 1) * 4096 + (k * 2 + (n & 1)) * 1024);
#pragma unroll
            for (int p = 0; p < 3; ++p)
#pragma unroll
                for (int m = 0; m < 2; ++m)
#pragma unroll
                    for (int n = 0; n < 4; ++n) acc[m][n] = mfma_16bit<true>(at[PA[p]][m], bf[PB[p]][n], acc[m][n]);
        }
    }
    OAI_USTAMP(1);
    if (a.Cout % 16 == 0) {
        const int q = tid & 63;
        const int cg = nb * 256 + (q >> 2) * 16;
        const bool qok = cg < N;
        const int par = qok ? cg / a.Cout : 0, cchunk = qok ? (cg - par * a.Cout) >> 4 : 0;
        const unsigned poff = (unsigned)(((par >> 2) * Ho + ((par >> 1) & 1)) * Wo + (par & 1));
        const size_t inrow = (size_t)cchunk * 8 * plane * 64 + (q & 3) * 16;
        float scn[4], shn[4];
#pragma unroll
        for (int n = 0; n < 4; ++n) {
            const int col = ncol0 + n * 32 + row;
            const bool cok = col < N;
            const int co = cok ? col % a.Cout : 0;
            scn[n] = cok ? a.scale[co] : 0.0f; shn[n] = cok ? a.shift[co] : 0.0f;
        }
        asm volatile("" : "+v"(scn[0]), "+v"(scn[1]), "+v"(scn[2]), "+v"(scn[3]), "+v"(shn[0]), "+v"(shn[1]), "+v"(shn[2]), "+v"(shn[3]));
#pragma unroll
        for (int m = 0; m < 2; ++m) {
            __syncthreads();
            OAI_USTAMP(2);
            if (active) {
                unsigned vmask = 0;
#pragma unroll
                for (int r = 0; r < 16; ++r)
                    vmask |= (vtab[wm * 64 + m * 32 + (r & 3) + 8 * (r >> 2) + 4 * half] != ~0u ? 1u : 0u) << r;
                const bool odd = row & 1;
                const unsigned sel = odd ? 0x03020706u : 0x05040100u;
#pragma unroll
                for (int n = 0; n < 4; ++n) {
                    const int col = ncol0 + n * 32 + row;
                    const float sc = scn[n], sh = shn[n];
                    unsigned om = col < N ? vmask : 0u;
                    asm volatile("" : "+v"(om));
                    unsigned char* lrow = ulds + ((wn * 128 + n * 32 + row) >> 4) * 64 + ((row & 15) >> 1) * 4 + (wm * 32 + 4 * half + (odd ? 1 : 0)) * 1024;
#pragma unroll
                    for (int r = 0; r < 16; r += 2) {
                        float v[2];
#pragma unroll
                        for (int e = 0; e < 2; ++e) {
                            const float x = fmaxf(acc[m][n][r + e] * sc + sh, 0.0f);
                            unsigned keep;
                            asm("v_bfe_i32 %0, %1, %2, 1" : "=v"(keep) : "v"(om), "n"(r + e));
                            v[e] = __builtin_bit_cast(float, __builtin_bit_cast(unsigned, x) & keep);
                        }
                        umax = max(umax, max(__builtin_bit_cast(unsigned, v[0]), __builtin_bit_cast(unsigned, v[1])));
                        unsigned w_hi, w_lo;
                        split_two_voxels(v[0], v[1], sel, w_hi, w_lo);
                        const int vl = (r & 3) + 8 * (r >> 2);
                        *reinterpret_cast<unsigned*>(lrow + vl * 1024) = w_hi;
                        *reinterpret_cast<unsigned*>(lrow + vl * 1024 + 32) = w_lo;
                    }
                }
            }
            OAI_USTAMP(3);
            __syncthreads();
            OAI_USTAMP(2);
#pragma unroll 4
            for (int it = 0; it < 16; ++it) {
                const int vl = it * 4 + (tid >> 6);
                const unsigned e = vtab[(vl >> 5) * 64 + m * 32 + (vl & 31)];
                if (qok && e != ~0u)
                    *reinterpret_cast<float4*>(outb + (size_t)(e + poff) * 64 + inrow) = *reinterpret_cast<const float4*>(ulds + vl * 1024 + q * 16);
            }
            OAI_USTAMP(4);
        }
        continue;
    }
    looped = false;
    break;
    }
    if (looped) {
        census_note(a.census, a.range_flag, __builtin_bit_cast(float, umax), seen);
#ifdef OAI_DIAG
        OAI_USTAMP(4);
        if (a.stamps && lane == 0) {
            for (int i = 0; i < 5; ++i) atomicAdd(a.stamps + 16 + i, (unsigned long long)ust[i]);
            atomicAdd(a.stamps + 24, 1ull);
        }
#endif
        return;
    }
    const bool active = ncol0 < N;
// ... 271 lines not shown
```

### oai_analysis_2_amd/csrc/unet_wino.h

```cpp
#pragma once
#include "unet_sres2.h"
namespace oai {

template <int NG, int TY, int NP, int MS = 1, bool WS = false, bool M16 = false>
__global__ void __launch_bounds__(WS ? 512 : 256 * NG * MS, 1) conv3_wino_sres(const ConvArgs a, const unsigned char* __restrict__ zero_rec) {
    constexpr int NT = 256 * NG * MS, MREP = 4 / MS, NREP = 2;
    static_assert((MS == 1 || MS == 2) && NG * MS <= 2, "eight waves at most");
    static_assert(!M16 || MS == 1 || (NG == 1 && !WS), "the 16x16x32 taps: the four-slice forms (two groups, or specialised waves) and the slice-split 64-cout form");
    static_assert(!WS || (NG == 1 && MS == 1), "specialised waves: four multiply, four stage");
    constexpr int TZ = 4, TX = 2 * NP, HZ = TZ + 2, HY = TY + 2, HX = TX + 2;
    constexpr int RS = 4 * HX + 1;
    constexpr int PIECES = HZ * HY * RS;
    constexpr int NIT = (PIECES + NT - 1) / NT;
    constexpr int TB = HZ * 4 * HY * NP * 64;
    constexpr int RPW = HZ * HY / 4, WNIT = (RPW * RS + 63) / 64;
    constexpr int RAWB = WS ? 4 * WNIT * 1024 : NIT * NT * 16;
    constexpr int UNITS = HZ * 2 * HY * NP;
    constexpr int XB = 3 * 4 * 4 * 1024;
    static_assert(NG == 1 || NG == 2, "one or two cout groups");
    static_assert(TY * NP == 32 && (NP == 2 || NP == 4 || NP == 8), "32 rows per accumulator tile");
    constexpr int NTB = WS ? 2 : 1;
    static_assert(!WS || (HZ * HY) % 4 == 0, "whole halo rows per staging wave");
    static_assert(NTB * TB + RAWB <= 160 * 1024 && NG * MS * XB <= TB + RAWB && TZ * TY * TX * 128 <= XB && TZ * TY * TX * 256 <= TB + RAWB, "epilogue buffers live in the idle T / raw space");
    __shared__ __attribute__((aligned(16))) unsigned char lds[NTB * TB + RAWB];
    unsigned char* const Tl = lds;
    unsigned char* const raw = lds + NTB * TB;

    const int tid = threadIdx.x, lane = tid & 63, wave = tid >> 6;
#ifdef OAI_DIAG
    unsigned long long wst[4] = {__builtin_amdgcn_s_memrealtime(), 0, 0, 0}, wep[3] = {0, 0, 0}, wlast = 0;
#define OAI_WSTAMP(i) do { if (a.stamps) wst[i] = __builtin_amdgcn_s_memrealtime(); } while (0)
#define OAI_WEP0() do { if (a.stamps) wlast = __builtin_amdgcn_s_memrealtime(); } while (0)
#define OAI_WEP(i) do { if (a.stamps) { const unsigned long long now_ = __builtin_amdgcn_s_memrealtime(); wep[i] += now_ - wlast; wlast = now_; } } while (0)
#else
#define OAI_WSTAMP(i) do { } while (0)
#define OAI_WEP0() do { } while (0)
#define OAI_WEP(i) do { } while (0)
#endif
    const int grp = (MS == 2 || WS) ? 0 : wave >> 2, zp = MS == 2 ? wave >> 2 : 0, f = wave & 3, gtid = tid & 255;
    const bool stager = WS && __builtin_amdgcn_readfirstlane(wave) >= 4;
    const int nch0 = (a.C0 + 15) / 16, nch1 = (a.C1 + 15) / 16, nchunks = nch0 + nch1;
    const size_t plane = (size_t)a.D * a.H * a.W;
    int tile, cb, oz0, oy0, ox0, m_lo, m_hi;
    int blo[3], bhi[3];
    const unsigned char *s0, *s1;
    auto set_block = [&](int tile_, int bz, int by, int bx, int cbg) __attribute__((always_inline)) -> bool {
        tile = tile_;
        cb = cbg * NG + grp;
        oz0 = a.lo[0] + bz * TZ; oy0 = a.lo[1] + by * TY; ox0 = a.lo[2] + bx * TX;
        if (!tile_box(a.boxes, tile, a.lo, a.hi, blo, bhi)) return false;
        if (oz0 >= bhi[0] || oz0 + TZ <= blo[0] || oy0 >= bhi[1] || oy0 + TY <= blo[1] || ox0 >= bhi[2] || ox0 + TX <= blo[2]) return false;
        m_lo = max(0, blo[0] - oz0); m_hi = min(TZ, bhi[0] - oz0);
        s0 = reinterpret_cast<const unsigned char*>(a.src0) + srec(tile, nch0, plane, 0, 0);
        s1 = reinterpret_cast<const unsigned char*>(a.src1) + srec(tile, nch1, plane, 0, 0);
        return true;
    };
    {
        int id = a.xcd_group ? xcd_block_id(a.nblocks, a.xcd_group) : (int)blockIdx.x;
        if (id < 0) return;
        const int cbg = id % a.ncb; id /= a.ncb;
        const int bx = id % a.nbx; id /= a.nbx;
        const int by = id % a.nby; id /= a.nby;
        const int bz = id % a.nbz; id /= a.nbz;
        if (!set_block(id, bz, by, bx, cbg)) return;
    }

    const int row = lane & 31, half = lane >> 5;

    f32x16 acc[M16 ? 1 : MREP][M16 ? 1 : NREP];
    f32x4 acc4[M16 ? MREP : 1][M16 ? NREP : 1][4];
#pragma unroll
    for (int m = 0; m < (M16 ? 1 : MREP); ++m)
#pragma unroll
        for (int n = 0; n < (M16 ? 1 : NREP); ++n)
#pragma unroll
            for (int r = 0; r < 16; ++r) acc[m][n][r] = 0.0f;
#pragma unroll
    for (int m = 0; m < (M16 ? MREP : 1); ++m)
#pragma unroll
        for (int n = 0; n < (M16 ? NREP : 1); ++n)
#pragma unroll
            for (int t = 0; t < 4; ++t) acc4[m][n][t] = f32x4{0.0f, 0.0f, 0.0f, 0.0f};
    auto acc_el = [&](int m, int n, int r) __attribute__((always_inline)) -> float {
        if constexpr (M16) return acc4[m][n][r >> 2][r & 3];
        else return acc[m][n][r];
    };

    constexpr unsigned kNoPiece = 0xFFFFFFFFu;
    unsigned poff[NIT];
#pragma unroll
    for (int it = 0; it < (WS ? 0 : NIT); ++it) {
        const int L = it * NT + tid;
        const int rw = L / RS, c = L - rw * RS;
        const int hz = rw / HY, hy = rw - hz * HY;
        const int term = c / (2 * HX), hx = (c - term * 2 * HX) >> 1, hf = c & 1;
        const int gz = oz0 - 1 + hz, gy = oy0 - 1 + hy, gx = ox0 - 1 + hx;
        const bool ok = L < PIECES && c < 4 * HX && (unsigned)gz < (unsigned)a.D && (unsigned)gy < (unsigned)a.H && (unsigned)gx < (unsigned)a.W;
        poff[it] = ok ? ((unsigned)((gz * a.H + gy) * a.W + gx) << 6) | (unsigned)(term * 32 + hf * 16) : kNoPiece;
    }
    const unsigned raw0 = lds_addr_of(raw);
    auto issue_piece = [&](int it, int ch) __attribute__((always_inline)) {
        const bool real = ch < nchunks;
        const bool first = ch < nch0;
        const unsigned char* cbase = (first ? s0 : s1) + (size_t)(first ? ch : ch - nch0) * plane * 64;
        const unsigned char* g = (real && poff[it] != kNoPiece) ? cbase + poff[it] : zero_rec;
        lds_dma16(g, __builtin_amdgcn_readfirstlane(raw0 + (it * NT + wave * 64) * 16));
    };
    auto issue_piece_s = [&](int it, int ch) __attribute__((always_inline)) {
        const int che = ch < nchunks ? ch : nchunks - 1;
        const bool first = che < nch0;
        const unsigned char* cbase = (first ? s0 : s1) + (size_t)(first ? che : che - nch0) * plane * 64;
        const unsigned off = poff[it] != kNoPiece ? poff[it] : 0u;
        unsigned keep;
        asm volatile("s_mov_b32 %0, m0\n\ts_mov_b32 m0, %3\n\ts_nop 0\n\tglobal_load_lds_dwordx4 %1, %2\n\ts_mov_b32 m0, %0"
                     : "=&s"(keep) : "v"(off), "s"(cbase), "s"(__builtin_amdgcn_readfirstlane(raw0 + (it * NT + wave * 64) * 16)) : "memory");
    };
    unsigned miss = 0;
    if constexpr (M16 && !WS) {
#pragma unroll
        for (int it = 0; it < NIT; ++it) miss |= poff[it] == kNoPiece ? 1u << it : 0u;
    }
    auto zero_missing = [&]() __attribute__((always_inline)) {
        if (__builtin_amdgcn_ballot_w64(miss != 0) == 0) return;
#pragma unroll
        for (int it = 0; it < NIT; ++it)
            if (miss & (1u << it)) *reinterpret_cast<float4*>(raw + (it * NT + tid) * 16) = float4{0.0f, 0.0f, 0.0f, 0.0f};
    };
    auto pieces_in_tap = [](int t) constexpr { return WS ? 0 : NIT / 9 + (t < NIT % 9 ? 1 : 0); };
    auto first_piece = [](int t) constexpr { return t * (NIT / 9) + (t < NIT % 9 ? t : NIT % 9); };
    static_assert(NIT <= 18, "at most two pieces per tap (vm_wait<0..2>)");

    auto transform_unit = [&](const unsigned char* rb, int hz, int hy, int p, int hf, unsigned char* Tdst) __attribute__((always_inline)) {
        float x[4][8];
#pragma unroll
        for (int i = 0; i < 4; ++i) {
            const u16x8 h0 = *reinterpret_cast<const u16x8*>(rb + (2 * i) * 16);
            const u16x8 h1 = *reinterpret_cast<const u16x8*>(rb + (2 * HX + 2 * i) * 16);
#pragma unroll
            for (int c = 0; c < 8; ++c) x[i][c] = join2_f16(h0[c], h1[c]);
        }
        unsigned char* tw = Tdst + (((hz * 4) * HY + hy) * NP + p) * 64;
        const int key = ((hy * NP + p) >> 2) & 3;
        const int sl0 = ((hf) ^ key) * 16, sl1 = ((2 + hf) ^ key) * 16;
#pragma unroll
        for (int fq = 0; fq < 4; ++fq) {
            u16x8 hi, lo;
#pragma unroll
            for (int c = 0; c < 8; c += 2) {
                f32x2 v;
#pragma unroll
                for (int e = 0; e < 2; ++e)
                    v[e] = fq == 0 ? x[0][c + e] - x[2][c + e] : fq == 1 ? x[1][c + e] + x[2][c + e] : fq == 2 ? x[2][c + e] - x[1][c + e] : x[1][c + e] - x[3][c + e];
                const f16x2 h = __builtin_convertvector(v, f16x2);
                const f32x2 res = v - __builtin_convertvector(h, f32x2);
                const f16x2 l = __builtin_convertvector(res, f16x2);
                const unsigned H = __builtin_bit_cast(unsigned, h), Lw = __builtin_bit_cast(unsigned, l);
                hi[c] = (unsigned short)H; hi[c + 1] = (unsigned short)(H >> 16);
                lo[c] = (unsigned short)Lw; lo[c + 1] = (unsigned short)(Lw >> 16);
            }
            *reinterpret_cast<u16x8*>(tw + fq * (HY * NP * 64) + sl0) = hi;
            *reinterpret_cast<u16x8*>(tw + fq * (HY * NP * 64) + sl1) = lo;
        }
    };
    auto transform = [&]() __attribute__((always_inline)) {
        int tq = tid;
        if constexpr (M16) asm volatile("" : "+v"(tq));
#pragma unroll
        for (int ui = 0; ui < (UNITS + NT - 1) / NT; ++ui) {
            const int u = ui * NT + tq;
            if (u < UNITS) {
                const int p = u % NP;
                int t = u / NP;
                const int hy = t % HY; t /= HY;
                const int hf = t & 1, hz = t >> 1;
                transform_unit(raw + (((hz * HY + hy) * RS) + 4 * p + hf) * 16, hz, hy, p, hf, Tl);
            }
        }
    };
    const int sw = wave & 3;
    unsigned char* const raw_w = raw + sw * (WNIT * 1024);
    unsigned woff[WS ? WNIT : 1];
    auto stage_plan = [&](unsigned (&wo)[WS ? WNIT : 1], int z0, int y0, int x0) __attribute__((always_inline)) {
#pragma unroll
        for (int it = 0; it < (WS ? WNIT : 0); ++it) {
            const int q = it * 64 + lane;
            const int rj = q / RS, c = q - rj * RS;
            const int r = sw + 4 * rj, hz = r / HY, hy = r - hz * HY;
            const int term = c / (2 * HX), hx = (c - term * 2 * HX) >> 1, hf = c & 1;
            const int gz = z0 - 1 + hz, gy = y0 - 1 + hy, gx = x0 - 1 + hx;
            const bool ok = rj < RPW && c < 4 * HX && (unsigned)gz < (unsigned)a.D && (unsigned)gy < (unsigned)a.H && (unsigned)gx < (unsigned)a.W;
            wo[WS ? it : 0] = ok ? ((unsigned)((gz * a.H + gy) * a.W + gx) << 6) | (unsigned)(term * 32 + hf * 16) : kNoPiece;
        }
    };
    if constexpr (WS) stage_plan(woff, oz0, oy0, ox0);
    auto stage_request_of = [&](const unsigned (&wo)[WS ? WNIT : 1], const unsigned char* b0, const unsigned char* b1, int ch) __attribute__((always_inline)) {
        const bool first = ch < nch0;
        const unsigned char* cbase = (first ? b0 : b1) + (size_t)(first ? ch : ch - nch0) * plane * 64;
        const unsigned dst = lds_addr_of(raw_w);
#pragma unroll
        for (int it = 0; it < (WS ? WNIT : 0); ++it) {
            const unsigned char* g = (wo[WS ? it : 0] != kNoPiece) ? cbase + wo[WS ? it : 0] : zero_rec;
            lds_dma16(g, __builtin_amdgcn_readfirstlane(dst + it * 1024));
        }
// ... 746 lines not shown
```

Measured before the change: 7.511.

## Cover each tile's own box in decoder Winograd and up-conv launches

Decoder Winograd conv layers and up-convolutions now cover each tile's own needed box. They no longer use the union box over the batch, so block origins are taken from the per-tile box and block counts from a per-layer maximum. The aim is to cut launched blocks that exit early or do partial work when tiles in a batch have different regions. It also picks the XCD grouping per launch by simulating block load per XCD, adds extra table rows, and adds a host stats entry point. The cost is host-side planning work on every batch and more complex indexing.

```diff
diff --git a/include/oai_hip.h b/include/oai_hip.h
--- a/include/oai_hip.h
+++ b/include/oai_hip.h
@@ -123,6 +123,8 @@
                              const int crop_zyx[3], int trimmed, int conv3_only);
 int oai_unet_tile_costs(const oai_unet* h, int D, int H, int W, const int tile_zyx[3], const int overlap_zyx[3],
                         const int crop_zyx[3], double* costs_host, int n_tiles);
+int oai_unet_cover_stats(int D, int H, int W, const int tile_zyx[3], const int overlap_zyx[3], const int crop_zyx[3], int batch, int layer,
+                         double stats_host[3], int* pieces_host, int n_tiles);
 double oai_unet_tile_flops_conv3(const oai_unet* h, int td, int th, int tw, const int overlap_zyx[3], int trimmed);
 
 
diff --git a/oai_analysis_2_amd/_lib.py b/oai_analysis_2_amd/_lib.py
--- a/oai_analysis_2_amd/_lib.py
+++ b/oai_analysis_2_amd/_lib.py
@@ -51,6 +51,7 @@
     "oai_resample_maps_through_phi": (_I, [_P, _I, _I, _I, _I, _P, _I, _I, _I, C.POINTER(Affine), C.POINTER(Affine),
                                            _P, _I, _I, _I, _P]),
     "oai_unet_tile_costs": (_I, [_P, _I, _I, _I, C.POINTER(C.c_int), C.POINTER(C.c_int), C.POINTER(C.c_int), C.POINTER(C.c_double), _I]),
+    "oai_unet_cover_stats": (_I, [_I, _I, _I, C.POINTER(C.c_int), C.POINTER(C.c_int), C.POINTER(C.c_int), _I, _I, C.POINTER(C.c_double), C.POINTER(C.c_int), _I]),
     "oai_mc_table": (_I, [_P]),
     "oai_mc_workspace_bytes": (_Z, [_I, _I, _I]),
     "oai_mc_count": (_I, [_P, _I, _I, _I, _F, _P, _Z, C.POINTER(C.c_longlong), C.POINTER(C.c_longlong), _P]),
diff --git a/oai_analysis_2_amd/csrc/unet.hip b/oai_analysis_2_amd/csrc/unet.hip
--- a/oai_analysis_2_amd/csrc/unet.hip
+++ b/oai_analysis_2_amd/csrc/unet.hip
@@ -2,6 +2,7 @@
 #include <cstdint>
 #include <cstdlib>
 #include <cstring>
+#include <algorithm>
 #include <vector>
 
 #include "common.h"
@@ -57,6 +58,7 @@
     int opt_wino_f32 = 1;
     int opt_first_blocks = 24;
     int opt_up_nbw = 0;
+    int opt_own_cover = 1;
     int opt_shared = 1;
     int opt_wide = 1;
     int opt_wino = 19;
@@ -492,6 +494,8 @@
 }
 
 constexpr int kMaxTilesPerTable = 4096;
+constexpr int kOwnLayers = 5, kTableRows = 18 + 3 * kOwnLayers;
+__host__ __device__ static inline int own_cover_slot(int k) { return k == DC8 ? 0 : k == DC7 ? 1 : k == DC5 ? 2 : k == DC4 ? 3 : k == DC2 ? 4 : -1; }
 enum Buf { B_E0, B_SYN0, B_P0, B_E2, B_SYN1, B_P1, B_E4, B_SYN2, B_P2, B_E6, B_E7, B_U9, B_D8, B_D7, B_U6, B_D5, B_D4, B_U3, B_D2, B_D1, B_COUNT };
 
 static size_t carve_workspace(const oai_unet* h, int td, int th, int tw, int batch, const void* base, float* buf[B_COUNT], int*& table) {
@@ -504,7 +508,7 @@
         v2 * pc(DC8), v2 * pc(DC7), v1 * pc(DC6), v1 * pc(DC5), v1 * pc(DC4), v0 * pc(DC3),
         v0 * pc(DC2), v0 * pc(DC1)};
     Ws ws(base);
-    table = ws.take<int>((size_t)18 * kMaxTilesPerTable * 6);
+    table = ws.take<int>((size_t)kTableRows * kMaxTilesPerTable * 6);
     for (int i = 0; i < B_COUNT; ++i) buf[i] = ws.take<float>(sizes[i] * batch);
     return ws.off;
 }
@@ -534,10 +538,10 @@
     return OAI_OK;
 }
 
-static unsigned xcd_deal(const oai_unet* h, unsigned grid, int& nblocks, int& xcd_group) {
+static unsigned xcd_deal(const oai_unet* h, unsigned grid, int& nblocks, int& xcd_group, int group = 0) {
     if (h->xcd_group <= 0) return grid;
-    nblocks = (int)grid; xcd_group = h->xcd_group;
-    const unsigned q = 8u * (unsigned)h->xcd_group;
+    nblocks = (int)grid; xcd_group = group > 0 ? group : h->xcd_group;
+    const unsigned q = 8u * (unsigned)xcd_group;
     return (grid + q - 1) / q * q;
 }
 
@@ -617,7 +621,7 @@
 }
 
 struct Cover { Box main, xs, ys; int hr, wr; };
-static Cover cover_box(const Box& box, int xunit, int tall_y, int tall_x, bool no_strips) {
+__host__ __device__ static Cover cover_box(const Box& box, int xunit, int tall_y, int tall_x, bool no_strips) {
     const int ry = box.hi[1] - box.lo[1], rx = box.hi[2] - box.lo[2], ny = ry / 8, nx = rx / xunit;
     Cover c{box, box, box, ry - 8 * ny, rx - xunit * nx};
     if (no_strips || ny == 0 || nx == 0) c.hr = c.wr = 0;
@@ -629,6 +633,71 @@
     c.ys.lo[1] = c.main.hi[1]; c.ys.hi[2] = c.main.hi[2];
     return c;
 }
+__host__ __device__ static void tile_cover(const Box& box, Box piece[3]) {
+    Box even = box;
+    even.lo[2] &= ~1;
+    const Cover c = cover_box(even, 8, 4, 4, false);
+    piece[0] = c.main; piece[1] = c.xs; piece[2] = c.ys;
+    piece[0].lo[2] = piece[2].lo[2] = box.lo[2];
+}
+constexpr int kWinoTY[3] = {8, 16, 4}, kWinoTX[3] = {8, 4, 16};
+__host__ __device__ static inline bool box_empty(const Box& b) { return b.hi[0] <= b.lo[0] || b.hi[1] <= b.lo[1] || b.hi[2] <= b.lo[2]; }
+static void piece_blocks(const Box& p, int s, int nb[3]) {
+    nb[0] = nb[1] = nb[2] = 0;
+    if (box_empty(p)) return;
+    nb[0] = cdiv(p.hi[0] - p.lo[0], 4); nb[1] = cdiv(p.hi[1] - p.lo[1], kWinoTY[s]); nb[2] = cdiv(p.hi[2] - (p.lo[2] & ~1), kWinoTX[s]);
+}
+struct OwnPlan { int nb[kOwnLayers][3][3]; int up_nvox[18]; std::vector<int> tile_nb; };
+constexpr int kTileNbStride = kOwnLayers * 3 * 3;
+static void own_plan_add(OwnPlan& op, const Box need[18]) {
+    const size_t row = op.tile_nb.size();
+    op.tile_nb.resize(row + kTileNbStride, 0);
+    for (int k = 0; k < 18; ++k) {
+        if (box_empty(need[k])) continue;
+        if (layer_kind(k) == 2) {
+            int v = 1;
+            for (int i = 0; i < 3; ++i) v *= (need[k].hi[i] + 1) / 2 - need[k].lo[i] / 2;
+            op.up_nvox[k] = std::max(op.up_nvox[k], v);
+        }
+        const int slot = own_cover_slot(k);
+        if (slot < 0) continue;
+        Box piece[3];
+        tile_cover(need[k], piece);
+        for (int s = 0; s < 3; ++s) {
+            int nb[3];
+            piece_blocks(piece[s], s, nb);
+            for (int i = 0; i < 3; ++i) { op.nb[slot][s][i] = std::max(op.nb[slot][s][i], nb[i]); op.tile_nb[row + (slot * 3 + s) * 3 + i] = nb[i]; }
+        }
+    }
+}
+struct OwnCover { const int* rows[3]; int nb[3][3]; int xcd_group[3]; };
+
+static int balanced_xcd_group(int configured, const int* tile_nb, int ntiles, const int nb[3], int ncb) {
+    if (configured <= 0) return configured;
+    auto heaviest = [&](int G) {
+        long long load[8] = {0, 0, 0, 0, 0, 0, 0, 0};
+        for (int t = 0; t < ntiles; ++t) {
+            const int* tn = tile_nb + (size_t)t * kTileNbStride;
+            for (int bz = 0; bz < tn[0]; ++bz)
+                for (int by = 0; by < tn[1]; ++by) {
+                    long long id = (((long long)t * nb[0] + bz) * nb[1] + by) * nb[2] * ncb, left = (long long)tn[2] * ncb;
+                    while (left > 0) {
+                        const long long g = id / G, take = std::min(left, (g + 1) * G - id);
+                        load[g & 7] += take; id += take; left -= take;
+                    }
+                }
+        }
+        return *std::max_element(load, load + 8);
+    };
+    int best = configured;
+    long long best_load = heaviest(configured);
+    for (int G = 30; G >= 16 && best_load > 0; G -= 2) {
+        const long long l = heaviest(G);
+        if (l * 100 < best_load * 98) { best = G; best_load = l; }
+    }
+    return best;
+}
+
 static Cover direct_cover(const oai_unet* h, const Box& box) { return cover_box(box, 16, 4, 8, h->variant == 2); }
 
 static bool first_fusion_ok(const oai_unet* h) {
@@ -696,16 +765,21 @@
     return cout % 128 != 0 && (h->opt_wino & 32) && !(h->opt_wino & (4 | 8)) && L.panel_wino16 && wino_ws_fits();
 }
 
+static inline int wino_groups(const oai_unet* h, int cout, int TY) {
+    return (cout % 128 == 0 && !((h->opt_wino & 8) && TY != 4)) ? 2 : 1;
+}
 template <int TY, int NP>
-static int launch_wino_shape(const oai_unet* h, const Layer& L, ConvArgs a, const Box& box, int ntiles, hipStream_t st) {
+static int launch_wino_shape(const oai_unet* h, const Layer& L, ConvArgs a, const Box& box, int ntiles, hipStream_t st, const int* own_nb = nullptr, int own_group = 0) {
     for (int i = 0; i < 3; ++i) { a.lo[i] = box.lo[i]; a.hi[i] = box.hi[i]; }
     if (box.hi[0] <= box.lo[0] || box.hi[1] <= box.lo[1] || box.hi[2] <= box.lo[2]) return OAI_OK;
-    const int ng = (a.Cout % 128 == 0 && !((h->opt_wino & 8) && TY != 4)) ? 2 : 1;
+    a.own_origin = own_nb != nullptr;
+    const int ng = wino_groups(h, a.Cout, TY);
     a.wpanel = L.panel_wino;
     a.ncb = a.Cout / (64 * ng);
     a.nbz = cdiv(box.hi[0] - box.lo[0], 4); a.nby = cdiv(box.hi[1] - box.lo[1], TY); a.nbx = cdiv(box.hi[2] - box.lo[2], 2 * NP);
+    if (own_nb) { a.nbz = own_nb[0]; a.nby = own_nb[1]; a.nbx = own_nb[2]; }
     unsigned grid = (unsigned)((size_t)ntiles * a.nbz * a.nby * a.nbx * a.ncb);
-    grid = xcd_deal(h, grid, a.nblocks, a.xcd_group);
+    grid = xcd_deal(h, grid, a.nblocks, a.xcd_group, own_group);
     if (int rc = launch_begin(h, st)) return rc;
     if (ng == 2 && (h->opt_wino & 16) && L.panel_wino16) {
         a.wpanel = L.panel_wino16;
@@ -724,7 +798,22 @@
     return launch_end(h, st);
 }
 
-static int launch_conv3_wino(const oai_unet* h, const Layer& L, const ConvArgs& a, Box box, int ntiles, hipStream_t st) {
+static int launch_conv3_wino(const oai_unet* h, const Layer& L, const ConvArgs& a, Box box, int ntiles, hipStream_t st, const OwnCover* oc = nullptr) {
+    if (oc && a.boxes) {
+        const int dims[3] = {a.D, a.H, a.W};
+        Box level;
+        full_box(level, dims);
+        ConvArgs b = a;
+        for (int s = 0; s < 3; ++s) {
+            if (oc->nb[s][0] == 0) continue;
+            b.boxes = oc->rows[s];
+            const int rc = s == 0 ? launch_wino_shape<8, 4>(h, L, b, level, ntiles, st, oc->nb[s], oc->xcd_group[s])
+                         : s == 1 ? launch_wino_shape<16, 2>(h, L, b, level, ntiles, st, oc->nb[s], oc->xcd_group[s])
+                                  : launch_wino_shape<4, 8>(h, L, b, level, ntiles, st, oc->nb[s], oc->xcd_group[s]);
+            if (rc) return rc;
+        }
+        return OAI_OK;
+    }
     box.lo[2] &= ~1;
     const Cover c = cover_box(box, 8, 4, 4, false);
     if (int rc = launch_wino_shape<8, 4>(h, L, a, c.main, ntiles, st)) return rc;
@@ -769,7 +858,7 @@
 static int launch_conv3(const oai_unet* h, const Layer& L, const float* s0, const float* s1, float* out,
                         const int dims[3], const Box& box, int ntiles, hipStream_t st, const int* boxes = nullptr,
                         float* pool_out = nullptr, const ConvArgs* head = nullptr, const TileSource* first = nullptr,
-                        const int* store_boxes = nullptr, const Scatter* sc = nullptr) {
+                        const int* store_boxes = nullptr, const Scatter* sc = nullptr, const OwnCover* oc = nullptr) {
     ConvArgs a;
     if (int rc = fill_conv_args(h, L, s0, s1, out, dims, boxes, pool_out, head, first, store_boxes, sc, a)) return rc;
     if (h->variant == 1) return launch_conv3_shape<2, 16, 16, 2, 4, 1>(h, a, box, ntiles, st);
@@ -778,7 +867,7 @@
         return launch_conv3_wino_f32(h, L, a, box, ntiles, st);
     if (h->sres && h->opt_wino && L.panel_wino && h->sres_mrep == 4 && !a.first_w && !a.head_w && !a.sc_boxes &&
         (!a.pool_out || (a.Cout % 128 == 0 && a.relu && wino_pool_box(box, dims))) && a.Cout % 64 == 0 && (h->opt_wino & (a.Cout % 128 == 0 ? 1 : 2)) && (a.Cout % 128 == 0 || (a.C0 + 15) / 16 + (a.C1 + 15) / 16 >= 8) && layer_bit(h, h->opt_wino_layers, L) && (size_t)dims[0] * dims[1] * dims[2] < (1u << 24))
-        return launch_conv3_wino(h, L, a, box, ntiles, st);
+        return launch_conv3_wino(h, L, a, box, ntiles, st, oc);
     const Cover c = direct_cover(h, box);
     if (int rc = launch_conv3_shape<4, 8, 16, 2, 4, 1>(h, a, c.main, ntiles, st)) return rc;
     if (c.wr) {
@@ -792,7 +881,7 @@
 }
 
 static int launch_up(const oai_unet* h, const Layer& L, const float* src, float* out, const int in_dims[3], const Box& out_need,
-                     int ntiles, hipStream_t st, const int* in_boxes = nullptr) {
+                     int ntiles, hipStream_t st, const int* in_boxes = nullptr, int own_nvox = 0) {
     UpArgs a;
     a.boxes = in_boxes;
     a.range_flag = h->range_flag;
@@ -813,6 +902,7 @@
     a.nnb = cdiv(8 * L.cout, 256);
     a.relu = 1;
     if (split && h->sres) {
+        if (own_nvox > 0 && in_boxes) { a.own_box = 1; a.nmb = cdiv(own_nvox, 128); }
         a.nbw = 1;
         if (L.cout % 16 == 0 && h->opt_up_nbw > 1) a.nbw = std::min(h->opt_up_nbw, a.nnb);
         else if (L.cout % 16 == 0 && h->opt_up_nbw == 0) {
@@ -860,8 +950,22 @@
 
 static int run_batch(oai_unet* h, const TileSource& src, int n, const Box need[18], int out_mode,
                      float* blocks_out, float* const buf[B_COUNT], hipStream_t st,
-                     const int* table = nullptr, int table_tiles = 0, int t0 = 0, const SharedEnc* se = nullptr) {
+                     const int* table = nullptr, int table_tiles = 0, int t0 = 0, const SharedEnc* se = nullptr, const OwnPlan* own = nullptr) {
     auto tb = [&](int layer) -> const int* { return table ? table + ((size_t)layer * table_tiles + t0) * 6 : nullptr; };
+    if (!table || !h->opt_own_cover) own = nullptr;
+    OwnCover ocs[kOwnLayers];
+    auto oc = [&](int layer) -> const OwnCover* {
+        if (!own) return nullptr;
+        const int slot = own_cover_slot(layer);
+        for (int s = 0; s < 3; ++s) {
+            ocs[slot].rows[s] = tb(18 + 3 * slot + s);
+            for (int i = 0; i < 3; ++i) ocs[slot].nb[s][i] = own->nb[slot][s][i];
+            const int ncb = h->L[layer].cout / (64 * wino_groups(h, h->L[layer].cout, kWinoTY[s]));
+            ocs[slot].xcd_group[s] = own->nb[slot][s][0] && ncb > 0 ? balanced_xcd_group(h->xcd_group, own->tile_nb.data() + (slot * 3 + s) * 3, n, own->nb[slot][s], ncb) : 0;
+        }
+        return &ocs[slot];
+    };
+    auto upv = [&](int layer) { return own ? own->up_nvox[layer] : 0; };
     const Layer* L = h->L;
     int d[4][3];
     for (int l = 0; l < 4; ++l) { d[l][0] = src.td >> l; d[l][1] = src.th >> l; d[l][2] = src.tw >> l; }
@@ -979,14 +1083,14 @@
     }
     RUN(launch_conv3(h, L[EC6], buf[B_P2], nullptr, buf[B_E6], d[3], need[EC6], n, st, tb(EC6)));
     RUN(launch_conv3(h, L[EC7], buf[B_E6], nullptr, buf[B_E7], d[3], need[EC7], n, st, tb(EC7)));
-    RUN(launch_up(h, L[DC9], buf[B_E7], buf[B_U9], d[3], need[DC9], n, st, tb(DC9)));
-    RUN(launch_conv3(h, L[DC8], buf[B_U9], buf[B_SYN2], buf[B_D8], d[2], need[DC8], n, st, tb(DC8)));
-    RUN(launch_conv3(h, L[DC7], buf[B_D8], nullptr, buf[B_D7], d[2], need[DC7], n, st, tb(DC7)));
-    RUN(launch_up(h, L[DC6], buf[B_D7], buf[B_U6], d[2], need[DC6], n, st, tb(DC6)));
-    RUN(launch_conv3(h, L[DC5], buf[B_U6], buf[B_SYN1], buf[B_D5], d[1], need[DC5], n, st, tb(DC5)));
-    RUN(launch_conv3(h, L[DC4], buf[B_D5], nullptr, buf[B_D4], d[1], need[DC4], n, st, tb(DC4)));
-    RUN(launch_up(h, L[DC3], buf[B_D4], buf[B_U3], d[1], need[DC3], n, st, tb(DC3)));
-    RUN(launch_conv3(h, L[DC2], buf[B_U3], buf[B_SYN0], buf[B_D2], d[0], need[DC2], n, st, tb(DC2)));
+    RUN(launch_up(h, L[DC9], buf[B_E7], buf[B_U9], d[3], need[DC9], n, st, tb(DC9), upv(DC9)));
+    RUN(launch_conv3(h, L[DC8], buf[B_U9], buf[B_SYN2], buf[B_D8], d[2], need[DC8], n, st, tb(DC8), nullptr, nullptr, nullptr, nullptr, nullptr, oc(DC8)));
+    RUN(launch_conv3(h, L[DC7], buf[B_D8], nullptr, buf[B_D7], d[2], need[DC7], n, st, tb(DC7), nullptr, nullptr, nullptr, nullptr, nullptr, oc(DC7)));
+    RUN(launch_up(h, L[DC6], buf[B_D7], buf[B_U6], d[2], need[DC6], n, st, tb(DC6), upv(DC6)));
+    RUN(launch_conv3(h, L[DC5], buf[B_U6], buf[B_SYN1], buf[B_D5], d[1], need[DC5], n, st, tb(DC5), nullptr, nullptr, nullptr, nullptr, nullptr, oc(DC5)));
+    RUN(launch_conv3(h, L[DC4], buf[B_D5], nullptr, buf[B_D4], d[1], need[DC4], n, st, tb(DC4), nullptr, nullptr, nullptr, nullptr, nullptr, oc(DC4)));
+    RUN(launch_up(h, L[DC3], buf[B_D4], buf[B_U3], d[1], need[DC3], n, st, tb(DC3), upv(DC3)));
+    RUN(launch_conv3(h, L[DC2], buf[B_U3], buf[B_SYN0], buf[B_D2], d[0], need[DC2], n, st, tb(DC2), nullptr, nullptr, nullptr, nullptr, nullptr, oc(DC2)));
     const int kz = src.vol ? src.oz : 0, ky = src.vol ? src.oy : 0, kx = src.vol ? src.ox : 0;
     const int ez = src.vol ? src.ez : src.td, ey = src.vol ? src.ey : src.th, ex = src.vol ? src.ex : src.tw;
     static const bool no_fuse = diag_env("OAI_NO_HEAD_FUSE", 0) != 0;
@@ -1203,6 +1307,7 @@
     {"winograd_f32", &oai_unet::opt_wino_f32, 0, 1, "oai_unet_set_option: winograd_f32 must be 0 or 1"},
     {"first_blocks", &oai_unet::opt_first_blocks, 1, 4096, "oai_unet_set_option: first_blocks must be in [1, 4096]"},
     {"up_nbw", &oai_unet::opt_up_nbw, 0, 64, "oai_unet_set_option: up_nbw must be in [0, 64]"},
+    {"own_cover", &oai_unet::opt_own_cover, 0, 1, "oai_unet_set_option: own_cover must be 0 or 1"},
     {"fuse_first", &oai_unet::fuse_first, 0, 1, "oai_unet_set_option: fuse_first must be 0 or 1"},
     {"xcd_group", &oai_unet::xcd_group, 0, 4096, "oai_unet_set_option: xcd_group must be in [0, 4096]"},
 };
@@ -1475,6 +1580,14 @@
         for (int i = 0; i < 3; ++i) {
             row[i] = up ? need[k].lo[i] / 2 : need[k].lo[i];
             row[3 + i] = up ? (need[k].hi[i] + 1) / 2 : need[k].hi[i];
+        }
+        const int slot = own_cover_slot(k);
+        if (slot < 0) continue;
+        Box piece[3];
+        tile_cover(need[k], piece);
+        for (int s = 0; s < 3; ++s) {
+            int* prow = table + ((size_t)(18 + 3 * slot + s) * n + t) * 6;
+            for (int i = 0; i < 3; ++i) { prow[i] = piece[s].lo[i]; prow[3 + i] = piece[s].hi[i]; }
         }
     }
 }
@@ -1561,8 +1674,10 @@
             const int n = c0 + nc - t < batch ? c0 + nc - t : batch;
             Box uni[18];
             for (int k = 0; k < 18; ++k) for (int i = 0; i < 3; ++i) { uni[k].lo[i] = 1 << 30; uni[k].hi[i] = 0; }
+            OwnPlan own{};
             for (int j = 0; j < n; ++j) {
                 tile_regions(t + j, sp, need);
+                own_plan_add(own, need);
                 for (int k = 0; k < 18; ++k) {
                     if (need[k].hi[0] <= need[k].lo[0]) continue;
                     for (int i = 0; i < 3; ++i) {
@@ -1574,7 +1689,7 @@
             if (uni[0].hi[0] == 0) continue;
             src.tile_begin = t;
             if (int rc = run_batch(h, src, n, uni, out_mode, blocks + (size_t)(t - tile_begin) * h->n_classes * bvox,
-                                   buf, st, table_dev, nc, t - c0, shared ? &se : nullptr)) return rc;
+                                   buf, st, table_dev, nc, t - c0, shared ? &se : nullptr, &own)) return rc;
         }
     }
     return OAI_OK;
@@ -1615,6 +1730,84 @@
     return OAI_OK;
 }
 
+static double started_block_voxels(const Box& launch, int TY, int TX, const Box& tb) {
+    if (box_empty(launch)) return 0.0;
+    Box b;
+    for (int i = 0; i < 3; ++i) { b.lo[i] = std::max(launch.lo[i], tb.lo[i]); b.hi[i] = std::min(launch.hi[i], tb.hi[i]); }
+    if (box_empty(b)) return 0.0;
+    auto started = [&](int i, int T) { int c = 0; for (int o = launch.lo[i]; o < launch.hi[i]; o += T) c += !(o >= b.hi[i] || o + T <= b.lo[i]); return c; };
+    const double yx = (double)started(1, TY) * started(2, TX) * TY * TX;
+    double v = 0.0;
+    for (int oz = launch.lo[0]; oz < launch.hi[0]; oz += 4) {
+        if (oz >= b.hi[0] || oz + 4 <= b.lo[0]) continue;
+        const int m_lo = std::max(0, b.lo[0] - oz), m_hi = std::min(4, b.hi[0] - oz);
+        v += (m_lo == 0 ? m_hi : 4) * yx;
+    }
+    return v;
+}
+
+int oai_unet_cover_stats(int D, int H, int W, const int tile[3], const int overlap[3], const int crop[3], int batch, int layer,
+                         double stats_host[3], int* pieces_host, int n_tiles) {
+    OAI_CHECK_ARG(tile && overlap && stats_host, "oai_unet_cover_stats: null pointer");
+    OAI_CHECK_ARG(batch > 0, "oai_unet_cover_stats: batch must be > 0");
+    const bool up = layer >= 0 && layer < 18 && layer_kind(layer) == 2;
+    OAI_CHECK_ARG(up || (layer >= 0 && layer < 18 && own_cover_slot(layer) >= 0), "oai_unet_cover_stats: layer %d is neither an own-cover conv layer nor an up-conv", layer);
+    if (int rc = check_tile(tile[0], tile[1], tile[2])) return rc;
+    SegGeom g;
+    if (int rc = seg_geometry(D, H, W, tile, overlap, g)) return rc;
+    OAI_CHECK_ARG(!pieces_host || n_tiles == g.ntiles, "oai_unet_cover_stats: the volume has %d tiles, not %d", g.ntiles, n_tiles);
+    const SegParams sp = seg_params(D, H, W, tile, overlap, crop, g, true);
+    auto in_box = [&](Box b) { if (up) for (int i = 0; i < 3; ++i) { b.lo[i] /= 2; b.hi[i] = (b.hi[i] + 1) / 2; } return b; };
+    auto voxels = [](const Box& b) { return box_empty(b) ? 0.0 : (double)(b.hi[0] - b.lo[0]) * (b.hi[1] - b.lo[1]) * (b.hi[2] - b.lo[2]); };
+    Box need[18];
+    stats_host[0] = stats_host[1] = stats_host[2] = 0.0;
+    for (int t0 = 0; t0 < g.ntiles; t0 += batch) {
+        const int n = std::min(batch, g.ntiles - t0);
+        Box uni;
+        for (int i = 0; i < 3; ++i) { uni.lo[i] = 1 << 30; uni.hi[i] = 0; }
+        for (int j = 0; j < n; ++j) {
+            tile_regions(t0 + j, sp, need);
+            if (box_empty(need[layer])) continue;
+            for (int i = 0; i < 3; ++i) { uni.lo[i] = std::min(uni.lo[i], need[layer].lo[i]); uni.hi[i] = std::max(uni.hi[i], need[layer].hi[i]); }
+        }
+        Box launch = in_box(uni);
+        launch.lo[2] &= up ? ~0 : ~1;
+        const Cover c = cover_box(launch, 8, 4, 4, false);
+        for (int j = 0; j < n; ++j) {
+            tile_regions(t0 + j, sp, need);
+            const Box b = in_box(need[layer]);
+            Box piece[3] = {b, {}, {}};
+            stats_host[0] += voxels(b);
+            if (up) {
+                if (!box_empty(b) && !box_empty(launch)) {
+                    const int ryx = (launch.hi[1] - launch.lo[1]) * (launch.hi[2] - launch.lo[2]), nvox = (launch.hi[0] - launch.lo[0]) * ryx;
+                    for (int mb = 0; mb < cdiv(nvox, 128); ++mb) {
+                        const int zf = launch.lo[0] + (mb * 128) / ryx, zl = launch.lo[0] + std::min(mb * 128 + 127, nvox - 1) / ryx;
+                        if (!(zl < b.lo[0] || zf >= b.hi[0])) stats_host[1] += 128.0;
+                    }
+                    stats_host[2] += 128.0 * cdiv((int)voxels(b), 128);
+                }
+            } else {
+                stats_host[1] += started_block_voxels(c.main, 8, 8, b);
+                if (c.wr) stats_host[1] += started_block_voxels(c.xs, 16, 4, b);
+                if (c.hr) stats_host[1] += started_block_voxels(c.ys, 4, 16, b);
+                tile_cover(b, piece);
+                for (int s = 0; s < 3; ++s) {
+                    int nb[3];
+                    piece_blocks(piece[s], s, nb);
+                    if (nb[0]) stats_host[2] += (double)(piece[s].hi[0] - piece[s].lo[0]) * nb[1] * nb[2] * kWinoTY[s] * kWinoTX[s];
+                }
+            }
+            if (pieces_host) {
+                int* row = pieces_host + (size_t)(t0 + j) * 24;
+                for (int i = 0; i < 3; ++i) { row[i] = b.lo[i]; row[3 + i] = b.hi[i]; }
+                for (int s = 0; s < 3; ++s) for (int i = 0; i < 3; ++i) { row[6 + 6 * s + i] = piece[s].lo[i]; row[9 + 6 * s + i] = piece[s].hi[i]; }
+            }
+        }
+    }
+    return OAI_OK;
+}
+
 int oai_stitch_blocks(const float* blocks, int ncls, int D, int H, int W, const int tile[3], const int overlap[3],
                       const int crop[3], float* maps, void* stream) {
     StitchRanges rg{};
diff --git a/oai_analysis_2_amd/csrc/unet_kernels.h b/oai_analysis_2_amd/csrc/unet_kernels.h
--- a/oai_analysis_2_amd/csrc/unet_kernels.h
+++ b/oai_analysis_2_amd/csrc/unet_kernels.h
@@ -45,7 +45,7 @@
     int sc_g[3] = {0, 0, 0}, sc_e[3] = {0, 0, 0}, sc_t[3] = {0, 0, 0};
     unsigned* census = nullptr;
     unsigned* first_census = nullptr;
-    int reserved0 = 0;
+    int own_origin = 0;
     unsigned long long* stamps = nullptr;
     int nblocks = 0, xcd_group = 0;
     int* reserved1 = nullptr;
@@ -466,7 +466,7 @@
     unsigned* census = nullptr;
     const unsigned char* zero = nullptr;
     unsigned long long* stamps = nullptr;
-    int reserved0 = 0;
+    int own_box = 0;
     int nblocks = 0, xcd_group = 0;
     int nbw = 1;
 };
diff --git a/oai_analysis_2_amd/csrc/unet_sres.h b/oai_analysis_2_amd/csrc/unet_sres.h
--- a/oai_analysis_2_amd/csrc/unet_sres.h
+++ b/oai_analysis_2_amd/csrc/unet_sres.h
@@ -809,12 +809,15 @@
     const int tile = id;
     const int N = 8 * a.Cout;
     const int row = lane & 31, half = lane >> 5;
-    const int rz = a.hi[0] - a.lo[0], ry = a.hi[1] - a.lo[1], rx = a.hi[2] - a.lo[2];
-    const int nvox = rz * ry * rx;
     int blo[3], bhi[3];
     if (!tile_box(a.boxes, tile, a.lo, a.hi, blo, bhi)) return;
+    const bool own = a.own_box && a.boxes;
+    const int elo[3] = {own ? blo[0] : a.lo[0], own ? blo[1] : a.lo[1], own ? blo[2] : a.lo[2]};
+    const int rz = (own ? bhi[0] : a.hi[0]) - elo[0], ry = (own ? bhi[1] : a.hi[1]) - elo[1], rx = (own ? bhi[2] : a.hi[2]) - elo[2];
+    const int nvox = rz * ry * rx;
+    if (mb * 128 >= nvox) return;
     {
-        const int zf = a.lo[0] + (mb * 128) / (rx * ry), zl = a.lo[0] + min(mb * 128 + 127, nvox - 1) / (rx * ry);
+        const int zf = elo[0] + (mb * 128) / (rx * ry), zl = elo[0] + min(mb * 128 + 127, nvox - 1) / (rx * ry);
         if (zl < blo[0] || zf >= bhi[0]) return;
     }
     const size_t plane = (size_t)a.D * a.H * a.W;
@@ -827,7 +830,7 @@
         unsigned e = ~0u;
         if (v < nvox) {
             const int x = v % rx, t = v / rx, y = t % ry, z = t / ry;
-            const int iz = a.lo[0] + z, iy = a.lo[1] + y, ix = a.lo[2] + x;
+            const int iz = elo[0] + z, iy = elo[1] + y, ix = elo[2] + x;
             if (iz >= blo[0] && iz < bhi[0] && iy >= blo[1] && iy < bhi[1] && ix >= blo[2] && ix < bhi[2])
                 e = (unsigned)(((2 * iz) * Ho + 2 * iy) * Wo + 2 * ix);
         }
@@ -840,7 +843,7 @@
         if (v < nvox) {
             const int x = v % rx, y = (v / rx) % ry, z = v / (rx * ry);
             asrc[it] = reinterpret_cast<const unsigned char*>(a.src) +
-                       srec(tile, nks, plane, 0, ((size_t)(a.lo[0] + z) * a.H + (a.lo[1] + y)) * a.W + (a.lo[2] + x)) + (((p & 3) ^ ((vl >> 2) & 3)) << 4);
+                       srec(tile, nks, plane, 0, ((size_t)(elo[0] + z) * a.H + (elo[1] + y)) * a.W + (elo[2] + x)) + (((p & 3) ^ ((vl >> 2) & 3)) << 4);
         } else asrc[it] = nullptr;
     }
     unsigned char* outb = reinterpret_cast<unsigned char*>(a.out) + srec(tile, nco, 8 * plane, 0, 0);
diff --git a/oai_analysis_2_amd/csrc/unet_wino.h b/oai_analysis_2_amd/csrc/unet_wino.h
--- a/oai_analysis_2_amd/csrc/unet_wino.h
+++ b/oai_analysis_2_amd/csrc/unet_wino.h
@@ -47,8 +47,8 @@
     auto set_block = [&](int tile_, int bz, int by, int bx, int cbg) __attribute__((always_inline)) -> bool {
         tile = tile_;
         cb = cbg * NG + grp;
-        oz0 = a.lo[0] + bz * TZ; oy0 = a.lo[1] + by * TY; ox0 = a.lo[2] + bx * TX;
         if (!tile_box(a.boxes, tile, a.lo, a.hi, blo, bhi)) return false;
+        oz0 = (a.own_origin ? blo[0] : a.lo[0]) + bz * TZ; oy0 = (a.own_origin ? blo[1] : a.lo[1]) + by * TY; ox0 = (a.own_origin ? blo[2] & ~1 : a.lo[2]) + bx * TX;
         if (oz0 >= bhi[0] || oz0 + TZ <= blo[0] || oy0 >= bhi[1] || oy0 + TY <= blo[1] || ox0 >= bhi[2] || ox0 + TX <= blo[2]) return false;
         m_lo = max(0, blo[0] - oz0); m_hi = min(TZ, bhi[0] - oz0);
         s0 = reinterpret_cast<const unsigned char*>(a.src0) + srec(tile, nch0, plane, 0, 0);
```

Measured after the change: 7.669 (median of 6 runs). +2.1%, better.
